# Fung-Lab/MatDeepLearn

Hardware: AMD Instinct MI355X
Metric: edges/sec training CGCNN on bulk_data (higher is better)
Workload: dtype bf16

## Files before the change

### include/mdl_hip.h

```cpp
#ifndef MDL_HIP_H
#define MDL_HIP_H

#include <stddef.h>
#include <stdint.h>

#ifdef __cplusplus
extern "C" {
#endif

#define MDL_VERSION 100

enum { MDL_F32 = 0, MDL_BF16 = 1 };
enum { MDL_SUM = 0, MDL_MEAN = 1, MDL_MAX = 2 };
enum {
    MDL_OK = 0,
    MDL_E_ARG = -1,
    MDL_E_UNSUPP = -2,
    MDL_E_LAUNCH = -3
};

#define MDL_DTYPE_MASK 0xff
#define MDL_DETERMINISTIC 0x100
#define MDL_K3_PER_WAVE 0x200
#define MDL_K3_EDGE_LANE 0x400
#define MDL_BN_SHIFT_ROW 0x800
#define MDL_SPLIT_BF16 0x1000
#define MDL_MLP_F32_IO 0x2000

typedef void* mdlStream_t;

int mdl_version(void);
const char* mdl_last_error_string(void);
int mdl_debug_last_k3(void);

int mdl_rbf_expand(const float* d, const float* offsets, float coeff, void* out, int64_t E, int G,
                   int64_t ld_out, int out_dtype, mdlStream_t stream);

int mdl_csr_rowptr(const int32_t* sorted_index, int64_t E, int64_t N, int32_t* rowptr, mdlStream_t stream);

int mdl_segment_reduce_fwd(const void* src, const int32_t* rowptr, const int32_t* perm, void* out,
                           int32_t* argmax, int64_t N, int64_t C, int reduce, int dtype, mdlStream_t stream);
int mdl_segment_reduce_bwd(const void* grad_out, const int32_t* rowptr, const int32_t* seg,
                           const int32_t* perm, const int32_t* argmax, void* grad_src, int64_t N,
                           int64_t E, int64_t C, int reduce, int dtype, mdlStream_t stream);
int mdl_segment_reduce_bwd_add(const void* grad_out, const int32_t* rowptr, const int32_t* seg, const int32_t* perm,
                               const void* addend, void* grad_src, int64_t N, int64_t E, int64_t C, int reduce, int dtype,
                               mdlStream_t stream);

size_t mdl_cgconv_wpack_bytes(int C, int G, int dtype);
int mdl_cgconv_pack_weights(const float* w_f, const float* b_f, const float* w_s, const float* b_s, int C,
                            int G, void* wpack, float* bpack, int dtype, mdlStream_t stream);
int mdl_cgconv_pack_weights_node(const float* w_f, const float* b_f, const float* w_s, const float* b_s, int C,
                                 int G, void* wpack, float* bpack, void* wn_t, int dtype, mdlStream_t stream);

int mdl_cgconv_pack_weights_multi(int L, const float* const* w_f, const float* const* b_f, const float* const* w_s,
                                  const float* const* b_s, int C, int G, void* const* wpack, float* const* bpack,
                                  void* const* wn_t, int dtype, mdlStream_t stream);

int mdl_cgconv_fwd(const void* x, const void* edge_attr, const int32_t* rowptr, const int32_t* src,
                   const int32_t* tgt, const int32_t* eperm, const void* wpack, const float* bpack,
                   void* out, int64_t N, int64_t E, int C, int G, int aggr, int dtype, mdlStream_t stream);

typedef struct MdlCgConv {
    uint32_t size;
    int32_t dtype;
    uint32_t flags;
    int32_t aggr;
    int64_t N, E;
    int32_t C, G;
    const void* x;
    const void* edge_attr;
    const int32_t* rowptr;
    const int32_t* src;
    const int32_t* tgt;
    const int32_t* eperm;
    const void* wpack;
    const float* bpack;
    void* out;
    const void* grad_out;
    void* r_tgt;
    void* r_src;
    int32_t r_src_dtype;
    float* dwe;
    float* db;
    void* workspace;
    size_t workspace_bytes;
    const int32_t* balance;
} MdlCgConv;
int mdl_cgconv_fwd_ex(const MdlCgConv* args, mdlStream_t stream);
int mdl_cgconv_bwd_ex(const MdlCgConv* args, mdlStream_t stream);

int mdl_cgconv_balance(const int32_t* rowptr, const int32_t* src, int64_t N, int32_t* cost, mdlStream_t stream);

size_t mdl_cgconv_workspace_bytes(int64_t N, int64_t E, int C, int G, int dtype);

typedef struct MdlCgNode {
    uint32_t size;
    int32_t dtype;
    uint32_t flags;
    int32_t zero_src;
    int64_t N;
    int32_t C;
    int32_t r_src_dtype;
    const void* x;
    const void* grad_out;
    const void* r_tgt;
    void* r_src;
    const void* wn_t;
    void* dx;
    float* dwn;
} MdlCgNode;
int mdl_cgconv_bwd_node_ex(const MdlCgNode* args, mdlStream_t stream);

int mdl_cgconv_pack_node_weights(const float* w_f, const float* w_s, int C, int G, void* wn_t, int dtype, mdlStream_t stream);
int mdl_cgconv_assemble_grads(const float* dwn, const float* dwe, const float* db, int C, int G, float* dw_f, float* dw_s,
                              float* db_f, float* db_s, mdlStream_t stream);

int mdl_assemble_batch(const int64_t* ids, const int64_t* noff, const int64_t* eoff, const int64_t* node_ptr,
                       const int64_t* edge_ptr, const float* x_all, const int32_t* src_l, const int32_t* tgt_l,
                       const float* dist, const float* dist_norm, const int32_t* lrowptr, const float* y_all,
                       void* x, int64_t* batch, int32_t* rowptr, int32_t* src, int32_t* tgt, float* ew, float* dn,
                       float* y, int B, int F, int T, int target_index, int dtype, mdlStream_t stream);
int mdl_assemble_batch_padded(const int64_t* ids, const int64_t* noff, const int64_t* eoff, const int64_t* node_ptr,
                              const int64_t* edge_ptr, const float* x_all, const int32_t* src_l, const int32_t* tgt_l,
                              const float* dist, const float* dist_norm, const int32_t* lrowptr, const float* y_all,
                              void* x, int64_t* batch, int32_t* rowptr, int32_t* src, int32_t* tgt, float* ew, float* dn,
                              float* y, int B, int F, int T, int target_index, int dtype, int64_t n_cap, int64_t e_cap,
                              int32_t* pool_seg, int32_t* col_s, int32_t* eid_s, int32_t* src_s, mdlStream_t stream);

int mdl_ssp_bwd(const void* g, const void* y, void* dx, int64_t n, int dtype, mdlStream_t stream);

int mdl_linear_act_stats(const void* x, const void* w, const void* bias, const void* p1, const int32_t* idx1, const void* p2,
                         const int32_t* idx2, const void* p3, const int32_t* idx3, void* out, int64_t N, int K, int M, int act,
                         float* bn_sums, const int64_t* n_rows_dev, int dtype, mdlStream_t stream);
int mdl_linear_gather_act(const void* x, const void* w, const void* bias, const void* p1, const int32_t* idx1,
                          const void* p2, const int32_t* idx2, const void* p3, const int32_t* idx3, void* out,
                          int64_t N, int K, int M, int act, int dtype, mdlStream_t stream);

int mdl_nnconv_msg_fwd(const void* Y, const void* h, const int32_t* rowptr_s, const int32_t* eid_s, void* m, int64_t N,
                       int Co, int D3, int dtype, mdlStream_t stream);
int mdl_nnconv_msg_bwd(const void* Y, const void* h, const void* dm, const int32_t* rowptr_s, const int32_t* eid_s,
                       void* dh, void* dY, int64_t N, int Co, int D3, int dtype, mdlStream_t stream);

int mdl_pad_batch_tail(const int64_t* noff, const int64_t* eoff, int B, int64_t n_cap, int32_t* rowptr, int64_t* batch,
                       mdlStream_t stream);

int mdl_assemble_transposed(const int64_t* ids, const int64_t* noff, const int64_t* eoff, const int64_t* node_ptr,
                            const int64_t* edge_ptr, const int32_t* src_l, const int32_t* tgt_l, const int32_t* eperm_s,
                            const int32_t* lrowptr_s, int32_t* rowptr_s, int32_t* col_s, int32_t* eid_s, int32_t* src_s, int B,
                            int64_t n_cap, mdlStream_t stream);
int mdl_pad_edge_tail(const int64_t* noff, const int64_t* eoff, int B, int64_t n_cap, int64_t e_cap, int32_t* src, int32_t* tgt,
                      int32_t* col_s, int32_t* eid_s, int32_t* src_s, mdlStream_t stream);

int mdl_loss_fwd_bwd(const float* pred, const float* y, int64_t n, int kind, float* loss, float* grad, mdlStream_t stream);
int mdl_loss_fwd_bwd_rows(const float* pred, const float* y, int64_t n, int64_t n_total, int kind, float* loss, float* grad,
                          mdlStream_t stream);

#define MDL_BN_REPLICAS 16
int mdl_bn_sums_rows(void);
int mdl_bn_stats_n(const void* x, float* sums, int64_t N, int C, const int64_t* n_rows_dev, int dtype, mdlStream_t stream);
int mdl_bn_apply_n(const void* x, float* sums, const float* gamma, const float* beta, float* save, float* running_mean,
                   float* running_var, void* y, int64_t N, int C, float eps, float momentum, const int64_t* n_rows_dev,
                   int dtype, mdlStream_t stream);
int mdl_bn_bwd_stats_n(const void* dy, const void* x, const float* save, float* sums, int64_t N, int C,
                       const int64_t* n_rows_dev, int dtype, mdlStream_t stream);
int mdl_bn_bwd_apply_n(const void* dy, const void* x, const float* save, float* sums, const float* gamma, void* dx,
                       int64_t N, int C, const int64_t* n_rows_dev, int dtype, mdlStream_t stream);
int mdl_bn_bwd_apply_relu_n(const void* dy, const void* x, const float* save, float* sums, const float* gamma, void* dx,
                            int64_t N, int C, const int64_t* n_rows_dev, int dtype, mdlStream_t stream);
int mdl_linear_act(const void* x, const void* w, const void* bias, void* out, int64_t N, int K, int M, int act, int dtype,
                   mdlStream_t stream);
int mdl_linear_act_in(const void* x, const void* y, int xact, const void* w, const void* bias, void* out, int64_t N, int K,
                      int M, int act, int dtype, mdlStream_t stream);

int mdl_mlp_head_fwd(const void* x, const void* const* w, const void* const* b, void* const* h, int64_t N, int K0, int NL,
                     const int* M, int dtype, mdlStream_t stream);
int mdl_mlp_head_bwd(const void* x, const void* const* w, const void* const* h, const void* gy, void* dx, float* const* dw,
                     float* const* db, int64_t N, int K0, int NL, const int* M, int dtype, mdlStream_t stream);

int mdl_gru_gates_fwd(const void* gi, const void* gh, const float* h, float* h_out, void* out_lp, int64_t N, int C, int dtype,
                      mdlStream_t stream);
int mdl_gru_gates_bwd(const void* gi, const void* gh, const float* h, const float* g_h, const void* g_lp, void* dgi, void* dgh,
                      float* dh, int64_t N, int C, int dtype, mdlStream_t stream);

int mdl_linear_wide(const void* x, const void* w, void* out, int64_t N, int K, int64_t M, int dtype, mdlStream_t stream);

int mdl_gemm_tn(const void* a, int64_t lda, int M, const void* b, int64_t ldb, int K, float* c, int64_t N, int dtype,
                mdlStream_t stream);
int mdl_gemm_tn_colsum(const void* a, int64_t lda, int M, const void* b, int64_t ldb, int K, float* c, float* colsum,
                       int64_t N, int dtype, mdlStream_t stream);
int mdl_gemm_tn_act(const void* a, int64_t lda, int M, const void* y, int64_t ldy, int act, const void* b, int64_t ldb,
                    int K, float* c, float* colsum, int64_t N, int dtype, mdlStream_t stream);
int mdl_dense_bwd(const void* g, int64_t ldg, int M, const void* y, int64_t ldy, int act, const void* x, int64_t ldx, int K,
                  const void* w, void* dx, int64_t lddx, int xout, void* gm, float* dw, float* db, int64_t N, int dtype,
                  mdlStream_t stream);
size_t mdl_tn_scratch_bytes(void);
int mdl_dense_bwd_ex(const void* g, int64_t ldg, int M, const void* y, int64_t ldy, int act, const void* x, int64_t ldx, int K,
                     const void* w, void* dx, int64_t lddx, int xout, void* gm, float* dw, float* db, void* scratch, int64_t N,
                     int dtype, mdlStream_t stream);
int mdl_gemm_tn_ex(const void* a, int64_t lda, int M, const void* y, int64_t ldy, int act, const void* b, int64_t ldb, int K,
                   float* c, float* colsum, void* scratch, int64_t N, int dtype, mdlStream_t stream);

int mdl_gather_rows(const void* src, const int32_t* idx, void* out, int64_t E, int64_t C, int dtype,
                    mdlStream_t stream);
int mdl_gather_mul_reduce(const void* h, const void* w, const float* scale, const int32_t* rowptr,
                          const int32_t* col, const int32_t* eid, void* out, int64_t N, int64_t F, int reduce,
                          int dtype, mdlStream_t stream);
int mdl_gather_mul_reduce_dw(const void* g, const void* w, const float* scale, const int32_t* rowptr_s,
                             const int32_t* col_s, const int32_t* eid_s, void* dh, const void* h, void* dw,
                             int64_t N, int64_t F, int dtype, mdlStream_t stream);
int mdl_cfconv_supported(int F, int G, int dtype);
size_t mdl_cfconv_wpack_bytes(void);
int mdl_cfconv_pack_weights(const float* w1, const float* b1, const float* w2, const float* b2, int F, int G, void* wpack,
                            mdlStream_t stream);
int mdl_cfconv_fwd(const void* rbf, const float* cut, const void* h, const int32_t* rowptr, const int32_t* src,
                   const int32_t* tgt, const void* wpack, void* out, void* a1, void* w, int64_t N, int64_t E, int F, int G,
                   int dtype, mdlStream_t stream);
size_t mdl_cfconv_bwd_w_scratch_bytes(void);
int mdl_cfconv_bwd_w(const void* rbf, const float* cut, const void* h, const void* g, const int32_t* rowptr, const int32_t* src,
                     const int32_t* tgt, const void* wpack, float* dw1, float* db1, float* dw2, float* db2, void* scratch, int64_t N,
                     int64_t E, int F, int G, int dtype, mdlStream_t stream);
int mdl_edge_mul(const void* a, const int32_t* ia, const void* b, const int32_t* ib, const float* scale, void* out,
                 int64_t E, int64_t F, int dtype, mdlStream_t stream);
int mdl_edge_dot(const void* a, const int32_t* ia, const void* b, const int32_t* ib, const void* w, float* out, int64_t E,
                 int64_t F, int dtype, mdlStream_t stream);
int mdl_cfconv_bwd_edge_supported(int F, int G, int dtype);
int mdl_cfconv_bwd_edge(const void* rbf, const float* cut, const void* h, const void* g, const int32_t* rowptr, const int32_t* src,
                        const int32_t* tgt, const void* wpack, const float* w1, const float* b1, const float* w2, const float* b2,
                        int64_t N, int64_t E, int F, int G, int dtype, float* dcut, void* drbf, const float* d_norm,
                        const float* offsets, float coeff, float scale, float* dd, mdlStream_t stream);

int mdl_split_bf16(const float* src, void* hi, void* lo, int64_t n, mdlStream_t stream);

size_t mdl_graph_workspace_bytes(int64_t N, int64_t G, int max_neighbors);
int mdl_graph_build(const double* pos, const int64_t* node_ptr, const double* cell, const int32_t* pbc, int64_t N, int64_t G,
                    double radius, int max_neighbors, int64_t* edge_ptr, int32_t* src, int32_t* tgt, float* dist,
                    int32_t* out_deg, int64_t edge_capacity, void* workspace, size_t workspace_bytes, mdlStream_t stream);

int mdl_rbf_expand_bwd(const void* g_out, int64_t ld_g, int g_dtype, const float* d, const float* offsets, float coeff,
                       float* dd, int64_t E, int G, mdlStream_t stream);

int mdl_cgconv_bwd_edge(const void* x, const void* edge_attr, const int32_t* rowptr, const int32_t* src, const int32_t* tgt,
                        const void* wpack, const float* bpack, const void* grad_out, int64_t N, int64_t E, int C, int G,
                        int aggr, int dtype, void* de, const float* d_norm, const float* offsets, float coeff, float scale,
                        float* dd, mdlStream_t stream);

int mdl_linear_rbf_dist_grad_supported(int M, int G, int dtype);
int mdl_linear_rbf_dist_grad(const void* g, int64_t ld_g, const void* act_y, int64_t ld_y, const void* w, int dtype,
                             const float* d, const float* offsets, float coeff, float scale, float* dd, int accumulate,
                             int64_t E, int M, int G, mdlStream_t stream);

size_t mdl_edge_geometry_workspace_bytes(int64_t G);
int mdl_edge_geometry_fwd(const double* pos, const int64_t* node_ptr, const double* cell, const int32_t* pbc, int64_t N,
                          int64_t G, const int32_t* src, const int32_t* tgt, int64_t E, float* dist, float* u,
                          void* workspace, size_t workspace_bytes, mdlStream_t stream);
int mdl_edge_geometry_bwd(const float* dd, const float* u, const int32_t* rowptr_t, const int32_t* eid_t,
                          const int32_t* rowptr_s, const int32_t* eid_s, int64_t N, int64_t E, float* dpos,
                          mdlStream_t stream);

size_t mdl_edge_strain_grad_workspace_bytes(int64_t G, int64_t E, int32_t slices);
int mdl_edge_strain_grad(const float* dd, const float* dist, const float* u, const int32_t* rowptr_t, const int32_t* eid_t,
                         const int64_t* node_ptr, int64_t N, int64_t G, int64_t E, int32_t slices, float* out, void* workspace,
                         size_t workspace_bytes, mdlStream_t stream);
// ... 37 lines not shown
```

### matdeeplearn_amd/_build.py

```python
import os
import shutil
import subprocess
import sys
from concurrent.futures import ThreadPoolExecutor

HERE = os.path.dirname(os.path.abspath(__file__))
CSRC = os.path.join(HERE, "csrc")
LIBDIR = os.path.join(HERE, "lib")
OBJDIR = os.path.join(HERE, "lib", "obj")
LIB = os.path.join(LIBDIR, "libmdl_hip.so")
FLAGS = ["--offload-arch=gfx950", "-O3", "-std=c++17", "-fPIC", "-munsafe-fp-atomics", "-Wno-unused-result"]
FILE_FLAGS = {"cgconv_ep.hip": ["-mllvm", "-amdgpu-mfma-vgpr-form=1"], "cfconv.hip": ["-mllvm", "-amdgpu-mfma-vgpr-form=1"],
              "graph_build.hip": ["-ffp-contract=off"],
              "edge_geom.hip": ["-ffp-contract=off"],
              "vacf.hip": ["-ffp-contract=off"]}
FILE_DEPS = {}


def _hipcc():
    for c in (os.environ.get("HIPCC"), "/opt/rocm/bin/hipcc", shutil.which("hipcc")):
        if c and os.path.exists(c):
            return c
    raise RuntimeError("hipcc not found (need ROCm >= 7.0 to build libmdl_hip.so)")


def sources():
    return sorted(os.path.join(CSRC, f) for f in os.listdir(CSRC) if f.endswith(".hip"))


def _deps_mtime():
    hdrs = [os.path.join(CSRC, f) for f in os.listdir(CSRC) if f.endswith((".h", ".inc"))]
    hdrs += [os.path.join(os.path.dirname(HERE), "include", h) for h in ("mdl_hip.h", "mdl_hip_analysis.h", "mdl_hip_dynamics.h")]
    return max(os.path.getmtime(h) for h in hdrs)


def needs_build():
    if not os.path.exists(LIB):
        return True
    t = os.path.getmtime(LIB)
    return any(os.path.getmtime(s) > t for s in sources()) or _deps_mtime() > t


def build(force=False, verbose=True):
    if not force and not needs_build():
        return LIB
    cc = _hipcc()
    os.makedirs(OBJDIR, exist_ok=True)
    hdr_t = _deps_mtime()

    def compile_one(src):
        base = os.path.basename(src)
        obj = os.path.join(OBJDIR, base[:-4] + ".o")
        src_t = max([os.path.getmtime(src)] + [os.path.getmtime(os.path.join(CSRC, d)) for d in FILE_DEPS.get(base, [])])
        if force or not os.path.exists(obj) or os.path.getmtime(obj) < max(src_t, hdr_t):
            cmd = [cc] + FLAGS + FILE_FLAGS.get(base, []) + ["-c", src, "-o", obj]
            if verbose:
                print("[mdl build]", " ".join(cmd), file=sys.stderr)
            subprocess.run(cmd, check=True)
        return obj

    with ThreadPoolExecutor(max_workers=4) as ex:
        objs = list(ex.map(compile_one, sources()))
    cmd = [cc, "--offload-arch=gfx950", "-shared", "-fPIC", "-o", LIB] + objs
    if verbose:
        print("[mdl build]", " ".join(cmd), file=sys.stderr)
    subprocess.run(cmd, check=True)
    return LIB


if __name__ == "__main__":
    print(build(force="--force" in sys.argv))
```

### matdeeplearn_amd/_lib.py

```python
import ctypes
import os

import torch

HERE = os.path.dirname(os.path.abspath(__file__))
LIB_PATH = os.path.join(HERE, "lib", "libmdl_hip.so")


def use_library(path):
    global LIB_PATH, _lib
    if _lib is not None and os.path.abspath(path) != os.path.abspath(LIB_PATH):
        raise MdlError("use_library(%s): %s is already loaded in this process" % (path, LIB_PATH))
    LIB_PATH = path

MDL_F32, MDL_BF16 = 0, 1
MDL_SUM, MDL_MEAN, MDL_MAX = 0, 1, 2
MDL_DTYPE_MASK, MDL_DETERMINISTIC, MDL_K3_PER_WAVE, MDL_K3_EDGE_LANE = 0xFF, 0x100, 0x200, 0x400
MDL_MLP_F32_IO = 0x2000
MDL_SPLIT_BF16 = 0x1000
MDL_BN_SHIFT_ROW = 0x800
MDL_BN_REPLICAS = 16
REDUCE = {"sum": MDL_SUM, "add": MDL_SUM, "mean": MDL_MEAN, "max": MDL_MAX}

_vp, _i64, _i32, _f32, _sz = ctypes.c_void_p, ctypes.c_int64, ctypes.c_int, ctypes.c_float, ctypes.c_size_t
_u32 = ctypes.c_uint32


class MdlCgConv(ctypes.Structure):
    _fields_ = [("size", _u32), ("dtype", _i32), ("flags", _u32), ("aggr", _i32), ("N", _i64), ("E", _i64), ("C", _i32), ("G", _i32),
                ("x", _vp), ("edge_attr", _vp), ("rowptr", _vp), ("src", _vp), ("tgt", _vp), ("eperm", _vp), ("wpack", _vp),
                ("bpack", _vp), ("out", _vp), ("grad_out", _vp), ("r_tgt", _vp), ("r_src", _vp), ("r_src_dtype", _i32),
                ("dwe", _vp), ("db", _vp), ("workspace", _vp), ("workspace_bytes", _sz), ("balance", _vp)]


class MdlCgNode(ctypes.Structure):
    _fields_ = [("size", _u32), ("dtype", _i32), ("flags", _u32), ("zero_src", _i32), ("N", _i64), ("C", _i32), ("r_src_dtype", _i32),
                ("x", _vp), ("grad_out", _vp), ("r_tgt", _vp), ("r_src", _vp), ("wn_t", _vp), ("dx", _vp), ("dwn", _vp)]


def _dp(t):
    return None if t is None else t.data_ptr()


def cg_args(**kw):
    a = MdlCgConv()
    a.size = ctypes.sizeof(MdlCgConv)
    for k, v in kw.items():
        setattr(a, k, _dp(v) if torch.is_tensor(v) else v)
    return a


def cg_node_args(**kw):
    a = MdlCgNode()
    a.size = ctypes.sizeof(MdlCgNode)
    for k, v in kw.items():
        setattr(a, k, _dp(v) if torch.is_tensor(v) else v)
    return a

PROTOTYPES = {
    "mdl_version": (_i32, []),
    "mdl_last_error_string": (ctypes.c_char_p, []),
    "mdl_debug_last_k3": (_i32, []),
    "mdl_rbf_expand": (_i32, [_vp, _vp, _f32, _vp, _i64, _i32, _i64, _i32, _vp]),
    "mdl_csr_rowptr": (_i32, [_vp, _i64, _i64, _vp, _vp]),
    "mdl_segment_reduce_fwd": (_i32, [_vp, _vp, _vp, _vp, _vp, _i64, _i64, _i32, _i32, _vp]),
    "mdl_segment_reduce_bwd": (_i32, [_vp, _vp, _vp, _vp, _vp, _vp, _i64, _i64, _i64, _i32, _i32, _vp]),
    "mdl_segment_reduce_bwd_add": (_i32, [_vp, _vp, _vp, _vp, _vp, _vp, _i64, _i64, _i64, _i32, _i32, _vp]),
    "mdl_cgconv_wpack_bytes": (_sz, [_i32, _i32, _i32]),
    "mdl_cgconv_pack_weights": (_i32, [_vp, _vp, _vp, _vp, _i32, _i32, _vp, _vp, _i32, _vp]),
    "mdl_cgconv_pack_weights_node": (_i32, [_vp, _vp, _vp, _vp, _i32, _i32, _vp, _vp, _vp, _i32, _vp]),
    "mdl_cgconv_pack_weights_multi": (_i32, [_i32, _vp, _vp, _vp, _vp, _i32, _i32, _vp, _vp, _vp, _i32, _vp]),
    "mdl_cgconv_fwd": (_i32, [_vp] * 9 + [_i64, _i64, _i32, _i32, _i32, _i32, _vp]),
    "mdl_cgconv_fwd_ex": (_i32, [ctypes.POINTER(MdlCgConv), _vp]),
    "mdl_cgconv_bwd_ex": (_i32, [ctypes.POINTER(MdlCgConv), _vp]),
    "mdl_cgconv_bwd_node_ex": (_i32, [ctypes.POINTER(MdlCgNode), _vp]),
    "mdl_cgconv_workspace_bytes": (ctypes.c_size_t, [_i64, _i64, _i32, _i32, _i32]),
    "mdl_cgconv_balance": (_i32, [_vp, _vp, _i64, _vp, _vp]),
    "mdl_cgconv_pack_node_weights": (_i32, [_vp, _vp, _i32, _i32, _vp, _i32, _vp]),
    "mdl_cgconv_assemble_grads": (_i32, [_vp, _vp, _vp, _i32, _i32, _vp, _vp, _vp, _vp, _vp]),
    "mdl_assemble_batch": (_i32, [_vp] * 20 + [_i32, _i32, _i32, _i32, _i32, _vp]),
    "mdl_assemble_batch_padded": (_i32, [_vp] * 20 + [_i32, _i32, _i32, _i32, _i32, _i64, _i64, _vp, _vp, _vp, _vp, _vp]),
    "mdl_nnconv_msg_fwd": (_i32, [_vp] * 5 + [_i64, _i32, _i32, _i32, _vp]),
    "mdl_nnconv_msg_bwd": (_i32, [_vp] * 7 + [_i64, _i32, _i32, _i32, _vp]),
    "mdl_pad_batch_tail": (_i32, [_vp, _vp, _i32, _i64, _vp, _vp, _vp]),
    "mdl_assemble_transposed": (_i32, [_vp] * 13 + [_i32, _i64, _vp]),
    "mdl_pad_edge_tail": (_i32, [_vp, _vp, _i32, _i64, _i64, _vp, _vp, _vp, _vp, _vp, _vp]),
    "mdl_loss_fwd_bwd": (_i32, [_vp, _vp, _i64, _i32, _vp, _vp, _vp]),
    "mdl_loss_fwd_bwd_rows": (_i32, [_vp, _vp, _i64, _i64, _i32, _vp, _vp, _vp]),
    "mdl_bn_sums_rows": (_i32, []),
    "mdl_bn_stats_n": (_i32, [_vp, _vp, _i64, _i32, _vp, _i32, _vp]),
    "mdl_bn_apply_n": (_i32, [_vp] * 8 + [_i64, _i32, _f32, _f32, _vp, _i32, _vp]),
    "mdl_bn_bwd_stats_n": (_i32, [_vp, _vp, _vp, _vp, _i64, _i32, _vp, _i32, _vp]),
    "mdl_bn_bwd_apply_n": (_i32, [_vp] * 6 + [_i64, _i32, _vp, _i32, _vp]),
    "mdl_bn_bwd_apply_relu_n": (_i32, [_vp] * 6 + [_i64, _i32, _vp, _i32, _vp]),
    "mdl_linear_act": (_i32, [_vp, _vp, _vp, _vp, _i64, _i32, _i32, _i32, _i32, _vp]),
    "mdl_dense_bwd": (_i32, [_vp, _i64, _i32, _vp, _i64, _i32, _vp, _i64, _i32, _vp, _vp, _i64, _i32, _vp, _vp, _vp, _i64, _i32, _vp]),
    "mdl_dense_bwd_ex": (_i32, [_vp, _i64, _i32, _vp, _i64, _i32, _vp, _i64, _i32, _vp, _vp, _i64, _i32, _vp, _vp, _vp, _vp, _i64, _i32, _vp]),
    "mdl_tn_scratch_bytes": (_sz, []),
    "mdl_linear_act_stats": (_i32, [_vp, _vp, _vp, _vp, _vp, _vp, _vp, _vp, _vp, _vp, _i64, _i32, _i32, _i32, _vp, _vp, _i32, _vp]),
    "mdl_linear_act_in": (_i32, [_vp, _vp, _i32, _vp, _vp, _vp, _i64, _i32, _i32, _i32, _i32, _vp]),
    "mdl_ssp_bwd": (_i32, [_vp, _vp, _vp, _i64, _i32, _vp]),
    "mdl_linear_gather_act": (_i32, [_vp] * 10 + [_i64, _i32, _i32, _i32, _i32, _vp]),
    "mdl_linear_wide": (_i32, [_vp, _vp, _vp, _i64, _i32, _i64, _i32, _vp]),
    "mdl_mlp_head_fwd": (_i32, [_vp, _vp, _vp, _vp, _i64, _i32, _i32, _vp, _i32, _vp]),
    "mdl_mlp_head_bwd": (_i32, [_vp, _vp, _vp, _vp, _vp, _vp, _vp, _i64, _i32, _i32, _vp, _i32, _vp]),
    "mdl_gru_gates_fwd": (_i32, [_vp, _vp, _vp, _vp, _vp, _i64, _i32, _i32, _vp]),
    "mdl_gru_gates_bwd": (_i32, [_vp, _vp, _vp, _vp, _vp, _vp, _vp, _vp, _i64, _i32, _i32, _vp]),
    "mdl_gemm_tn": (_i32, [_vp, _i64, _i32, _vp, _i64, _i32, _vp, _i64, _i32, _vp]),
    "mdl_split_bf16": (_i32, [_vp, _vp, _vp, _i64, _vp]),
    "mdl_gemm_tn_colsum": (_i32, [_vp, _i64, _i32, _vp, _i64, _i32, _vp, _vp, _i64, _i32, _vp]),
    "mdl_gemm_tn_act": (_i32, [_vp, _i64, _i32, _vp, _i64, _i32, _vp, _i64, _i32, _vp, _vp, _i64, _i32, _vp]),
    "mdl_gemm_tn_ex": (_i32, [_vp, _i64, _i32, _vp, _i64, _i32, _vp, _i64, _i32, _vp, _vp, _vp, _i64, _i32, _vp]),
    "mdl_gather_rows": (_i32, [_vp, _vp, _vp, _i64, _i64, _i32, _vp]),
    "mdl_gather_mul_reduce": (_i32, [_vp] * 7 + [_i64, _i64, _i32, _i32, _vp]),
    "mdl_gather_mul_reduce_dw": (_i32, [_vp] * 9 + [_i64, _i64, _i32, _vp]),
    "mdl_edge_mul": (_i32, [_vp] * 6 + [_i64, _i64, _i32, _vp]),
    "mdl_cfconv_supported": (_i32, [_i32, _i32, _i32]),
    "mdl_cfconv_wpack_bytes": (_sz, []),
    "mdl_cfconv_pack_weights": (_i32, [_vp] * 4 + [_i32, _i32, _vp, _vp]),
    "mdl_cfconv_fwd": (_i32, [_vp] * 10 + [_i64, _i64, _i32, _i32, _i32, _vp]),
    "mdl_cfconv_bwd_w_scratch_bytes": (_sz, []),
    "mdl_cfconv_bwd_w": (_i32, [_vp] * 13 + [_i64, _i64, _i32, _i32, _i32, _vp]),
    "mdl_cfconv_bwd_edge_supported": (_i32, [_i32, _i32, _i32]),
    "mdl_cfconv_bwd_edge": (_i32, [_vp] * 12 + [_i64, _i64, _i32, _i32, _i32, _vp, _vp, _vp, _vp, _f32, _f32, _vp, _vp]),
    "mdl_edge_dot": (_i32, [_vp] * 6 + [_i64, _i64, _i32, _vp]),
    "mdl_graph_workspace_bytes": (_sz, [_i64, _i64, _i32]),
    "mdl_graph_build": (_i32, [_vp] * 4 + [_i64, _i64, ctypes.c_double, _i32] + [_vp] * 5 + [_i64, _vp, _sz, _vp]),
    "mdl_rbf_expand_bwd": (_i32, [_vp, _i64, _i32, _vp, _vp, _f32, _vp, _i64, _i32, _vp]),
    "mdl_cgconv_bwd_edge": (_i32, [_vp] * 8 + [_i64, _i64, _i32, _i32, _i32, _i32, _vp, _vp, _vp, _f32, _f32, _vp, _vp]),
    "mdl_linear_rbf_dist_grad_supported": (_i32, [_i32, _i32, _i32]),
    "mdl_linear_rbf_dist_grad": (_i32, [_vp, _i64, _vp, _i64, _vp, _i32, _vp, _vp, _f32, _f32, _vp, _i32, _i64, _i32, _i32, _vp]),
    "mdl_edge_geometry_workspace_bytes": (_sz, [_i64]),
    "mdl_edge_geometry_fwd": (_i32, [_vp] * 4 + [_i64, _i64, _vp, _vp, _i64, _vp, _vp, _vp, _sz, _vp]),
    "mdl_edge_geometry_bwd": (_i32, [_vp] * 6 + [_i64, _i64, _vp, _vp]),
    "mdl_edge_strain_grad_workspace_bytes": (_sz, [_i64, _i64, _i32]),
    "mdl_edge_strain_grad": (_i32, [_vp] * 6 + [_i64, _i64, _i64, _i32, _vp, _vp, _sz, _vp]),
    "mdl_set2set_supported": (_i32, [_i32, _i32, _i32]),
    "mdl_set2set_fwd": (_i32, [_vp] * 12 + [_i64, _i64, _i32, _i32, _i32, _vp]),
    "mdl_set2set_bwd": (_i32, [_vp] * 13 + [_i64, _i64, _i32, _i32, _i32, _vp]),
    "mdl_fire_step": (_i32, [_vp] * 5 + [_i64, _i64] + [_vp] * 7 + [_i32] + [ctypes.c_double] * 6 + [_vp, _vp, _i64] + [_vp] * 9 + [_vp]),
    "mdl_fire_cell_step": (_i32, [_vp] * 13 + [_i64, _i64] + [_vp] * 9 + [_i32] + [ctypes.c_double] * 7 + [_vp]),
    "mdl_md_step": (_i32, [_vp] * 6 + [_i64, _i64] + [_vp] * 8 + [ctypes.c_double] + [_vp] * 6 + [ctypes.c_double, _vp]),
    "mdl_md_velocities": (_i32, [_vp] * 4 + [_i64, _i64, _vp, _vp, _i32, _vp]),
}

_f64 = ctypes.c_double
ANALYSIS_PROTOTYPES = {
    "mdl_rdf_accumulate": (_i32, [_vp] * 6 + [_i64, _i64, _i64, _f64, _i32, _i32] + [_vp] * 4 + [_vp]),
    "mdl_msd_accumulate": (_i32, [_vp] * 8 + [_i64, _i64, _i32, _i32, _i32, _i32, _vp, _vp, _vp]),
}

DYNAMICS_PROTOTYPES = {
    "mdl_md_onstep_velocity": (_i32, [_vp] * 8 + [_i64, _i64, _vp, _vp]),
    "mdl_vacf_accumulate": (_i32, [_vp] * 8 + [_i64, _i64, _i32, _i32, _i32, _i32, _vp, _vp, _vp]),
}

_lib = None


class MdlError(RuntimeError):
    pass


def lib():
    global _lib
    if _lib is None:
        if not os.path.exists(LIB_PATH):
            raise MdlError(
                "libmdl_hip.so not found at %s — build it with `python -m matdeeplearn_amd._build` "
                "(hipcc --offload-arch=gfx950).  matdeeplearn_amd has no CPU/eager fallback." % LIB_PATH)
        handle = ctypes.CDLL(LIB_PATH)
        for name, (res, args) in list(PROTOTYPES.items()) + list(ANALYSIS_PROTOTYPES.items()) + list(DYNAMICS_PROTOTYPES.items()):
            fn = getattr(handle, name)
            fn.restype, fn.argtypes = res, args
        _lib = handle
    return _lib


def check(rc, what):
    if rc != 0:
        raise MdlError("%s failed (%d): %s" % (what, rc, lib().mdl_last_error_string().decode()))


def dtype_code(t):
    if t.dtype == torch.float32:
        return MDL_F32
    if t.dtype == torch.bfloat16:
        return MDL_BF16
    raise MdlError("unsupported dtype %s (float32 or bfloat16)" % t.dtype)


def require_hip(*tensors):
    cur = None
    for t in tensors:
        if t is None:
            continue
        if not t.is_cuda:
            raise MdlError("matdeeplearn_amd ops need tensors on a HIP device (got %s); there is no CPU path — "
                           "the CPU restatement lives in oracle/ and is test infrastructure only" % t.device)
        if cur is None:
            cur = torch.cuda.current_device()
        if t.device.index != cur:
            raise MdlError("tensor on %s but the current HIP device is cuda:%d — call torch.cuda.set_device(%d) in "
                           "this process before using matdeeplearn_amd" % (t.device, cur, t.device.index))


def ptr(t):
    return None if t is None else ctypes.c_void_p(t.data_ptr())


def stream():
    return ctypes.c_void_p(torch._C._cuda_getCurrentRawStream(torch.cuda.current_device()))
```

### matdeeplearn_amd/csrc/cgconv.hip

```cpp
#include "cgconv_tiles.inc"
#include "cgconv_fwd.inc"
#include "cgconv_bwd.inc"

namespace mdl {
#if MDL_EXPERIMENTS
#include "../../experiments/csrc/cgconv_ab.inc"
#include "../../experiments/csrc/cgconv_cb.inc"
#endif
namespace ep {
constexpr int EP_DEFAULT = 2;
constexpr int64_t EP2_MIN_EDGES = 400000;
#if MDL_EXPERIMENTS
int launch(CgParams& p, hipStream_t st, int wgs, const char* name);
#endif
int launch2(CgParams& p, hipStream_t st, int wgs, const char* name);
}

template <typename T>
__device__ __forceinline__ void cgconv_pack_body(const float* __restrict__ wf, const float* __restrict__ bfv,
                                                 const float* __restrict__ ws, const float* __restrict__ bsv,
                                                 int C, int G, const CgDims& d, T* __restrict__ wpack,
                                                 float* __restrict__ bpack, float scale, int bias_col,
                                                 bf16_t* __restrict__ wn_t, int x3 = 0) {
    const int total = 2 * d.Cp * d.WS;
    const int ldw = 2 * C + G;
    if (wn_t) {
        const int tn = C * 4 * d.Cp;
        for (int q = blockIdx.x * blockDim.x + threadIdx.x; q < tn; q += gridDim.x * blockDim.x) {
            const int k = q / (4 * d.Cp), r = q - k * (4 * d.Cp);
            const int blk = r / d.Cp, c = r - blk * d.Cp;
            float v = 0.0f;
            if (c < C) v = ((blk & 1) ? ws : wf)[c * ldw + (blk >> 1) * C + k];
            wn_t[q] = f2bf(v);
        }
    }
    for (int q = blockIdx.x * blockDim.x + threadIdx.x; q < total; q += gridDim.x * blockDim.x) {
        const int row = q / d.WS, k = q - row * d.WS;
        const int part = row / d.Cp, c = row - part * d.Cp;
        const float* W = part ? ws : wf;
        float v = 0.0f;
        if (c < C) {
            if (k < d.KE) {
                if (k < G) v = W[c * ldw + 2 * C + k];
                else if (k == G && bias_col) { const float* b = part ? bsv : bfv; v = b ? b[c] : 0.0f; }
            } else if (k < d.KE + d.Cp) {
                const int kc = k - d.KE;
                if (kc < C) v = W[c * ldw + kc];
            } else if (k < d.KT) {
                const int kc = k - d.KE - d.Cp;
                if (kc < C) v = W[c * ldw + C + kc];
            }
        }
        if constexpr (std::is_same<T, float>::value) {
            if (x3) {
                if (k < d.KT) {
                    unsigned hi, lo;
                    split_pair(v * scale, 0.0f, hi, lo);
                    bf16_t* g = reinterpret_cast<bf16_t*>(wpack + row * d.WS) + (k >> 3) * 16 + (k & 7);
                    g[0] = (bf16_t)(hi & 0xffffu);
                    g[8] = (bf16_t)(lo & 0xffffu);
                } else {
                    wpack[q] = 0.0f;
                }
                continue;
            }
        }
        Elem<T>::st(wpack + q, v * scale);
    }
    for (int q = blockIdx.x * blockDim.x + threadIdx.x; q < 2 * d.Cp; q += gridDim.x * blockDim.x) {
        const int part = q / d.Cp, c = q - part * d.Cp;
        const float* b = part ? bsv : bfv;
        bpack[q] = (c < C && b) ? b[c] * scale : 0.0f;
    }
}

template <typename T>
__global__ __launch_bounds__(256) void cgconv_pack_kernel(const float* __restrict__ wf, const float* __restrict__ bfv,
                                                          const float* __restrict__ ws, const float* __restrict__ bsv,
                                                          int C, int G, CgDims d, T* __restrict__ wpack,
                                                          float* __restrict__ bpack, float scale, int bias_col,
                                                          bf16_t* __restrict__ wn_t = nullptr, int x3 = 0) {
    cgconv_pack_body<T>(wf, bfv, ws, bsv, C, G, d, wpack, bpack, scale, bias_col, wn_t, x3);
}

constexpr int PACK_MAXL = 16;
struct PackMulti {
    const float* wf[PACK_MAXL]; const float* bf[PACK_MAXL]; const float* ws[PACK_MAXL]; const float* bs[PACK_MAXL];
    void* wpack[PACK_MAXL]; float* bpack[PACK_MAXL]; bf16_t* wn_t[PACK_MAXL];
};
template <typename T>
__global__ __launch_bounds__(256) void cgconv_pack_multi_kernel(PackMulti a, int C, int G, CgDims d, float scale, int bias_col, int x3 = 0) {
    const int l = blockIdx.y;
    cgconv_pack_body<T>(a.wf[l], a.bf[l], a.ws[l], a.bs[l], C, G, d, static_cast<T*>(a.wpack[l]), a.bpack[l], scale, bias_col, a.wn_t[l], x3);
}

#if MDL_EXPERIMENTS
__global__ __launch_bounds__(256) void cgconv_pack_split_kernel(const float* __restrict__ wf, const float* __restrict__ bfv,
                                                                const float* __restrict__ ws, const float* __restrict__ bsv,
                                                                int C, int G, int Cp, int KE, int WSe, bf16_t* __restrict__ wpe,
                                                                bf16_t* __restrict__ wproj, float scale) {
    const int ldw = 2 * C + G;
    const int ne = 2 * Cp * WSe, np_ = 2 * 2 * Cp * Cp;
    for (int q = blockIdx.x * blockDim.x + threadIdx.x; q < ne + np_; q += gridDim.x * blockDim.x) {
        float v = 0.0f;
        if (q < ne) {
            const int row = q / WSe, k = q - row * WSe;
            const int part = row / Cp, c = row - part * Cp;
            const float* W = part ? ws : wf;
            if (c < C) {
                if (k < G) v = W[c * ldw + 2 * C + k];
                else if (k == G) { const float* b = part ? bsv : bfv; v = b ? b[c] : 0.0f; }
            }
            wpe[q] = f2bf(v * scale);
        } else {
            const int r = q - ne;
            const int side = r / (2 * Cp * Cp), rr = r - side * (2 * Cp * Cp);
            const int row = rr / Cp, k = rr - row * Cp;
            const int part = row / Cp, c = row - part * Cp;
            const float* W = part ? ws : wf;
            if (c < C && k < C) v = W[c * ldw + side * C + k];
            wproj[r] = f2bf(v * scale);
        }
    }
}
#endif

static constexpr int LDS_CAP = 160 * 1024;
constexpr int FWD_RANGE_EDGES = 64;
constexpr int BWD_RANGE_EDGES = 128;

struct CgEnv {
    int64_t grid_cap;
    int cb_fwd, cb_bwd;
    int cb_wgs;
    int ab_wgs;
    int no_half_groups;
    int no_fast128;
    int no_w_slice;
    int ep;
    int ep_wgs;
};
static const CgEnv& cg_env() {
#if MDL_EXPERIMENTS
    static const CgEnv e = [] {
        CgEnv v;
        const char* s;
        v.grid_cap = (s = getenv("MDL_GRID_CAP")) ? atoll(s) : 0;
        v.cb_fwd = (s = getenv("MDL_CG_CB")) ? (atoi(s) != 0) : -1;
        v.cb_bwd = (s = getenv("MDL_CG_CB_BWD")) ? (atoi(s) != 0) : -1;
        v.cb_wgs = (s = getenv("MDL_CB_WGS")) ? atoi(s) : 0;
        v.ab_wgs = (s = getenv("MDL_AB_WGS")) ? atoi(s) : 0;
        v.no_half_groups = (s = getenv("MDL_CG_NO_HALF")) ? (atoi(s) != 0) : 0;
        v.no_w_slice = (s = getenv("MDL_CG_NO_WSLICE")) ? (atoi(s) != 0) : 0;
        v.no_fast128 = (s = getenv("MDL_CG_NO_FAST128")) ? (atoi(s) != 0) : 0;
        v.ep = (s = getenv("MDL_CG_EP")) ? atoi(s) : -1;
        v.ep_wgs = (s = getenv("MDL_EP_WGS")) ? atoi(s) : 0;
        return v;
    }();
#else
    static const CgEnv e = {0, -1, -1, 0, 0, 0, 0, 0, -1, 0};
#endif
    return e;
}

static volatile int g_last_k3 = 0;

template <typename T>
static int cg_launch(bool bwd, CgParams& p, int dtype, hipStream_t st, const char* name) {
    const bool x3 = (p.flags & MDL_SPLIT_BF16) != 0;
    const CgDims d = cg_dims(p.C, p.G, dtype, x3);
    p.Cp = d.Cp; p.KE = d.KE; p.KT = d.KT; p.WS = d.WS; p.EKS = d.EKS; p.NS = d.NS; p.GP = d.GP;
    p.w_elems = 2 * d.Cp * d.WS;
    const bool wsp = p.pt != nullptr;
    if (wsp) { p.WS = d.EKS; p.w_elems = 2 * d.Cp * d.EKS; }
    p.bias_col = (p.G % 16) != 0;
    p.n_groups = (int)cdiv(p.N, 32);
    if (p.n_groups == 0) return MDL_OK;

    const bool word4 = (p.G * sizeof(T)) % 4 == 0 && (reinterpret_cast<uintptr_t>(p.ea) % 4) == 0;
    const int EW = word4 ? (int)(4 / sizeof(T)) : 1;
    p.GW = p.G / EW;
    p.gw_inv = (unsigned)((0x100000000ull + p.GW - 1) / p.GW);

    int vec = 1;
    if (sizeof(T) == 2) {
        const bool a16 = reinterpret_cast<uintptr_t>(p.x) % 16 == 0, a8 = reinterpret_cast<uintptr_t>(p.x) % 8 == 0;
        if (p.C % 8 == 0 && a16) vec = 8; else if (p.C % 4 == 0 && a8) vec = 4;
    }

    const int et_bytes = (32 * d.EKS * (int)sizeof(T) + 15) & ~15;
    p.wave_lds_bytes = et_bytes + 32 + 128 + 32 + 16 + ((bwd && sizeof(T) == 2) ? 128 * OHS * 2 + 64 + 256 : 0);
    const int w_bytes = (p.w_elems * (int)sizeof(T) + 15) & ~15;
    const bool det = bwd && (p.flags & MDL_DETERMINISTIC) != 0;
    const int waves = det ? 1 : (bwd ? 4 : FWD_THREADS / 64);
    const bool fast = !p.eperm && p.G == 50 && p.C == d.Cp && (d.Cp == 32 || d.Cp == 64) &&
                      (sizeof(T) == 2 ? (vec == 8 && EW == 2) : d.Cp == 64) &&
                      (bwd || (reinterpret_cast<uintptr_t>(p.out) % 16 == 0 && reinterpret_cast<uintptr_t>(p.x) % 16 == 0));
    const bool fast128 = sizeof(T) == 2 && !wsp && !p.ab && !p.eperm && p.G == 50 && p.C == 128 && d.Cp == 128 && vec == 8 && EW == 2 &&
                         p.bias_col && reinterpret_cast<uintptr_t>(p.x) % 16 == 0 &&
                         (bwd ? reinterpret_cast<uintptr_t>(p.gout) % 16 == 0 : reinterpret_cast<uintptr_t>(p.out) % 16 == 0) &&
                         !cg_env().no_fast128;
    bool w_lds = w_bytes + waves * p.wave_lds_bytes <= LDS_CAP;
    int lds = (w_lds ? w_bytes : 0) + waves * p.wave_lds_bytes;
    p.w_slice = 0;
    if (!w_lds && !fast && !wsp && d.NS > 1 && (d.WS * (int)sizeof(T)) % 16 == 0 &&
        64 * d.WS * (int)sizeof(T) + waves * p.wave_lds_bytes <= LDS_CAP && !cg_env().no_w_slice) {
        p.w_slice = 1;
        p.w_elems = 64 * d.WS;
        w_lds = true;
        lds = 64 * d.WS * (int)sizeof(T) + waves * p.wave_lds_bytes;
    }
    const int wg_per_cu = lds * 2 <= LDS_CAP ? 2 : 1;

    const bool all_slices = !bwd && fast && (sizeof(T) == 2 || w_lds);
    const int64_t ranges = std::max<int64_t>(1, std::min<int64_t>(cdiv(p.E, bwd ? BWD_RANGE_EDGES : FWD_RANGE_EDGES), p.N));
    int64_t items = ranges * (all_slices ? 1 : d.NS);
    int64_t grid = cdiv(items, waves);
    const int64_t cap = 256 * ((bwd && BWD_WAVES == 1) ? 1 : wg_per_cu);
    if (grid > cap) grid = cap;
    const CgEnv& env = cg_env();
    if (env.grid_cap > 0 && grid > env.grid_cap) grid = env.grid_cap;
    if (det) { grid = d.NS; p.ctr = nullptr; }
    if constexpr (sizeof(T) == 2) {
        int ep_sel = env.ep >= 0 ? env.ep : ep::EP_DEFAULT;
        if (p.flags & MDL_K3_PER_WAVE) ep_sel = 0;
        const bool force2 = env.ep == 2 || (p.flags & MDL_K3_EDGE_LANE) != 0;
        if (force2) ep_sel = 2;
        if (ep_sel != 0 && !det && bwd && fast && !wsp && d.Cp == 64 && p.bias_col && p.E >= 64) {
            if (ep_sel == 2 && p.rs16 && (force2 || p.E >= ep::EP2_MIN_EDGES)) { g_last_k3 = 2; return ep::launch2(p, st, env.ep_wgs, name); }
#if MDL_EXPERIMENTS
            if (ep_sel == 1 && !p.rs16) return ep::launch(p, st, env.ep_wgs, name);
#endif
        }
    }
    if (bwd) g_last_k3 = det ? 3 : 1;
    p.dwe_combine = (bwd && !det && waves == 4 && d.NS == 2 && w_lds && !p.w_slice && w_bytes >= 2 * 2 * 2 * 16 * 64 * 4) ? 1 : 0;
    while ((grid * waves) % d.NS) ++grid;
    if (p.w_slice) while (grid % d.NS) ++grid;
    p.g_full = p.n_groups;
    if (bwd && p.ctr) {
        if ((int64_t)p.n_groups * d.NS >= 4 * grid * waves && d.NS <= 16) {
            if (hipMemsetAsync(p.ctr, 0, 64, st) != hipSuccess) { set_error("%s: workspace memset failed", name); return MDL_E_LAUNCH; }
            const int64_t tail = 2 * (grid * waves / d.NS);
            p.g_full = (int)std::max<int64_t>(0, (int64_t)p.n_groups - tail);
            if (env.no_half_groups) p.g_full = p.n_groups;
        } else {
            p.ctr = nullptr;
        }
    }

#if MDL_EXPERIMENTS
    if constexpr (sizeof(T) == 2) {
        if (!bwd && p.ab) {
            if (!(fast && all_slices && p.bias_col)) {
                set_error("%s: the saved-gate forward supports bf16, C in {32, 64}, G = 50, target-sorted edge features", name);
                return MDL_E_UNSUPP;
            }
            if (d.Cp == 64) {
                auto kf = cgconv_fwd_kernel<T, 64, 50, 9, 2, 1, true>;
                (void)set_max_dynamic_lds(reinterpret_cast<const void*>(kf), lds);
                hipLaunchKernelGGL(kf, dim3((unsigned)grid), dim3(waves * 64), lds, st, p);
            } else {
                auto kf = cgconv_fwd_kernel<T, 32, 50, 9, 2, 1, true>;
                (void)set_max_dynamic_lds(reinterpret_cast<const void*>(kf), lds);
                hipLaunchKernelGGL(kf, dim3((unsigned)grid), dim3(waves * 64), lds, st, p);
            }
            return check_launch(name);
        }
    }

    if constexpr (sizeof(T) == 2) {
        constexpr int CB_FWD_WG_PER_CU = 2;
        if (env.cb_fwd > 0 && fast && !wsp && !bwd && p.E >= 64 && p.bias_col) {
            const int cb_wgs = env.cb_wgs > 0 ? env.cb_wgs : CB_FWD_WG_PER_CU;
            int64_t cb_grid = std::min<int64_t>(256 * cb_wgs, ranges);
            if (env.grid_cap > 0 && cb_grid > env.grid_cap) cb_grid = env.grid_cap;
            if (d.Cp == 64) {
                const int cb_lds = 2 * cb::Cfg<64>::BUF_FWD;
                hipLaunchKernelGGL(cb::fwd_kernel<64>, dim3((unsigned)cb_grid), dim3(cb::Cfg<64>::NT), cb_lds, st, p);
            } else {
                const int cb_lds = 2 * cb::Cfg<32>::BUF_FWD;
                hipLaunchKernelGGL(cb::fwd_kernel<32>, dim3((unsigned)cb_grid), dim3(cb::Cfg<32>::NT), cb_lds, st, p);
            }
            return check_launch(name);
        }
        if (env.cb_bwd > 0 && fast && !wsp && !p.rs16 && bwd && p.E >= 64 && p.bias_col) {
            const int cb_wgs = env.cb_wgs > 0 ? env.cb_wgs : MDL_CB_BWD_OCC;
            const int64_t cb_grid = std::min<int64_t>(256 * cb_wgs, ranges);
            if (d.Cp == 64) {
                const int cb_lds = 2 * cb::BwdLds<64>::BUF + cb::Cfg<64>::NCB * 32 * (cb::Cfg<64>::KE + 8) * 2;
                auto kf = cb::bwd_kernel<64>;
                set_max_dynamic_lds(reinterpret_cast<const void*>(kf), cb_lds);
                hipLaunchKernelGGL(kf, dim3((unsigned)cb_grid), dim3(cb::Cfg<64>::NT), cb_lds, st, p);
            } else {
                const int cb_lds = 2 * cb::BwdLds<32>::BUF + cb::Cfg<32>::NCB * 32 * (cb::Cfg<32>::KE + 8) * 2;
                auto kf = cb::bwd_kernel<32>;
                set_max_dynamic_lds(reinterpret_cast<const void*>(kf), cb_lds);
                hipLaunchKernelGGL(kf, dim3((unsigned)cb_grid), dim3(cb::Cfg<32>::NT), cb_lds, st, p);
            }
            return check_launch(name);
        }
    }

#endif

#define MDL_CG_LAUNCH(CP_, G_, VEC_, EW_, WM_)                                                               \
    do {                                                                                                     \
        auto kf = bwd ? cgconv_bwd_kernel<T, CP_, G_, VEC_, EW_, WM_> : cgconv_fwd_kernel<T, CP_, G_, VEC_, EW_, WM_>; \
        hipError_t e = set_max_dynamic_lds(reinterpret_cast<const void*>(kf), lds);                 \
        if (e != hipSuccess) { set_error("%s: LDS attribute (%d B): %s", name, lds, hipGetErrorString(e)); return MDL_E_LAUNCH; } \
        hipLaunchKernelGGL(kf, dim3((unsigned)grid), dim3(waves * 64), lds, st, p);                           \
    } while (0)
#define MDL_CG_BY_WL(VEC_, EW_) do { if (w_lds) MDL_CG_LAUNCH(0, 0, VEC_, EW_, 1); else MDL_CG_LAUNCH(0, 0, VEC_, EW_, 0); } while (0)
#define MDL_CG_BY_EW(VEC_) do { if (EW == 2) MDL_CG_BY_WL(VEC_, 2); else MDL_CG_BY_WL(VEC_, 1); } while (0)

#if MDL_EXPERIMENTS
    if (wsp) {
        if constexpr (sizeof(T) == 2) {
            if (!(fast && w_lds && p.bias_col && (bwd || all_slices))) {
                set_error("%s: the W-split kernels support bf16, C in {32, 64}, G = 50, target-sorted edge features", name);
                return MDL_E_UNSUPP;
            }
#define MDL_CG_LAUNCH_WSP(CP_)                                                                                         \
            do {                                                                                                       \
                hipError_t e;                                                                                          \
                if (bwd) {                                                                                             \
                    auto kf = cgconv_bwd_kernel<T, CP_, 50, 9, 2, 1, 1>;                                               \
                    e = set_max_dynamic_lds(reinterpret_cast<const void*>(kf), lds);                                   \
                    if (e == hipSuccess) hipLaunchKernelGGL(kf, dim3((unsigned)grid), dim3(waves * 64), lds, st, p);   \
                } else {                                                                                               \
                    auto kf = cgconv_fwd_kernel<T, CP_, 50, 9, 2, 1, false, 1>;                                        \
                    e = set_max_dynamic_lds(reinterpret_cast<const void*>(kf), lds);                                   \
                    if (e == hipSuccess) hipLaunchKernelGGL(kf, dim3((unsigned)grid), dim3(waves * 64), lds, st, p);   \
                }                                                                                                      \
                if (e != hipSuccess) { set_error("%s: LDS attribute (%d B): %s", name, lds, hipGetErrorString(e)); return MDL_E_LAUNCH; } \
            } while (0)
            if (d.Cp == 64) MDL_CG_LAUNCH_WSP(64); else MDL_CG_LAUNCH_WSP(32);
#undef MDL_CG_LAUNCH_WSP
            return check_launch(name);
        } else {
            set_error("%s: the W-split kernels are bf16 only", name);
            return MDL_E_UNSUPP;
        }
    }
#endif
#ifdef MDL_CG_FAST_ONLY
    if constexpr (sizeof(T) == 2) {
        if (fast && d.Cp == 64) MDL_CG_LAUNCH(64, 50, 9, 2, 1);
        else if (fast128 && p.w_slice) MDL_CG_LAUNCH(128, 50, 9, 2, 1);
    }
#else
    if constexpr (sizeof(T) == 2) {
        if (fast && d.Cp == 64) MDL_CG_LAUNCH(64, 50, 9, 2, 1);
        else if (fast && d.Cp == 32) MDL_CG_LAUNCH(32, 50, 9, 2, 1);
        else if (fast128 && p.w_slice) MDL_CG_LAUNCH(128, 50, 9, 2, 1);
        else if (vec == 8) MDL_CG_BY_EW(8);
        else if (vec == 4) MDL_CG_BY_EW(4);
        else MDL_CG_BY_EW(1);
    } else {
        if (x3) {
            const bool x3_64 = fast && w_lds && d.Cp == 64;
            const bool x3_128 = !p.eperm && p.G == 50 && p.C == 128 && d.Cp == 128 && w_lds && p.w_slice;
            if (!((x3_64 || x3_128) && p.bias_col && !wsp && !det && reinterpret_cast<uintptr_t>(p.x) % 16 == 0)) {
                set_error("%s: MDL_SPLIT_BF16 needs fp32, C = 64 or 128, G = 50, edge features in CSR order, 16-byte aligned x", name);
                return MDL_E_UNSUPP;
            }
            hipError_t e;
#define MDL_CG_LAUNCH_X3(CP_)                                                                                                 \
            do {                                                                                                              \
                if (bwd) {                                                                                                    \
                    auto kf = cgconv_bwd_kernel<T, CP_, 50, 9, 1, 1, 0, true>;                                                \
                    e = set_max_dynamic_lds(reinterpret_cast<const void*>(kf), lds);                                          \
                    if (e == hipSuccess) hipLaunchKernelGGL(kf, dim3((unsigned)grid), dim3(waves * 64), lds, st, p);          \
                } else {                                                                                                      \
                    auto kf = cgconv_fwd_kernel<T, CP_, 50, 9, 1, 1, false, 0, true>;                                         \
                    e = set_max_dynamic_lds(reinterpret_cast<const void*>(kf), lds);                                          \
                    if (e == hipSuccess) hipLaunchKernelGGL(kf, dim3((unsigned)grid), dim3(waves * 64), lds, st, p);          \
                }                                                                                                             \
            } while (0)
            if (x3_64) MDL_CG_LAUNCH_X3(64); else MDL_CG_LAUNCH_X3(128);
#undef MDL_CG_LAUNCH_X3
            if (e != hipSuccess) { set_error("%s: LDS attribute (%d B): %s", name, lds, hipGetErrorString(e)); return MDL_E_LAUNCH; }
        }
        else if (fast && w_lds) MDL_CG_LAUNCH(64, 50, 9, 1, 1);
        else MDL_CG_BY_WL(1, 1);
    }
#endif
#undef MDL_CG_BY_EW
// ... 163 lines not shown
    p.flags = (int)(a->flags & MDL_SPLIT_BF16);
    if (a->dtype == MDL_BF16) return cg_launch<bf16_t>(false, p, a->dtype, (hipStream_t)stream, "mdl_cgconv_fwd_ex");
    return cg_launch<float>(false, p, a->dtype, (hipStream_t)stream, "mdl_cgconv_fwd_ex");
}

extern "C" size_t mdl_cgconv_workspace_bytes(int64_t, int64_t, int, int, int) { return 64; }

#if MDL_EXPERIMENTS
extern "C" size_t mdl_cgconv_gate_row_bytes(int C, int G, int dtype) {
    return (dtype == MDL_BF16 && G == 50 && (C == 32 || C == 64)) ? (size_t)4 * C : 0;
}

extern "C" int mdl_cgconv_fwd_save(const void* x, const void* edge_attr, const int32_t* rowptr, const int32_t* src,
                                   const int32_t* tgt, const void* wpack, const float* bpack, void* out, void* gate,
                                   int64_t N, int64_t E, int C, int G, int aggr, int dtype, mdlStream_t stream) {
    using namespace mdl;
    int rc = cg_check("mdl_cgconv_fwd_save", x, edge_attr, rowptr, src, tgt, wpack, bpack, N, E, C, G, aggr, dtype);
    if (rc) return rc;
    MDL_REQUIRE(mdl_cgconv_gate_row_bytes(C, G, dtype) != 0, MDL_E_UNSUPP,
                "mdl_cgconv_fwd_save: unsupported C=%d G=%d dtype=%d (bf16, C in {32, 64}, G = 50)", C, G, dtype);
    MDL_REQUIRE(N == 0 || out, MDL_E_ARG, "mdl_cgconv_fwd_save: null out");
    MDL_REQUIRE(E == 0 || (gate && reinterpret_cast<uintptr_t>(gate) % 4 == 0), MDL_E_ARG, "mdl_cgconv_fwd_save: bad gate buffer");
    MDL_REQUIRE(reinterpret_cast<uintptr_t>(x) % 16 == 0 && reinterpret_cast<uintptr_t>(edge_attr) % 4 == 0, MDL_E_ARG,
                "mdl_cgconv_fwd_save: x must be 16-byte and edge_attr 4-byte aligned");
    CgParams p = {};
    p.x = x; p.ea = edge_attr; p.rowptr = rowptr; p.src = src; p.tgt = tgt; p.eperm = nullptr;
    p.wpack = wpack; p.bpack = bpack; p.out = out; p.ab = E ? gate : nullptr; p.N = N; p.E = E; p.C = C; p.G = G; p.aggr = aggr;
    return cg_launch<bf16_t>(false, p, dtype, (hipStream_t)stream, "mdl_cgconv_fwd_save");
}

extern "C" int mdl_cgconv_bwd_saved(const void* edge_attr, const int32_t* rowptr, const int32_t* src, const int32_t* tgt,
                                    const void* gate, const void* grad_out, void* r_tgt, float* r_src, float* dwe, float* db,
                                    int64_t N, int64_t E, int C, int G, int aggr, int dtype, void* workspace, size_t ws_bytes,
                                    mdlStream_t stream) {
    using namespace mdl;
    MDL_REQUIRE(mdl_cgconv_gate_row_bytes(C, G, dtype) != 0, MDL_E_UNSUPP,
                "mdl_cgconv_bwd_saved: unsupported C=%d G=%d dtype=%d (bf16, C in {32, 64}, G = 50)", C, G, dtype);
    MDL_REQUIRE(N >= 0 && E >= 0 && N < (1ll << 31) - 64 && E < (1ll << 31) - 64, MDL_E_ARG, "mdl_cgconv_bwd_saved: bad N=%lld E=%lld",
                (long long)N, (long long)E);
    MDL_REQUIRE(aggr == MDL_MEAN || aggr == MDL_SUM, MDL_E_UNSUPP, "mdl_cgconv_bwd_saved: unsupported aggr %d", aggr);
    MDL_REQUIRE(N == 0 || (rowptr && grad_out && r_tgt && r_src && dwe), MDL_E_ARG, "mdl_cgconv_bwd_saved: null pointer");
    MDL_REQUIRE(E == 0 || (edge_attr && src && tgt && gate), MDL_E_ARG, "mdl_cgconv_bwd_saved: null edge pointer");
    MDL_REQUIRE(reinterpret_cast<uintptr_t>(gate) % 4 == 0 && reinterpret_cast<uintptr_t>(edge_attr) % 4 == 0, MDL_E_ARG,
                "mdl_cgconv_bwd_saved: gate / edge_attr must be 4-byte aligned");
    CgParams p = {};
    p.ea = edge_attr; p.rowptr = rowptr; p.src = src; p.tgt = tgt; p.ab = const_cast<void*>(gate); p.gout = grad_out;
    p.r_tgt = r_tgt; p.r_src = r_src; p.dwe = dwe; p.db = db; p.N = N; p.E = E; p.C = C; p.G = G; p.aggr = aggr;
    p.ctr = (workspace && ws_bytes >= 64) ? static_cast<unsigned*>(workspace) : nullptr;
    return cg_launch_bwd_ab(p, (hipStream_t)stream, "mdl_cgconv_bwd_saved");
}

extern "C" size_t mdl_cgconv_wsplit_bytes(int C, int G, int dtype, int which) {
    using namespace mdl;
    if (dtype != MDL_BF16 || G != 50 || (C != 32 && C != 64)) return 0;
    const CgDims d = cg_dims(C, G, dtype);
    const size_t b = which == 0 ? (size_t)2 * d.Cp * d.EKS * 2 : (size_t)2 * 2 * d.Cp * d.Cp * 2;
    return (b + 15) & ~(size_t)15;
}

extern "C" int mdl_cgconv_pack_weights_split(const float* w_f, const float* b_f, const float* w_s, const float* b_s, int C,
                                             int G, void* wpack_e, void* wproj, float* bpack, int dtype, mdlStream_t stream) {
    using namespace mdl;
    MDL_REQUIRE(w_f && w_s && wpack_e && wproj && bpack, MDL_E_ARG, "mdl_cgconv_pack_weights_split: null pointer");
    MDL_REQUIRE(mdl_cgconv_wsplit_bytes(C, G, dtype, 0) != 0, MDL_E_UNSUPP,
                "mdl_cgconv_pack_weights_split: unsupported C=%d G=%d dtype=%d (bf16, C in {32, 64}, G = 50)", C, G, dtype);
    const CgDims d = cg_dims(C, G, dtype);
    const int total = 2 * d.Cp * d.EKS + 4 * d.Cp * d.Cp;
    hipStream_t st = (hipStream_t)stream;
    hipLaunchKernelGGL(cgconv_pack_split_kernel, dim3((unsigned)cdiv(total, 256)), dim3(256), 0, st, w_f, b_f, w_s, b_s, C, G, d.Cp,
                       d.KE, d.EKS, (bf16_t*)wpack_e, (bf16_t*)wproj, Gate<true>::W_SCALE);
    if (hipMemsetAsync(bpack, 0, 2 * d.Cp * sizeof(float), st) != hipSuccess) { set_error("mdl_cgconv_pack_weights_split: memset failed"); return MDL_E_LAUNCH; }
    return check_launch("mdl_cgconv_pack_weights_split");
}

extern "C" int mdl_cgconv_fwd_p(const void* x, const void* p_tgt, const void* p_src, const void* edge_attr, const int32_t* rowptr,
                                const int32_t* src, const int32_t* tgt, const void* wpack_e, const float* bpack, void* out,
                                int64_t N, int64_t E, int C, int G, int aggr, int dtype, mdlStream_t stream) {
    using namespace mdl;
    int rc = cg_check("mdl_cgconv_fwd_p", x, edge_attr, rowptr, src, tgt, wpack_e, bpack, N, E, C, G, aggr, dtype);
    if (rc) return rc;
    MDL_REQUIRE(N == 0 || (out && p_tgt && p_src), MDL_E_ARG, "mdl_cgconv_fwd_p: null pointer");
    MDL_REQUIRE(reinterpret_cast<uintptr_t>(p_tgt) % 16 == 0 && reinterpret_cast<uintptr_t>(p_src) % 16 == 0, MDL_E_ARG,
                "mdl_cgconv_fwd_p: the projections must be 16-byte aligned");
    CgParams p = {};
    p.x = x; p.pt = p_tgt; p.ps = p_src; p.ea = edge_attr; p.rowptr = rowptr; p.src = src; p.tgt = tgt; p.eperm = nullptr;
    p.wpack = wpack_e; p.bpack = bpack; p.out = out; p.N = N; p.E = E; p.C = C; p.G = G; p.aggr = aggr;
    if (dtype != MDL_BF16) { set_error("mdl_cgconv_fwd_p: bf16 only"); return MDL_E_UNSUPP; }
    return cg_launch<bf16_t>(false, p, dtype, (hipStream_t)stream, "mdl_cgconv_fwd_p");
}

extern "C" int mdl_cgconv_bwd_p(const void* p_tgt, const void* p_src, const void* edge_attr, const int32_t* rowptr,
                                const int32_t* src, const int32_t* tgt, const void* wpack_e, const float* bpack,
                                const void* grad_out, void* r_tgt, float* r_src, float* dwe, float* db, int64_t N, int64_t E,
                                int C, int G, int aggr, int dtype, void* workspace, size_t ws_bytes, mdlStream_t stream) {
    using namespace mdl;
    int rc = cg_check("mdl_cgconv_bwd_p", p_tgt, edge_attr, rowptr, src, tgt, wpack_e, bpack, N, E, C, G, aggr, dtype);
    if (rc) return rc;
    MDL_REQUIRE(N == 0 || (grad_out && r_tgt && r_src && dwe && p_src), MDL_E_ARG, "mdl_cgconv_bwd_p: null pointer");
    MDL_REQUIRE(reinterpret_cast<uintptr_t>(p_tgt) % 16 == 0 && reinterpret_cast<uintptr_t>(p_src) % 16 == 0, MDL_E_ARG,
                "mdl_cgconv_bwd_p: the projections must be 16-byte aligned");
    CgParams p = {};
    p.x = p_tgt; p.pt = p_tgt; p.ps = p_src; p.ea = edge_attr; p.rowptr = rowptr; p.src = src; p.tgt = tgt; p.eperm = nullptr;
    p.wpack = wpack_e; p.bpack = bpack; p.gout = grad_out; p.r_tgt = r_tgt; p.r_src = r_src; p.dwe = dwe; p.db = db;
    p.N = N; p.E = E; p.C = C; p.G = G; p.aggr = aggr;
    p.ctr = (workspace && ws_bytes >= mdl_cgconv_workspace_bytes(N, E, C, G, dtype)) ? static_cast<unsigned*>(workspace) : nullptr;
    if (dtype != MDL_BF16) { set_error("mdl_cgconv_bwd_p: bf16 only"); return MDL_E_UNSUPP; }
    return cg_launch<bf16_t>(true, p, dtype, (hipStream_t)stream, "mdl_cgconv_bwd_p");
}
#endif

namespace mdl {
__global__ __launch_bounds__(256) void cgconv_balance_kernel(const int32_t* __restrict__ rowptr, const int32_t* __restrict__ src,
                                                             int64_t N, int32_t* __restrict__ cost, int far_w, int far_t, int zero_w) {
    const int64_t n = (int64_t)blockIdx.x * blockDim.x + threadIdx.x;
    if (n == 0) cost[0] = 0;
    if (n >= N) return;
    const int b = rowptr[n], e = rowptr[n + 1];
    int far = 0;
    for (int k = b; k < e; ++k) {
        const int d = src[k] - (int)n;
        far += (d >= far_t || d <= -far_t) ? 1 : 0;
    }
    cost[n + 1] = 4 * (e - b + 1) + far_w * far + (e == b ? zero_w : 0);
}
}

extern "C" int mdl_cgconv_balance(const int32_t* rowptr, const int32_t* src, int64_t N, int32_t* cost, mdlStream_t stream) {
    using namespace mdl;
    MDL_REQUIRE(N >= 0 && (N == 0 || (rowptr && src && cost)), MDL_E_ARG, "mdl_cgconv_balance: bad arguments");
#if MDL_EXPERIMENTS
    static const int far_w = [] { const char* s = getenv("MDL_BAL_W"); return s ? atoi(s) : 5; }();
    static const int far_t = [] { const char* s = getenv("MDL_BAL_T"); return s ? atoi(s) : 48; }();
    static const int zero_w = [] { const char* s = getenv("MDL_BAL_Z"); return s ? atoi(s) : 4; }();
#else
    constexpr int far_w = 5, far_t = 48, zero_w = 4;
#endif
    hipLaunchKernelGGL(cgconv_balance_kernel, dim3((unsigned)cdiv(N + 1, 256)), dim3(256), 0, (hipStream_t)stream, rowptr, src, N, cost,
                       far_w, far_t, zero_w);
    return check_launch("mdl_cgconv_balance");
}

extern "C" int mdl_cgconv_bwd_ex(const MdlCgConv* a, mdlStream_t stream) {
    using namespace mdl;
    MDL_REQUIRE(a && a->size == sizeof(MdlCgConv), MDL_E_ARG, "mdl_cgconv_bwd_ex: argument struct of another layout (size %u, expected %u)",
                a ? a->size : 0u, (unsigned)sizeof(MdlCgConv));
    MDL_REQUIRE((a->flags & ~(uint32_t)(MDL_DETERMINISTIC | MDL_K3_PER_WAVE | MDL_K3_EDGE_LANE | MDL_SPLIT_BF16)) == 0, MDL_E_ARG,
                "mdl_cgconv_bwd_ex: unknown flag bits %#x", a->flags);
    MDL_REQUIRE(!(a->flags & MDL_SPLIT_BF16) || (a->dtype == MDL_F32 && !(a->flags & MDL_DETERMINISTIC)), MDL_E_UNSUPP,
                "mdl_cgconv_bwd_ex: MDL_SPLIT_BF16 goes with MDL_F32 storage (and not with MDL_DETERMINISTIC)");
    const int dtype = a->dtype;
    int rc = cg_check("mdl_cgconv_bwd_ex", a->x, a->edge_attr, a->rowptr, a->src, a->tgt, a->wpack, a->bpack, a->N, a->E, a->C, a->G,
                      a->aggr, dtype);
    if (rc) return rc;
    MDL_REQUIRE(a->N == 0 || (a->grad_out && a->r_tgt && a->r_src && a->dwe), MDL_E_ARG, "mdl_cgconv_bwd_ex: null pointer");
    MDL_REQUIRE(a->r_src_dtype == MDL_F32 || a->r_src_dtype == MDL_BF16, MDL_E_ARG, "mdl_cgconv_bwd_ex: r_src_dtype must be MDL_F32 or MDL_BF16");
    CgParams p = {};
    p.flags = (int)a->flags;
    p.x = a->x; p.ea = a->edge_attr; p.rowptr = a->rowptr; p.src = a->src; p.tgt = a->tgt; p.eperm = a->eperm;
    p.wpack = a->wpack; p.bpack = a->bpack; p.gout = a->grad_out; p.r_tgt = a->r_tgt; p.r_src = static_cast<float*>(a->r_src);
    p.dwe = a->dwe; p.db = a->db;
    p.N = a->N; p.E = a->E; p.C = a->C; p.G = a->G; p.aggr = a->aggr;
    p.ctr = (a->workspace && a->workspace_bytes >= mdl_cgconv_workspace_bytes(a->N, a->E, a->C, a->G, dtype))
                ? static_cast<unsigned*>(a->workspace) : nullptr;
    if (a->r_src_dtype == MDL_BF16) {
        MDL_REQUIRE(dtype == MDL_BF16 && a->G == 50 && (a->C == 32 || a->C == 64 || a->C == 128) && !a->eperm, MDL_E_UNSUPP,
                    "mdl_cgconv_bwd_ex: bf16 by-source sums need bf16, C in {32, 64, 128}, G = 50, no eperm (C=%d G=%d dtype=%d)",
                    a->C, a->G, dtype);
        MDL_REQUIRE(reinterpret_cast<uintptr_t>(a->x) % 16 == 0 && reinterpret_cast<uintptr_t>(a->edge_attr) % 4 == 0 &&
                        reinterpret_cast<uintptr_t>(a->r_src) % 4 == 0, MDL_E_ARG,
                    "mdl_cgconv_bwd_ex: x must be 16-byte, edge_attr / r_src 4-byte aligned");
        p.rs16 = 1;
        p.balance = a->balance;
    } else {
        MDL_REQUIRE(!a->balance && (a->flags & (MDL_K3_PER_WAVE | MDL_K3_EDGE_LANE)) == 0, MDL_E_ARG,
                    "mdl_cgconv_bwd_ex: the balance prefix and the MDL_K3_* flags go with bf16 by-source sums");
    }
    if (dtype == MDL_BF16) return cg_launch<bf16_t>(true, p, dtype, (hipStream_t)stream, "mdl_cgconv_bwd_ex");
    return cg_launch<float>(true, p, dtype, (hipStream_t)stream, "mdl_cgconv_bwd_ex");
}

extern "C" int mdl_debug_last_k3(void) { return mdl::g_last_k3; }
```

### matdeeplearn_amd/csrc/cgconv_ep.hip

```cpp
#define MDL_CG_EP_TU 1
#include "cgconv_tiles.inc"

namespace mdl {
#include "cgconv_ep_common.inc"
#if MDL_EXPERIMENTS
#include "../../experiments/csrc/cgconv_ep.inc"
#endif
#include "cgconv_ep2.inc"
namespace ep {
int launch2(CgParams& p, hipStream_t st, int wgs, const char* name) {
    typedef Cfg2<64> F;
    const int64_t eg = std::min<int64_t>(wgs > 0 ? wgs : 256, std::max<int64_t>(1, cdiv(p.E, 32 * F::NA * 2)));
    auto kf = bwd2_kernel<64>;
    hipError_t e = set_max_dynamic_lds(reinterpret_cast<const void*>(kf), F::LDS);
    if (e != hipSuccess) { set_error("%s: LDS attribute (%d B): %s", name, F::LDS, hipGetErrorString(e)); return MDL_E_LAUNCH; }
    p.ctr = nullptr;
    hipLaunchKernelGGL(kf, dim3((unsigned)eg), dim3(F::NT), F::LDS, st, p);
    return check_launch(name);
}
#if MDL_EXPERIMENTS
int launch(CgParams& p, hipStream_t st, int wgs, const char* name) {
    typedef Cfg<64> F;
    const int64_t eg = std::min<int64_t>(wgs > 0 ? wgs : 256, std::max<int64_t>(1, cdiv(p.E, 32 * F::NW * 2)));
    auto kf = bwd_kernel<64>;
    hipError_t e = set_max_dynamic_lds(reinterpret_cast<const void*>(kf), F::LDS);
    if (e != hipSuccess) { set_error("%s: LDS attribute (%d B): %s", name, F::LDS, hipGetErrorString(e)); return MDL_E_LAUNCH; }
    hipLaunchKernelGGL(kf, dim3((unsigned)eg), dim3(F::NT), F::LDS, st, p);
    return check_launch(name);
}
#endif
}
}
```

### matdeeplearn_amd/csrc/cgconv_ep2.inc

```

namespace ep {

template <int C_>
struct Cfg2 {
    static constexpr int NB = 2 * C_ / 32;
    static constexpr int NA = 4;
    static constexpr int NT = (NA + NB) * WAVE;
    static constexpr int G = 50, KE = 64, EKS = KE + 8;
    static constexpr int KT = KE + 2 * C_;
    static constexpr int WS = KT + 8;
    static constexpr int NKX = C_ / 16;
    static constexpr int NWT = 4;
    static constexpr int WOFF = 48;
    static constexpr int NCH = 2 * C_ / 4;
    static constexpr int DCS = 32 * 8 + 32;
    static constexpr int W_BYTES = 2 * C_ * WS * 2;
    static constexpr int OFF_ET = 0;
    static constexpr int OFF_DP = OFF_ET + 32 * EKS * 2;
    static constexpr int OFF_TSL = OFF_DP + NCH * DCS;
    static constexpr int OFF_SSL = OFF_TSL + 64;
    static constexpr int OFF_META = OFF_SSL + 64;
    static constexpr int BUF = OFF_META + 32;
    static constexpr int LDS = W_BYTES + 2 * NA * BUF;
    static_assert(NB == 4 && NA == 4, "written for C = 64");
// ... 292 lines not shown
        for (int r = 0; r < 16; ++r) A[r] = 0.0f;
    };
    const unsigned rsplat = (unsigned)(i << OHK_SH) * 0x00010001u;

    bf16x8 dpf[2];
    u32x2 tq[2][2], sq[2][2];
    auto request = [&](const char* bj) {
        const char* a = bj + F::OFF_DP + (8 * cb + 4 * (i >> 4) + (t16 & 3)) * F::DCS + (4 * h + (t16 >> 2)) * 8;
#pragma unroll
        for (int ks = 0; ks < 2; ++ks) {
            const s16x4 lo = __builtin_amdgcn_ds_read_tr16_b64_v4i16((lds4_t)(a + 128 * ks));
            const s16x4 hi = __builtin_amdgcn_ds_read_tr16_b64_v4i16((lds4_t)(a + 128 * ks + 64));
            dpf[ks] = bf16x8{lo[0], lo[1], lo[2], lo[3], hi[0], hi[1], hi[2], hi[3]};
        }
        const u32x2* tw = reinterpret_cast<const u32x2*>(bj + F::OFF_TSL) + h;
        const u32x2* sw = reinterpret_cast<const u32x2*>(bj + F::OFF_SSL) + h;
#pragma unroll
        for (int ks = 0; ks < 2; ++ks) {
            tq[ks][0] = tw[4 * ks]; tq[ks][1] = tw[4 * ks + 2];
            sq[ks][0] = sw[4 * ks]; sq[ks][1] = sw[4 * ks + 2];
        }
    };

    auto tile_step = [&](const char* bj, int jn0, int jn1, int jfl, unsigned touched, const char* bnext) {
        const bool valid = (jfl & 1) != 0;
        const bool act = valid && ((jfl >> 8) & 0xff) != 0;
        const bool newg = valid && jn0 != cn0;
        TMARK(0);
        if (newg) {
            const int nwb = max(jn0 - F::WOFF, 0);
            if (cn0 >= 0) {
                TMARK(7);
                flush_r();
                TMARK(8);
                if (act && nwb == cwb + 32) {
                    flush_w(Wacc[0], cwb);
                    TMARK(9);
#pragma unroll
                    for (int mt = 0; mt + 1 < NWT; ++mt) Wacc[mt] = Wacc[mt + 1];
                    zero16(Wacc[NWT - 1]);
                    TMARK(10);
                } else if (!act || nwb != cwb) {
#pragma unroll
                    for (int mt = 0; mt < NWT; ++mt) {
                        flush_w(Wacc[mt], cwb + 32 * mt);
                        zero16(Wacc[mt]);
                    }
                }
            }
            zero16(Racc);
            cwb = nwb;
        }
        if (valid && !act) {
            bf16_t* rt = static_cast<bf16_t*>(p.r_tgt);
#pragma unroll
            for (int r = 0; r < 16; ++r) {
                const int n = jn0 + d_row(r, h);
                if (n < jn1) rt[(int64_t)n * C2 + col] = 0;
            }
        }
        cn0 = valid ? (act ? jn0 : -1) : cn0;
        cn1 = valid ? jn1 : cn1;
        TMARK(1);
        if (!act) {
            request(bnext);
            return;
        }
        unsigned xs[2][4];
        const bf16x8 d0 = dpf[0], d1 = dpf[1];
        {
            const u32x2 t0 = tq[0][0], t1 = tq[0][1];
            const bf16x8 tf0 = __builtin_bit_cast(bf16x8, u32x4{oh2x(t0[0] ^ rsplat), oh2x(t0[1] ^ rsplat), oh2x(t1[0] ^ rsplat), oh2x(t1[1] ^ rsplat)});
            asm volatile("s_nop 1\n\tv_mfma_f32_32x32x16_bf16 %[R], %[t0], %[d0], %[R]" : [R] "+v"(Racc) : [t0] "v"(tf0), [d0] "v"(d0));
            const u32x2 u0 = tq[1][0], u1 = tq[1][1];
            const bf16x8 tf1 = __builtin_bit_cast(bf16x8, u32x4{oh2x(u0[0] ^ rsplat), oh2x(u0[1] ^ rsplat), oh2x(u1[0] ^ rsplat), oh2x(u1[1] ^ rsplat)});
#pragma unroll
            for (int ks = 0; ks < 2; ++ks) {
                const u32x2 s0 = sq[ks][0], s1 = sq[ks][1];
                xs[ks][0] = s0[0] ^ rsplat; xs[ks][1] = s0[1] ^ rsplat; xs[ks][2] = s1[0] ^ rsplat; xs[ks][3] = s1[1] ^ rsplat;
            }
            asm volatile("s_nop 1\n\tv_mfma_f32_32x32x16_bf16 %[R], %[t1], %[d1], %[R]\n\ts_nop 3" : [R] "+v"(Racc) : [t1] "v"(tf1), [d1] "v"(d1));
        }
        TMARK(2);
        bf16x8 ebf[2][2];
        {
            const bf16_t* const etj = reinterpret_cast<const bf16_t*>(bj + F::OFF_ET);
#pragma unroll
            for (int nt = 0; nt < 2; ++nt)
#pragma unroll
                for (int ks = 0; ks < 2; ++ks) {
                    const bf16_t* base = etj + (16 * ks + 4 * h + (t16 >> 2)) * F::EKS + nt * 32 + (i & 16) + 4 * (t16 & 3);
                    const s16x4 lo = __builtin_amdgcn_ds_read_tr16_b64_v4i16((lds4_t)(base));
                    const s16x4 hi = __builtin_amdgcn_ds_read_tr16_b64_v4i16((lds4_t)(base + 8 * F::EKS));
                    ebf[nt][ks] = bf16x8{lo[0], lo[1], lo[2], lo[3], hi[0], hi[1], hi[2], hi[3]};
                }
        }
        request(bnext);
#pragma unroll
        for (int mt = 0; mt < NWT; ++mt) {
            if (touched & (1u << mt)) {
                const unsigned m = (unsigned)((32 * mt) << OHK_SH) * 0x00010001u;
                const bf16x8 w0 = __builtin_bit_cast(bf16x8, u32x4{oh2x(xs[0][0] ^ m), oh2x(xs[0][1] ^ m), oh2x(xs[0][2] ^ m), oh2x(xs[0][3] ^ m)});
                asm volatile("s_nop 1\n\tv_mfma_f32_32x32x16_bf16 %[W], %[w0], %[d0], %[W]" : [W] "+v"(Wacc[mt]) : [w0] "v"(w0), [d0] "v"(d0));
                const bf16x8 w1 = __builtin_bit_cast(bf16x8, u32x4{oh2x(xs[1][0] ^ m), oh2x(xs[1][1] ^ m), oh2x(xs[1][2] ^ m), oh2x(xs[1][3] ^ m)});
                asm volatile("s_nop 1\n\tv_mfma_f32_32x32x16_bf16 %[W], %[w1], %[d1], %[W]\n\ts_nop 3" : [W] "+v"(Wacc[mt]) : [w1] "v"(w1), [d1] "v"(d1));
            }
        }
        TMARK(3);
        asm volatile(
            "v_mfma_f32_32x32x16_bf16 %[E0], %[d0], %[e00], %[E0]\n\t"
            "v_mfma_f32_32x32x16_bf16 %[E1], %[d0], %[e10], %[E1]\n\t"
            "v_mfma_f32_32x32x16_bf16 %[E0], %[d1], %[e01], %[E0]\n\t"
            "v_mfma_f32_32x32x16_bf16 %[E1], %[d1], %[e11], %[E1]\n\t"
            "s_nop 7"
            : [E0] "+v"(dwe[0]), [E1] "+v"(dwe[1])
            : [d0] "v"(d0), [d1] "v"(d1), [e00] "v"(ebf[0][0]), [e01] "v"(ebf[0][1]), [e10] "v"(ebf[1][0]), [e11] "v"(ebf[1][1]));
        TMARK(4);
    };

    {
        bool rh0, rh1, rh2;
        (void)take<NA>(p, wk, 0, rh0);
        (void)take<NA>(p, wk, 0, rh1);
        (void)take<NA>(p, wk, 0, rh2);
        bool have = rh0;
        for (int t = 0;; ++t) {
            if (t > 0) {
                const char* set = smem + F::W_BYTES + (((t - 1) & 1) * NA) * F::BUF;
                have = __builtin_amdgcn_readfirstlane(reinterpret_cast<const int*>(set + F::OFF_META)[6]) != 0;
                TMARK(11);
                const i32x4 hd = *reinterpret_cast<const i32x4*>(set + (lane & (NA - 1)) * F::BUF + F::OFF_META);
                request(set);
                TMARK(12);
#pragma unroll 1
                for (int j = 0; j < NA; ++j)
                    tile_step(set + j * F::BUF, __builtin_amdgcn_readlane(hd[0], j), __builtin_amdgcn_readlane(hd[1], j),
                              __builtin_amdgcn_readlane(hd[2], j), (unsigned)__builtin_amdgcn_readlane(hd[3], j),
                              set + ((j + 1) & (NA - 1)) * F::BUF);
            }
            TMARK(5);
            lds_barrier();
            TMARK(6);
            TTILE();
            if (!have) break;
        }
    }
    if (cn0 >= 0) {
        flush_r();
#pragma unroll
        for (int mt = 0; mt < NWT; ++mt) flush_w(Wacc[mt], cwb + 32 * mt);
    }
    TFLUSH(32);
    asm volatile("s_nop 15\n\ts_nop 15\n\ts_nop 15\n\ts_nop 15\n\ts_nop 15\n\ts_nop 15" : "+v"(dwe[0]), "+v"(dwe[1]));
#pragma unroll
    for (int nt = 0; nt < 2; ++nt) {
        const int gcol = nt * 32 + i;
        if (gcol < F::G) {
#pragma unroll
            for (int r = 0; r < 16; ++r) unsafeAtomicAdd(p.dwe + (int64_t)(32 * cb + d_row(r, h)) * p.GP + gcol, dwe[nt][r] * escale);
        } else if (gcol == F::G && p.db) {
#pragma unroll
            for (int r = 0; r < 16; ++r) unsafeAtomicAdd(p.db + 32 * cb + d_row(r, h), dwe[nt][r] * escale);
        }
    }
}

}
```

### matdeeplearn_amd/csrc/cgconv_node.hip

```cpp
#include "mdl_common.h"

namespace mdl {

constexpr int K3C_NW = 8;

typedef __attribute__((ext_vector_type(4))) unsigned u32x4_t;

__device__ __forceinline__ bf16x8 pack8(const float* v) {
    u32x4_t r = {pk_bf16(v[0], v[1]), pk_bf16(v[2], v[3]), pk_bf16(v[4], v[5]), pk_bf16(v[6], v[7])};
    return __builtin_bit_cast(bf16x8, r);
}

template <int CP, bool RS16 = false, int NW = 4>
__global__ __launch_bounds__(64 * NW, 2) void cgconv_node_stream_kernel(const bf16_t* __restrict__ x, const bf16_t* __restrict__ gout,
                                                                    const bf16_t* __restrict__ r_tgt,
                                                                    const float* __restrict__ r_src,
                                                                    const bf16_t* __restrict__ wn_t, bf16_t* __restrict__ dx,
                                                                    float* __restrict__ dwn, int64_t N, int zero_src) {
    typedef __attribute__((ext_vector_type(4))) short s16x4;
    typedef __attribute__((address_space(3))) s16x4* lds4_t;
    constexpr int TN = 64;
    constexpr int K4 = 4 * CP;
    constexpr int LD = K4 + 8;
    constexpr int LX = CP + 8;
    constexpr int NT = CP / 32;
    constexpr int TCH = 2 * CP / 8;
    constexpr int SCH = 2 * CP / 4;
    constexpr int NTH = 64 * NW;
    constexpr int NTL = TN * TCH / NTH;
    constexpr int NSL = RS16 ? NTL : TN * SCH / NTH;
    constexpr int XCH = CP / 8;
    constexpr int NXL = TN * XCH / NTH;
    constexpr int MJ = (K4 / 32) * NT / NW;
    static_assert(NTL >= 1 && NSL >= 1 && NXL >= 1 && MJ >= 1, "too many waves for this width");
    extern __shared__ __attribute__((aligned(16))) char smem[];
    bf16_t* wl = reinterpret_cast<bf16_t*>(smem);
    bf16_t* rl = wl + CP * LD;
    bf16_t* xl = rl + TN * LD;
    const int tid = threadIdx.x, lane = tid & 63, i = lane & 31, h = lane >> 5, wv = __builtin_amdgcn_readfirstlane(tid >> 6);
    for (int q = tid; q < CP * (K4 / 8); q += NTH) {
        const int row = q / (K4 / 8), c8 = q - row * (K4 / 8);
        *reinterpret_cast<bf16x8*>(wl + row * LD + c8 * 8) = *reinterpret_cast<const bf16x8*>(wn_t + row * K4 + c8 * 8);
    }
    f32x16 dw[MJ];
#pragma unroll
    for (int j = 0; j < MJ; ++j)
#pragma unroll
        for (int r = 0; r < 16; ++r) dw[j][r] = 0.0f;

    const int64_t n_tiles = (N + TN - 1) / TN;
    u32x4_t treg[NTL];
    f32x4 sreg[NSL];
    u32x4_t xreg[NXL];
    static_assert(NTH % TCH == 0 && NTH % SCH == 0 && NTH % XCH == 0, "chunk mapping");
    constexpr int TROWS = NTH / TCH, SROWS = NTH / SCH, XROWS = NTH / XCH;
    const int trow0 = tid / TCH, tcc = tid % TCH, srow0 = tid / SCH, scc = tid % SCH, xrow0 = tid / XCH, xcc = tid % XCH;
    const int to = (trow0 * (2 * CP) + 8 * tcc) * 2, so = (srow0 * (2 * CP) + 4 * scc) * 4, xo = (xrow0 * CP + 8 * xcc) * 2;
    auto rsrc = [](const void* base, int64_t bytes) {
        return __builtin_amdgcn_make_buffer_rsrc(const_cast<void*>(base), 0, (int)(bytes < 0x7fffffffLL ? bytes : 0x7fffffffLL), 0x00020000);
    };
    auto opaque = [](int v) { asm volatile("" : "+s"(v)); return v; };
    auto load_tile = [&](int64_t tile) {
        const int64_t nb = tile * TN, rem = N - nb;
        const __amdgpu_buffer_rsrc_t tr = rsrc(r_tgt + nb * (2 * CP), rem * (2 * CP * 2));
        const __amdgpu_buffer_rsrc_t sr = RS16 ? rsrc(reinterpret_cast<const bf16_t*>(r_src) + nb * (2 * CP), rem * (2 * CP * 2))
                                               : rsrc(r_src + nb * (2 * CP), rem * (2 * CP * 4));
        const __amdgpu_buffer_rsrc_t xr = rsrc(x + nb * CP, rem * (CP * 2));
#pragma unroll
        for (int l = 0; l < NTL; ++l) treg[l] = __builtin_amdgcn_raw_buffer_load_b128(tr, to + opaque(l * (TROWS * 2 * CP * 2)), 0, 0);
#pragma unroll
        for (int l = 0; l < NSL; ++l)
            sreg[l] = __builtin_bit_cast(f32x4, __builtin_amdgcn_raw_buffer_load_b128(
                sr, RS16 ? to + opaque(l * (TROWS * 2 * CP * 2)) : so + opaque(l * (SROWS * 2 * CP * 4)), 0, 0));
#pragma unroll
        for (int l = 0; l < NXL; ++l) xreg[l] = __builtin_amdgcn_raw_buffer_load_b128(xr, xo + opaque(l * (XROWS * CP * 2)), 0, 0);
    };
    int64_t tile = blockIdx.x;
    if (tile < n_tiles) load_tile(tile);
    for (; tile < n_tiles; tile += gridDim.x) {
        const int64_t nb = tile * TN;
        __syncthreads();
#pragma unroll
        for (int l = 0; l < NTL; ++l) *reinterpret_cast<u32x4_t*>(rl + (trow0 + l * TROWS) * LD + 8 * tcc) = treg[l];
#pragma unroll
        for (int l = 0; l < NSL; ++l) {
            if constexpr (RS16) {
                *reinterpret_cast<u32x4_t*>(rl + (trow0 + l * TROWS) * LD + 2 * CP + 8 * tcc) = __builtin_bit_cast(u32x4_t, sreg[l]);
            } else {
                typedef __attribute__((ext_vector_type(2))) unsigned u32x2_t;
                const u32x2_t v = {pk_bf16(sreg[l][0], sreg[l][1]), pk_bf16(sreg[l][2], sreg[l][3])};
                *reinterpret_cast<u32x2_t*>(rl + (srow0 + l * SROWS) * LD + 2 * CP + 4 * scc) = v;
            }
        }
        if (zero_src) {
            const int64_t rem = N - nb;
            const __amdgpu_buffer_rsrc_t sz = RS16 ? rsrc(reinterpret_cast<const bf16_t*>(r_src) + nb * (2 * CP), rem * (2 * CP * 2))
                                                   : rsrc(r_src + nb * (2 * CP), rem * (2 * CP * 4));
#pragma unroll
            for (int l = 0; l < NSL; ++l)
                __builtin_amdgcn_raw_buffer_store_b128(u32x4_t{0u, 0u, 0u, 0u}, sz,
                                                       RS16 ? to + opaque(l * (TROWS * 2 * CP * 2)) : so + opaque(l * (SROWS * 2 * CP * 4)), 0, 0);
        }
#pragma unroll
        for (int l = 0; l < NXL; ++l) {
            *reinterpret_cast<u32x4_t*>(xl + (xrow0 + l * XROWS) * LX + 8 * xcc) = xreg[l];
        }
        __syncthreads();
        const bool dxw = wv < 2 * NT;
        const int mt0 = wv / NT, nt0 = wv - mt0 * NT;
        const int64_t remg = N - nb - mt0 * 32;
        const int go = (4 * h * CP + nt0 * 32 + i) * 2;
        const bool more = tile + gridDim.x < n_tiles;
        if (!dxw) {
            if (more) load_tile(tile + gridDim.x);
        } else {
            short gv[16];
            const __amdgpu_buffer_rsrc_t gr = rsrc(gout + (nb + mt0 * 32) * CP, (remg > 0 ? remg : 0) * (CP * 2));
#pragma unroll
            for (int r = 0; r < 16; ++r) gv[r] = __builtin_amdgcn_raw_buffer_load_b16(gr, go + ((r & 3) + 8 * (r >> 2)) * CP * 2, 0, 0);
            if (more) load_tile(tile + gridDim.x);
            f32x16 acc;
#pragma unroll
            for (int r = 0; r < 16; ++r) acc[r] = 0.0f;
#pragma unroll
            for (int kk = 0; kk < K4 / 16; ++kk) {
                const bf16x8 a = *reinterpret_cast<const bf16x8*>(rl + (mt0 * 32 + i) * LD + 16 * kk + 8 * h);
                const bf16x8 b = *reinterpret_cast<const bf16x8*>(wl + (nt0 * 32 + i) * LD + 16 * kk + 8 * h);
                acc = __builtin_amdgcn_mfma_f32_32x32x16_bf16(a, b, acc, 0, 0, 0);
            }
            const __amdgpu_buffer_rsrc_t dr = rsrc(dx + (nb + mt0 * 32) * CP, (remg > 0 ? remg : 0) * (CP * 2));
#pragma unroll
            for (int r = 0; r < 16; ++r)
                __builtin_amdgcn_raw_buffer_store_b16((short)f2bf(bf2f((bf16_t)gv[r]) + acc[r]), dr, go + ((r & 3) + 8 * (r >> 2)) * CP * 2, 0, 0);
        }
#pragma unroll
        for (int j = 0; j < MJ; ++j) {
            const int blk = wv * MJ + j, mt = blk / NT, nt = blk - mt * NT;
            const int t = i & 15;
#pragma unroll
            for (int ks = 0; ks < TN / 16; ++ks) {
                const bf16_t* pa = rl + (16 * ks + 8 * h + (t >> 2)) * LD + mt * 32 + (i & 16) + 4 * (t & 3);
                const bf16_t* pb = xl + (16 * ks + 8 * h + (t >> 2)) * LX + nt * 32 + (i & 16) + 4 * (t & 3);
                const s16x4 a0 = __builtin_amdgcn_ds_read_tr16_b64_v4i16((lds4_t)pa), a1 = __builtin_amdgcn_ds_read_tr16_b64_v4i16((lds4_t)(pa + 4 * LD));
                const s16x4 b0 = __builtin_amdgcn_ds_read_tr16_b64_v4i16((lds4_t)pb), b1 = __builtin_amdgcn_ds_read_tr16_b64_v4i16((lds4_t)(pb + 4 * LX));
                const bf16x8 af = {a0[0], a0[1], a0[2], a0[3], a1[0], a1[1], a1[2], a1[3]};
                const bf16x8 bfr = {b0[0], b0[1], b0[2], b0[3], b1[0], b1[1], b1[2], b1[3]};
                dw[j] = __builtin_amdgcn_mfma_f32_32x32x16_bf16(af, bfr, dw[j], 0, 0, 0);
            }
        }
    }
#pragma unroll
    for (int j = 0; j < MJ; ++j) {
        const int blk = wv * MJ + j, mt = blk / NT, nt = blk - mt * NT;
#pragma unroll
        for (int r = 0; r < 16; ++r) {
            const int R = mt * 32 + d_row(r, h), K = nt * 32 + i;
            unsafeAtomicAdd(dwn + (int64_t)R * CP + K, dw[j][r]);
        }
    }
}

template <int CP, int NW>
__global__ __launch_bounds__(64 * NW, 1) void cgconv_node_x3_kernel(const float* __restrict__ x, const float* __restrict__ gout,
                                                                    const float* __restrict__ r_tgt, float* __restrict__ r_src,
                                                                    const float* __restrict__ wn_t, float* __restrict__ dx,
                                                                    float* __restrict__ dwn, int64_t N, int zero_src) {
    typedef __attribute__((ext_vector_type(4))) short s16x4;
    typedef __attribute__((address_space(3))) s16x4* lds4_t;
    typedef __attribute__((ext_vector_type(2))) unsigned u32x2_t;
    constexpr int TN = 64, K4 = 4 * CP, LD = K4 + 8, LX = CP + 8, NT = CP / 32, NTH = 64 * NW;
    constexpr int RCH = 2 * CP / 4;
    constexpr int XCH = CP / 4;
    constexpr int NRL = TN * RCH / NTH;
    constexpr int NXL = TN * XCH / NTH;
    constexpr int MJ = (K4 / 32) * NT / NW;
    static_assert(NRL >= 1 && NXL >= 1 && MJ >= 1 && NTH % RCH == 0 && NTH % XCH == 0 && 2 * NT <= NW, "shape / wave count");
    extern __shared__ __attribute__((aligned(16))) char smem[];
    bf16_t* wl_h = reinterpret_cast<bf16_t*>(smem);
    bf16_t* wl_l = wl_h + CP * LD;
    bf16_t* rl_h = wl_l + CP * LD;
    bf16_t* rl_l = rl_h + TN * LD;
    bf16_t* xl_h = rl_l + TN * LD;
    bf16_t* xl_l = xl_h + TN * LX;
    const int tid = threadIdx.x, lane = tid & 63, i = lane & 31, h = lane >> 5, wv = __builtin_amdgcn_readfirstlane(tid >> 6);
    auto split4 = [](const f32x4& v, u32x2_t& hi, u32x2_t& lo) {
        const unsigned ha = pk_bf16(v[0], v[1]), hb = pk_bf16(v[2], v[3]);
        hi = u32x2_t{ha, hb};
        lo = u32x2_t{pk_bf16(v[0] - __builtin_bit_cast(float, ha << 16), v[1] - __builtin_bit_cast(float, ha & 0xffff0000u)),
                     pk_bf16(v[2] - __builtin_bit_cast(float, hb << 16), v[3] - __builtin_bit_cast(float, hb & 0xffff0000u))};
    };
    for (int q = tid; q < CP * (K4 / 4); q += NTH) {
        const int row = q / (K4 / 4), c4 = q - row * (K4 / 4);
        u32x2_t hi, lo;
        split4(*reinterpret_cast<const f32x4*>(wn_t + row * K4 + c4 * 4), hi, lo);
        *reinterpret_cast<u32x2_t*>(wl_h + row * LD + c4 * 4) = hi;
        *reinterpret_cast<u32x2_t*>(wl_l + row * LD + c4 * 4) = lo;
    }
    f32x16 dw[MJ];
#pragma unroll
    for (int j = 0; j < MJ; ++j)
#pragma unroll
        for (int r = 0; r < 16; ++r) dw[j][r] = 0.0f;

    const int64_t n_tiles = (N + TN - 1) / TN;
    f32x4 treg[NRL], sreg[NRL], xreg[NXL];
    constexpr int RROWS = NTH / RCH, XROWS = NTH / XCH;
    const int rrow0 = tid / RCH, rcc = tid % RCH, xrow0 = tid / XCH, xcc = tid % XCH;
    const int ro = (rrow0 * (2 * CP) + 4 * rcc) * 4, xo = (xrow0 * CP + 4 * xcc) * 4;
    auto rsrc = [](const void* base, int64_t bytes) {
        return __builtin_amdgcn_make_buffer_rsrc(const_cast<void*>(base), 0, (int)(bytes < 0 ? 0 : (bytes < 0x7fffffffLL ? bytes : 0x7fffffffLL)), 0x00020000);
    };
    auto opaque = [](int v) { asm volatile("" : "+s"(v)); return v; };
    auto load_tile = [&](int64_t tile) {
        const int64_t nb = tile * TN, rem = N - nb;
        const __amdgpu_buffer_rsrc_t tr = rsrc(r_tgt + nb * (2 * CP), rem * (2 * CP * 4));
        const __amdgpu_buffer_rsrc_t sr = rsrc(r_src + nb * (2 * CP), rem * (2 * CP * 4));
        const __amdgpu_buffer_rsrc_t xr = rsrc(x + nb * CP, rem * (CP * 4));
#pragma unroll
        for (int l = 0; l < NRL; ++l) treg[l] = __builtin_bit_cast(f32x4, __builtin_amdgcn_raw_buffer_load_b128(tr, ro + opaque(l * (RROWS * 2 * CP * 4)), 0, 0));
#pragma unroll
        for (int l = 0; l < NRL; ++l) sreg[l] = __builtin_bit_cast(f32x4, __builtin_amdgcn_raw_buffer_load_b128(sr, ro + opaque(l * (RROWS * 2 * CP * 4)), 0, 0));
#pragma unroll
        for (int l = 0; l < NXL; ++l) xreg[l] = __builtin_bit_cast(f32x4, __builtin_amdgcn_raw_buffer_load_b128(xr, xo + opaque(l * (XROWS * CP * 4)), 0, 0));
    };
    int64_t tile = blockIdx.x;
    if (tile < n_tiles) load_tile(tile);
    for (; tile < n_tiles; tile += gridDim.x) {
        const int64_t nb = tile * TN;
        __syncthreads();
#pragma unroll
        for (int l = 0; l < NRL; ++l) {
            u32x2_t hi, lo;
            split4(treg[l], hi, lo);
            *reinterpret_cast<u32x2_t*>(rl_h + (rrow0 + l * RROWS) * LD + 4 * rcc) = hi;
            *reinterpret_cast<u32x2_t*>(rl_l + (rrow0 + l * RROWS) * LD + 4 * rcc) = lo;
            split4(sreg[l], hi, lo);
            *reinterpret_cast<u32x2_t*>(rl_h + (rrow0 + l * RROWS) * LD + 2 * CP + 4 * rcc) = hi;
            *reinterpret_cast<u32x2_t*>(rl_l + (rrow0 + l * RROWS) * LD + 2 * CP + 4 * rcc) = lo;
        }
        if (zero_src) {
            const __amdgpu_buffer_rsrc_t sz = rsrc(r_src + nb * (2 * CP), (N - nb) * (2 * CP * 4));
#pragma unroll
            for (int l = 0; l < NRL; ++l)
                __builtin_amdgcn_raw_buffer_store_b128(u32x4_t{0u, 0u, 0u, 0u}, sz, ro + opaque(l * (RROWS * 2 * CP * 4)), 0, 0);
        }
#pragma unroll
        for (int l = 0; l < NXL; ++l) {
            u32x2_t hi, lo;
            split4(xreg[l], hi, lo);
            *reinterpret_cast<u32x2_t*>(xl_h + (xrow0 + l * XROWS) * LX + 4 * xcc) = hi;
            *reinterpret_cast<u32x2_t*>(xl_l + (xrow0 + l * XROWS) * LX + 4 * xcc) = lo;
        }
        __syncthreads();
        const bool dxw = wv < 2 * NT;
        const int mt0 = wv / NT, nt0 = wv - mt0 * NT;
        const int64_t remg = N - nb - mt0 * 32;
        const int go = (4 * h * CP + nt0 * 32 + i) * 4;
        const bool more = tile + gridDim.x < n_tiles;
        if (!dxw) {
            if (more) load_tile(tile + gridDim.x);
        } else {
            float gv[16];
            const __amdgpu_buffer_rsrc_t gr = rsrc(gout + (nb + mt0 * 32) * CP, (remg > 0 ? remg : 0) * (CP * 4));
#pragma unroll
            for (int r = 0; r < 16; ++r)
                gv[r] = __builtin_bit_cast(float, __builtin_amdgcn_raw_buffer_load_b32(gr, go + ((r & 3) + 8 * (r >> 2)) * CP * 4, 0, 0));
            if (more) load_tile(tile + gridDim.x);
            f32x16 acc;
#pragma unroll
            for (int r = 0; r < 16; ++r) acc[r] = 0.0f;
#pragma unroll
            for (int kk = 0; kk < K4 / 16; ++kk) {
                const int ao = (mt0 * 32 + i) * LD + 16 * kk + 8 * h, bo = (nt0 * 32 + i) * LD + 16 * kk + 8 * h;
                const bf16x8 ah = *reinterpret_cast<const bf16x8*>(rl_h + ao), al = *reinterpret_cast<const bf16x8*>(rl_l + ao);
                const bf16x8 bh = *reinterpret_cast<const bf16x8*>(wl_h + bo), bl = *reinterpret_cast<const bf16x8*>(wl_l + bo);
                acc = __builtin_amdgcn_mfma_f32_32x32x16_bf16(al, bh, acc, 0, 0, 0);
                acc = __builtin_amdgcn_mfma_f32_32x32x16_bf16(ah, bl, acc, 0, 0, 0);
                acc = __builtin_amdgcn_mfma_f32_32x32x16_bf16(ah, bh, acc, 0, 0, 0);
            }
            const __amdgpu_buffer_rsrc_t dr = rsrc(dx + (nb + mt0 * 32) * CP, (remg > 0 ? remg : 0) * (CP * 4));
#pragma unroll
            for (int r = 0; r < 16; ++r)
                __builtin_amdgcn_raw_buffer_store_b32(__builtin_bit_cast(unsigned, gv[r] + acc[r]), dr, go + ((r & 3) + 8 * (r >> 2)) * CP * 4, 0, 0);
        }
#pragma unroll
        for (int j = 0; j < MJ; ++j) {
            const int blk = wv * MJ + j, mt = blk / NT, nt = blk - mt * NT;
            const int t = i & 15;
#pragma unroll
            for (int ks = 0; ks < TN / 16; ++ks) {
                const int pa = (16 * ks + 8 * h + (t >> 2)) * LD + mt * 32 + (i & 16) + 4 * (t & 3);
                const int pb = (16 * ks + 8 * h + (t >> 2)) * LX + nt * 32 + (i & 16) + 4 * (t & 3);
                auto frag = [&](const bf16_t* base, int off, int ld) {
                    const s16x4 v0 = __builtin_amdgcn_ds_read_tr16_b64_v4i16((lds4_t)(base + off));
                    const s16x4 v1 = __builtin_amdgcn_ds_read_tr16_b64_v4i16((lds4_t)(base + off + 4 * ld));
                    return bf16x8{v0[0], v0[1], v0[2], v0[3], v1[0], v1[1], v1[2], v1[3]};
                };
                const bf16x8 ah = frag(rl_h, pa, LD), al = frag(rl_l, pa, LD), bh = frag(xl_h, pb, LX), bl = frag(xl_l, pb, LX);
                dw[j] = __builtin_amdgcn_mfma_f32_32x32x16_bf16(al, bh, dw[j], 0, 0, 0);
                dw[j] = __builtin_amdgcn_mfma_f32_32x32x16_bf16(ah, bl, dw[j], 0, 0, 0);
                dw[j] = __builtin_amdgcn_mfma_f32_32x32x16_bf16(ah, bh, dw[j], 0, 0, 0);
            }
        }
    }
#pragma unroll
    for (int j = 0; j < MJ; ++j) {
        const int blk = wv * MJ + j, mt = blk / NT, nt = blk - mt * NT;
#pragma unroll
        for (int r = 0; r < 16; ++r) {
            const int R = mt * 32 + d_row(r, h), K = nt * 32 + i;
            unsafeAtomicAdd(dwn + (int64_t)R * CP + K, dw[j][r]);
        }
    }
}

}

namespace mdl {
template <typename TO>
__global__ __launch_bounds__(256) void cgconv_pack_node_kernel(const float* __restrict__ wf, const float* __restrict__ ws, int C,
                                                               int Cp, int ldw, TO* __restrict__ wn_t) {
    const int total = C * 4 * Cp;
    for (int q = blockIdx.x * blockDim.x + threadIdx.x; q < total; q += gridDim.x * blockDim.x) {
        const int k = q / (4 * Cp), r = q - k * (4 * Cp);
        const int blk = r / Cp, c = r - blk * Cp;
        float v = 0.0f;
        if (c < C) v = ((blk & 1) ? ws : wf)[c * ldw + (blk >> 1) * C + k];
        if constexpr (std::is_same<TO, float>::value) wn_t[q] = v; else wn_t[q] = f2bf(v);
    }
}
__global__ __launch_bounds__(256) void cgconv_grads_kernel(const float* __restrict__ dwn, const float* __restrict__ dwe,
                                                           const float* __restrict__ db, int C, int Cp, int G, int GP,
                                                           float* __restrict__ dwf, float* __restrict__ dws,
                                                           float* __restrict__ dbf, float* __restrict__ dbs) {
    const int ldw = 2 * C + G, total = 2 * C * ldw;
    for (int q = blockIdx.x * blockDim.x + threadIdx.x; q < total; q += gridDim.x * blockDim.x) {
        const int part = q / (C * ldw), rem = q - part * (C * ldw);
        const int c = rem / ldw, k = rem - c * ldw;
        float v;
        if (k < C) v = dwn[(part * Cp + c) * C + k];
        else if (k < 2 * C) v = dwn[((2 + part) * Cp + c) * C + (k - C)];
        else v = dwe[(part * Cp + c) * GP + (k - 2 * C)];
        (part ? dws : dwf)[rem] = v;
    }
    for (int q = blockIdx.x * blockDim.x + threadIdx.x; q < 2 * C; q += gridDim.x * blockDim.x) {
        const int part = q / C, c = q - part * C;
        float* dst = part ? dbs : dbf;
        if (dst) dst[c] = db[part * Cp + c];
    }
}
}

extern "C" int mdl_cgconv_pack_node_weights(const float* w_f, const float* w_s, int C, int G, void* wn_t, int dtype,
                                            mdlStream_t stream) {
    using namespace mdl;
    MDL_REQUIRE(dtype == MDL_BF16 || dtype == MDL_F32, MDL_E_UNSUPP, "mdl_cgconv_pack_node_weights: dtype must be MDL_BF16 or MDL_F32");
    MDL_REQUIRE(w_f && w_s && wn_t && C >= 1 && G >= 0, MDL_E_ARG, "mdl_cgconv_pack_node_weights: bad arguments");
    const int Cp = (C + 31) / 32 * 32;
    if (dtype == MDL_F32)
        hipLaunchKernelGGL(cgconv_pack_node_kernel<float>, dim3((unsigned)cdiv((int64_t)C * 4 * Cp, 256)), dim3(256), 0, (hipStream_t)stream,
                           w_f, w_s, C, Cp, 2 * C + G, (float*)wn_t);
    else
    hipLaunchKernelGGL(cgconv_pack_node_kernel<bf16_t>, dim3((unsigned)cdiv((int64_t)C * 4 * Cp, 256)), dim3(256), 0, (hipStream_t)stream, w_f,
                       w_s, C, Cp, 2 * C + G, (bf16_t*)wn_t);
    return check_launch("mdl_cgconv_pack_node_weights");
}

extern "C" int mdl_cgconv_assemble_grads(const float* dwn, const float* dwe, const float* db, int C, int G, float* dw_f,
                                         float* dw_s, float* db_f, float* db_s, mdlStream_t stream) {
    using namespace mdl;
    MDL_REQUIRE(dwn && dwe && db && dw_f && dw_s && C >= 1 && G >= 0, MDL_E_ARG, "mdl_cgconv_assemble_grads: bad arguments");
    const int Cp = (C + 31) / 32 * 32, GP = (G + 63) / 64 * 64;
    hipLaunchKernelGGL(cgconv_grads_kernel, dim3((unsigned)cdiv((int64_t)2 * C * (2 * C + G), 256)), dim3(256), 0, (hipStream_t)stream,
                       dwn, dwe, db, C, Cp, G, GP, dw_f, dw_s, db_f, db_s);
    return check_launch("mdl_cgconv_assemble_grads");
}

static int bwd_node_launch(const void* x, const void* grad_out, const void* r_tgt, float* r_src, const void* wn_t, void* dx,
                           float* dwn, int64_t N, int C, int dtype, int zero_src, bool rs16, mdlStream_t stream);

extern "C" int mdl_cgconv_bwd_node_ex(const MdlCgNode* a, mdlStream_t stream) {
    MDL_REQUIRE(a && a->size == sizeof(MdlCgNode), MDL_E_ARG, "mdl_cgconv_bwd_node_ex: argument struct of another layout (size %u, expected %u)",
                a ? a->size : 0u, (unsigned)sizeof(MdlCgNode));
    MDL_REQUIRE((a->flags & ~(uint32_t)(MDL_DETERMINISTIC | MDL_SPLIT_BF16)) == 0, MDL_E_ARG, "mdl_cgconv_bwd_node_ex: unknown flag bits %#x", a->flags);
    MDL_REQUIRE(a->r_src_dtype == MDL_F32 || a->r_src_dtype == MDL_BF16, MDL_E_ARG, "mdl_cgconv_bwd_node_ex: r_src_dtype must be MDL_F32 or MDL_BF16");
    if (a->flags & MDL_SPLIT_BF16) {
        using namespace mdl;
        MDL_REQUIRE(a->dtype == MDL_F32 && a->r_src_dtype == MDL_F32 && a->C == 64 && !(a->flags & MDL_DETERMINISTIC), MDL_E_UNSUPP,
                    "mdl_cgconv_bwd_node_ex: MDL_SPLIT_BF16 needs MDL_F32 storage, fp32 by-source sums, C = 64 (C=%d dtype=%d)", a->C, a->dtype);
        MDL_REQUIRE(a->N >= 0 && (a->N == 0 || (a->x && a->grad_out && a->r_tgt && a->r_src && a->wn_t && a->dx && a->dwn)), MDL_E_ARG,
                    "mdl_cgconv_bwd_node_ex: bad arguments");
        MDL_REQUIRE(reinterpret_cast<uintptr_t>(a->wn_t) % 16 == 0 && reinterpret_cast<uintptr_t>(a->r_tgt) % 16 == 0 &&
                        reinterpret_cast<uintptr_t>(a->r_src) % 16 == 0 && reinterpret_cast<uintptr_t>(a->x) % 16 == 0 &&
                        reinterpret_cast<uintptr_t>(a->grad_out) % 4 == 0 && reinterpret_cast<uintptr_t>(a->dx) % 4 == 0, MDL_E_ARG,
                    "mdl_cgconv_bwd_node_ex: 16-byte alignment required");
        if (a->N == 0) return MDL_OK;
        constexpr int NWX = 8;
        const int lds = (2 * 64 * (256 + 8) + 2 * 64 * (256 + 8) + 2 * 64 * (64 + 8)) * 2;
        int64_t sgrid = cdiv(a->N, 64);
        if (sgrid > 256) sgrid = 256;
        auto kf = cgconv_node_x3_kernel<64, NWX>;
        hipError_t e = set_max_dynamic_lds(reinterpret_cast<const void*>(kf), lds);
        if (e != hipSuccess) { set_error("mdl_cgconv_bwd_node_ex: LDS attribute (%d B): %s", lds, hipGetErrorString(e)); return MDL_E_LAUNCH; }
        hipLaunchKernelGGL(kf, dim3((unsigned)sgrid), dim3(64 * NWX), lds, (hipStream_t)stream, (const float*)a->x, (const float*)a->grad_out,
                           (const float*)a->r_tgt, static_cast<float*>(a->r_src), (const float*)a->wn_t, (float*)a->dx, a->dwn, a->N, a->zero_src);
        return check_launch("mdl_cgconv_bwd_node_ex");
    }
    return bwd_node_launch(a->x, a->grad_out, a->r_tgt, static_cast<float*>(a->r_src), a->wn_t, a->dx, a->dwn, a->N, a->C,
                           a->dtype | (int)a->flags, a->zero_src, a->r_src_dtype == MDL_BF16, stream);
}

static int bwd_node_launch(const void* x, const void* grad_out, const void* r_tgt, float* r_src, const void* wn_t, void* dx,
                           float* dwn, int64_t N, int C, int dtype, int zero_src, bool rs16, mdlStream_t stream) {
    using namespace mdl;
    const bool det = (dtype & MDL_DETERMINISTIC) != 0;
    dtype &= MDL_DTYPE_MASK;
    MDL_REQUIRE(dtype == MDL_BF16, MDL_E_UNSUPP, "mdl_cgconv_bwd_node: bf16 only (fp32 parity mode uses library GEMMs)");
    MDL_REQUIRE(C == 32 || C == 64, MDL_E_UNSUPP, "mdl_cgconv_bwd_node: C must be 32 or 64 (got %d)", C);
    MDL_REQUIRE(N >= 0 && (N == 0 || (x && grad_out && r_tgt && r_src && wn_t && dx && dwn)), MDL_E_ARG,
                "mdl_cgconv_bwd_node: bad arguments");
    MDL_REQUIRE(reinterpret_cast<uintptr_t>(wn_t) % 16 == 0 && reinterpret_cast<uintptr_t>(r_tgt) % 16 == 0 &&
                    reinterpret_cast<uintptr_t>(r_src) % 16 == 0, MDL_E_ARG, "mdl_cgconv_bwd_node: 16-byte alignment required");
    if (N == 0) return MDL_OK;
    hipStream_t st = (hipStream_t)stream;
    int64_t sgrid = cdiv(N, 64);
    if (det) sgrid = 1;
    if (sgrid > 256) sgrid = 256;
    if (C == 64) {
        const int lds = (64 * (256 + 8) + 64 * (256 + 8) + 64 * (64 + 8)) * 2;
        auto kf = rs16 ? cgconv_node_stream_kernel<64, true, K3C_NW> : cgconv_node_stream_kernel<64, false, K3C_NW>;
        set_max_dynamic_lds(reinterpret_cast<const void*>(kf), lds);
        hipLaunchKernelGGL(kf, dim3((unsigned)sgrid), dim3(64 * K3C_NW), lds, st, (const bf16_t*)x, (const bf16_t*)grad_out,
                           (const bf16_t*)r_tgt, r_src, (const bf16_t*)wn_t, (bf16_t*)dx, dwn, N, zero_src);
    } else {
        const int lds = (32 * (128 + 8) + 64 * (128 + 8) + 64 * (32 + 8)) * 2;
        auto kf = rs16 ? cgconv_node_stream_kernel<32, true> : cgconv_node_stream_kernel<32, false>;
        hipLaunchKernelGGL(kf, dim3((unsigned)sgrid), dim3(256), lds, st, (const bf16_t*)x, (const bf16_t*)grad_out,
                           (const bf16_t*)r_tgt, r_src, (const bf16_t*)wn_t, (bf16_t*)dx, dwn, N, zero_src);
    }
    return check_launch("mdl_cgconv_bwd_node");
}
```

### matdeeplearn_amd/csrc/cgconv_tiles.inc

```
#pragma once
#include <stdlib.h>
#include <type_traits>

#include "mdl_common.h"

#ifndef MDL_EXPERIMENTS
#define MDL_EXPERIMENTS 0
#endif

#ifdef MDL_CG_EP_TU
#define mdl_debug_life mdl_debug_life_ep
#define mdl_debug_read mdl_debug_read_ep
#define mdl_debug_reset mdl_debug_reset_ep
#endif
#ifdef MDL_CG_TIMING
__device__ long long g_cg_dbg[48];
__device__ long long g_cg_life[2][4096][3];
extern "C" int mdl_debug_life(long long* host, int which) {
    return (int)hipMemcpyFromSymbol(host, HIP_SYMBOL(g_cg_life), sizeof(long long) * 4096 * 3, sizeof(long long) * 4096 * 3 * which);
}
extern "C" int mdl_debug_read(long long* host48) {
    return (int)hipMemcpyFromSymbol(host48, HIP_SYMBOL(g_cg_dbg), 48 * sizeof(long long));
}
extern "C" int mdl_debug_reset() {
    long long z[48] = {0};
    return (int)hipMemcpyToSymbol(HIP_SYMBOL(g_cg_dbg), z, sizeof(z));
}
#define TDECL const long long tstart = clock64(), wstart = wall_clock64(); long long tprev = tstart; long long tacc[13] = {0, 0, 0, 0, 0, 0, 0, 0, 0, 0, 0, 0, 0}; long long tcount = 0
#define TMARK(k) do { __builtin_amdgcn_sched_barrier(0); const long long _t = clock64(); tacc[k] += _t - tprev; tprev = _t; __builtin_amdgcn_sched_barrier(0); } while (0)
#define TPIN16(v) do { _Pragma("unroll") for (int _r = 0; _r < 16; ++_r) asm volatile("" : "+v"(v[_r])); } while (0)
#define TTILE() (tcount += 1)
#define TRESET() TMARK(10)
#define TFLUSH(base) do { if (gw == 0 && lane == 0) { for (int _k = 0; _k < 13; ++_k) g_cg_dbg[(base) + _k] += tacc[_k]; g_cg_dbg[(base) + 15] += tcount; g_cg_dbg[(base) + 14] += clock64() - tstart; g_cg_dbg[(base) + 13] += wall_clock64() - wstart; } if (lane == 0 && gw < 4096) { g_cg_life[(base) / 16][gw][0] = wstart; g_cg_life[(base) / 16][gw][1] = wall_clock64(); g_cg_life[(base) / 16][gw][2] = tcount; } } while (0)
#else
#define TDECL do { } while (0)
#define TMARK(k) do { } while (0)
#define TPIN16(v) do { } while (0)
#define TTILE() do { } while (0)
#define TRESET() do { } while (0)
#define TFLUSH(base) do { } while (0)
#endif


namespace mdl {

struct CgParams {
    const void* x;
    const void* ea;
    const int32_t* rowptr;
    const int32_t* src;
    const int32_t* tgt;
    const int32_t* eperm;
    const void* wpack;
    const float* bpack;
    void* out;
    const void* gout;
    void* r_tgt;
    float* r_src;
    float* dwe;
    float* db;
    unsigned* ctr;
    void* ab;
    const int32_t* balance;
    int dwe_combine;
    int rs16;
    int flags;
    const void* pt;
    const void* ps;
    int64_t N, E;
    int C, G, Cp, KE, KT, WS, EKS, NS, GP, aggr;
    int GW;
    unsigned gw_inv;
    int n_groups;
    int g_full;
    int w_elems;
    int w_slice;
    int wave_lds_bytes;
    int bias_col;
};

struct CgDims {
    int Cp, KE, KT, WS, EKS, NS, GP;
};

static inline int rup(int a, int b) { return (a + b - 1) / b * b; }

static CgDims cg_dims(int C, int G, int dtype, bool x3 = false) {
    CgDims d;
    d.Cp = rup(C, 32);
    d.KE = rup(G, 16);
    d.KT = d.KE + 2 * d.Cp;
    const int pad = dtype == MDL_BF16 ? 8 : (x3 ? 4 : 1);
    d.WS = d.KT + pad;
    d.EKS = d.KE + pad;
    d.NS = d.Cp / 32;
    d.GP = rup(G, 64);
    return d;
}

template <typename T> struct Mma;
template <> struct Mma<bf16_t> {
    static constexpr int KSTEP = 16;
    static constexpr bool FAST = true;
    typedef bf16x8 frag_t;
    __device__ static __forceinline__ f32x16 mma(frag_t a, frag_t b, f32x16 c) {
        return __builtin_amdgcn_mfma_f32_32x32x16_bf16(a, b, c, 0, 0, 0);
    }
    __device__ static __forceinline__ frag_t zero() { return frag_t{0, 0, 0, 0, 0, 0, 0, 0}; }
};
template <> struct Mma<float> {
    static constexpr int KSTEP = 2;
    static constexpr bool FAST = false;
    typedef float frag_t;
    __device__ static __forceinline__ f32x16 mma(frag_t a, frag_t b, f32x16 c) {
        return __builtin_amdgcn_mfma_f32_32x32x2f32(a, b, c, 0, 0, 0);
    }
    __device__ static __forceinline__ frag_t zero() { return 0.0f; }
};

__device__ __forceinline__ bf16x8 ld_frag(const bf16_t* base, int row, int ld, int k0, int h) {
    return *reinterpret_cast<const bf16x8*>(base + row * ld + k0 + 8 * h);
}
__device__ __forceinline__ float ld_frag(const float* base, int row, int ld, int k0, int h) {
    return base[row * ld + k0 + h];
}

template <int VEC>
__device__ __forceinline__ bf16x8 ld_xfrag(const bf16_t* rowp, int c0, int h, int C) {
    const int c = c0 + 8 * h;
    bf16x8 v = {0, 0, 0, 0, 0, 0, 0, 0};
    if (VEC == 9) {
        v = *reinterpret_cast<const bf16x8*>(rowp + c);
    } else if (VEC == 8) {
        if (c < C) v = *reinterpret_cast<const bf16x8*>(rowp + c);
    } else if (VEC == 4) {
        bf16x4 lo = {0, 0, 0, 0}, hi = {0, 0, 0, 0};
        if (c < C) lo = *reinterpret_cast<const bf16x4*>(rowp + c);
        if (c + 4 < C) hi = *reinterpret_cast<const bf16x4*>(rowp + c + 4);
        v = bf16x8{lo[0], lo[1], lo[2], lo[3], hi[0], hi[1], hi[2], hi[3]};
    } else {
#pragma unroll
        for (int j = 0; j < 8; ++j)
            if (c + j < C) v[j] = (short)rowp[c + j];
    }
    return v;
}
template <int VEC>
__device__ __forceinline__ float ld_xfrag(const float* rowp, int c0, int h, int C) {
    const int c = c0 + h;
    if (VEC == 9) return rowp[c];
    return c < C ? rowp[c] : 0.0f;
}

typedef __attribute__((ext_vector_type(4))) unsigned u32x4;
__device__ __forceinline__ bf16x8 pack_bf16x8(const float* v) {
    u32x4 r = {pk_bf16(v[0], v[1]), pk_bf16(v[2], v[3]), pk_bf16(v[4], v[5]), pk_bf16(v[6], v[7])};
    return __builtin_bit_cast(bf16x8, r);
}

struct SplitFrag { bf16x8 hi, lo; };
__device__ __forceinline__ void split_pair(float v0, float v1, unsigned& hi, unsigned& lo) {
    hi = pk_bf16(v0, v1);
    const float r0 = v0 - __builtin_bit_cast(float, hi << 16);
    const float r1 = v1 - __builtin_bit_cast(float, hi & 0xffff0000u);
    lo = pk_bf16(r0, r1);
}
__device__ __forceinline__ SplitFrag split8(const f32x4& a, const f32x4& b) {
    unsigned h0, h1, h2, h3, l0, l1, l2, l3;
    split_pair(a[0], a[1], h0, l0);
    split_pair(a[2], a[3], h1, l1);
    split_pair(b[0], b[1], h2, l2);
    split_pair(b[2], b[3], h3, l3);
    return SplitFrag{__builtin_bit_cast(bf16x8, u32x4{h0, h1, h2, h3}), __builtin_bit_cast(bf16x8, u32x4{l0, l1, l2, l3})};
}
__device__ __forceinline__ SplitFrag split8_at(const float* p) {
    return split8(*reinterpret_cast<const f32x4*>(p), *reinterpret_cast<const f32x4*>(p + 4));
}
__device__ __forceinline__ f32x16 mma_x3(const SplitFrag& a, const SplitFrag& b, f32x16 c) {
    c = __builtin_amdgcn_mfma_f32_32x32x16_bf16(a.lo, b.hi, c, 0, 0, 0);
    c = __builtin_amdgcn_mfma_f32_32x32x16_bf16(a.hi, b.lo, c, 0, 0, 0);
    return __builtin_amdgcn_mfma_f32_32x32x16_bf16(a.hi, b.hi, c, 0, 0, 0);
}
__device__ __forceinline__ SplitFrag ld_wfrag_x3(const float* wbase, int row, int ld, int k0, int h) {
    const char* g = reinterpret_cast<const char*>(wbase + row * ld) + (k0 / 8 + h) * 32;
    return SplitFrag{*reinterpret_cast<const bf16x8*>(g), *reinterpret_cast<const bf16x8*>(g + 16)};
}

template <typename T, int CP_, int G_, int EW, int WSP = 0, bool X3 = false>
struct Dims {
    static constexpr bool STATIC = (CP_ != 0) && (G_ != 0);
    static constexpr int PADW = std::is_same<T, bf16_t>::value ? 8 : (X3 ? 4 : 1);
    static_assert(!X3 || (std::is_same<T, float>::value && STATIC && WSP == 0), "x3: fp32 storage, static shapes");
    int C, Cp, G, KE, WS, EKS, GW;
    __device__ __forceinline__ Dims(const CgParams& p) {
        C = p.C;
        Cp = CP_ ? CP_ : p.Cp;
        G = G_ ? G_ : p.G;
        KE = G_ ? ((G_ + 15) / 16 * 16) : p.KE;
        WS = KE + (WSP ? 0 : 2 * Cp) + PADW;
        EKS = KE + PADW;
        GW = G / EW;
    }
};

template <typename T>
struct WaveCtx {
    T* et;
    unsigned* tsl;
    int* srcl;
    unsigned* ssl;
    bf16_t* oh_t;
    bf16_t* oh_e;
    bf16_t* oh_w;
// ... 504 lines not shown
```

### matdeeplearn_amd/ops.py

```python
import collections
import os
import weakref

import torch

from . import _lib
from ._lib import MdlError, check, dtype_code, lib, ptr, require_hip, stream

_ACT_CODE = {"relu": 1, "ssp": 2}
_LN2 = 0.6931471805599453


def _f32c(t):
    return None if t is None else t.detach().float().contiguous()


def _stream_key(device):
    return (device.index, torch.cuda.current_stream(device).cuda_stream)


class EdgeCSR:

    __slots__ = ("rowptr", "src", "tgt", "eperm", "N", "E", "_row", "_col", "_t", "_attr", "_tb", "_bal", "partial", "__weakref__")

    def __init__(self, rowptr, src, tgt, eperm, N, E, row=None, col=None):
        self.rowptr, self.src, self.tgt, self.eperm, self.N, self.E = rowptr, src, tgt, eperm, int(N), int(E)
        self._attr = None
        self._bal = None
        self._row, self._col, self._t, self._tb = row, col, None, None
        self.partial = False

    def set_transposed(self, t):
        self._t = tuple(t)

    def set_transposed_builder(self, fn):
        self._tb = fn

    def balance(self):
        if self._bal is None:
            cost = torch.empty(self.N + 1, dtype=torch.int32, device=self.rowptr.device)
            check(lib().mdl_cgconv_balance(ptr(self.rowptr), ptr(self.src), self.N, ptr(cost), stream()), "mdl_cgconv_balance")
            self._bal = torch.cumsum(cost, 0, dtype=torch.int32)
        return self._bal

    def refresh_balance(self):
        if not (_BALANCE and self.E >= 400000 and self.eperm is None):
            return
        if self._bal is None:
            self._bal = torch.zeros(self.N + 1, dtype=torch.int32, device=self.rowptr.device)
        cost = torch.empty(self.N + 1, dtype=torch.int32, device=self.rowptr.device)
        check(lib().mdl_cgconv_balance(ptr(self.rowptr), ptr(self.src), self.N, ptr(cost), stream()), "mdl_cgconv_balance")
        torch.cumsum(cost, 0, dtype=torch.int32, out=self._bal)

    def seg_tgt(self):
        if self.eperm is not None:
            return None
        return make_seg_index(self.rowptr, self.tgt, partial=self.partial)

    def seg_src(self):
        if self.eperm is not None:
            return None
        rowptr_s, _, eid_s, src_sorted = self.transposed()
        si = make_seg_index(rowptr_s, src_sorted, partial=self.partial)
        si.perm = eid_s
        return si

    def sorted_attr(self, edge_attr):
        if self.eperm is None:
            return edge_attr
        k = (edge_attr.data_ptr(), edge_attr._version, edge_attr.dtype, tuple(edge_attr.shape))
        if self._attr is None or self._attr[0] != k:
            self._attr = (k, edge_attr.index_select(0, self.eperm.long()).contiguous(), edge_attr)
        return self._attr[1]

    @property
    def row(self):
        if self._row is None:
            self._row = _unsort_edges(self.src, self)
        return self._row

    @property
    def col(self):
        if self._col is None:
            self._col = _unsort_edges(self.tgt, self)
        return self._col

    def transposed(self):
        if self._t is None and self._tb is not None:
            self._t = tuple(self._tb())
        if self._t is None:
            perm = torch.argsort(self.src, stable=True)
            src_sorted = self.src.index_select(0, perm)
            col_s = self.tgt.index_select(0, perm)
            eid_s = (perm if self.eperm is None else self.eperm.long().index_select(0, perm)).to(torch.int32)
            self._t = (csr_rowptr(src_sorted.contiguous(), self.N), col_s.contiguous(), eid_s.contiguous(),
                       src_sorted.contiguous())
        return self._t


def csr_rowptr(sorted_index_i32, num_segments):
    require_hip(sorted_index_i32)
    rowptr = torch.empty(num_segments + 1, dtype=torch.int32, device=sorted_index_i32.device)
    check(lib().mdl_csr_rowptr(ptr(sorted_index_i32), sorted_index_i32.numel(), num_segments, ptr(rowptr), stream()),
          "mdl_csr_rowptr")
    return rowptr


def build_csr(edge_index, num_nodes, assume_sorted=False):
    require_hip(edge_index)
    row, col = edge_index[0], edge_index[1]
    if assume_sorted:
        tgt = col.to(torch.int32).contiguous()
        src = row.to(torch.int32).contiguous()
        eperm = None
    else:
        perm = torch.argsort(col, stable=True)
        tgt = col.index_select(0, perm).to(torch.int32)
        src = row.index_select(0, perm).to(torch.int32)
        eperm = perm.to(torch.int32)
    return EdgeCSR(csr_rowptr(tgt, num_nodes), src, tgt, eperm, num_nodes, col.numel(),
                   row=None if assume_sorted else row.to(torch.int32).contiguous(),
                   col=None if assume_sorted else col.to(torch.int32).contiguous())


_CSR_CACHE = collections.OrderedDict()
_CSR_CACHE_MAX = 64
_CSR_CACHE_MAX_BYTES = 256 << 20
_csr_cache_bytes = 0


def _key(edge_index, n):
    return (edge_index.data_ptr(), edge_index._version, tuple(edge_index.shape), int(n), edge_index.device.index)


def _csr_entry_bytes(edge_index, csr):
    return edge_index.numel() * edge_index.element_size() + 4 * (3 * csr.E + csr.N + 1) + (4 * csr.E if csr.eperm is not None else 0)


def register_csr(edge_index, csr):
    global _csr_cache_bytes
    k = _key(edge_index, csr.N)
    old = _CSR_CACHE.pop(k, None)
    if old is not None:
        _csr_cache_bytes -= old[2]
    nb = _csr_entry_bytes(edge_index, csr)
    _CSR_CACHE[k] = (csr, edge_index, nb)
    _csr_cache_bytes += nb
    while len(_CSR_CACHE) > 1 and (len(_CSR_CACHE) > _CSR_CACHE_MAX or _csr_cache_bytes > _CSR_CACHE_MAX_BYTES):
        _csr_cache_bytes -= _CSR_CACHE.popitem(last=False)[1][2]


def csr_for(edge_index, num_nodes):
    if NO_INDEX_CACHE:
# ... 192 lines not shown


def make_seg_index(rowptr_i32, seg_i32, partial=False):
    si = _SegIndex()
    si.N, si.E, si.partial = rowptr_i32.numel() - 1, seg_i32.numel(), bool(partial)
    si.rowptr, si.seg, si.perm = rowptr_i32, seg_i32, None
    return si


def scatter_mean(src, index, dim=0, dim_size=None, assume_sorted=False):
    return scatter(src, index, dim, dim_size, "mean", assume_sorted)


def scatter_add(src, index, dim=0, dim_size=None, assume_sorted=False):
    return scatter(src, index, dim, dim_size, "sum", assume_sorted)


def global_mean_pool(x, batch, size=None, seg_index=None):
    return scatter(x, batch, 0, size, "mean", assume_sorted=True, seg_index=seg_index)


def global_add_pool(x, batch, size=None, seg_index=None):
    return scatter(x, batch, 0, size, "sum", assume_sorted=True, seg_index=seg_index)


def global_max_pool(x, batch, size=None, seg_index=None):
    return scatter(x, batch, 0, size, "max", assume_sorted=True, seg_index=seg_index)


POOLS = {"global_mean_pool": global_mean_pool, "global_add_pool": global_add_pool,
         "global_max_pool": global_max_pool}


def _rup(a, b):
    return (a + b - 1) // b * b


KERNEL_EVENTS = None


def _launch_timed(key, fn):
    ev = KERNEL_EVENTS
    if ev is None or key not in ev:
        return fn()
    a, b = torch.cuda.Event(enable_timing=True), torch.cuda.Event(enable_timing=True)
    a.record()
    rc = fn()
    b.record()
    ev[key].append((a, b))
    return rc


class ZeroArena:

    def __init__(self, device, nbytes=4 << 20):
        self.buf = torch.empty(nbytes // 4, dtype=torch.float32, device=device)
        self.off = 0

    def reset(self):
        self.buf.zero_()
        self.off = 0

    def take(self, shape):
        n = 1
        for d in shape:
            n *= int(d)
        n_al = (n + 63) & ~63
        if self.off + n_al > self.buf.numel():
            return None
        t = self.buf[self.off:self.off + n].view(*shape)
        self.off += n_al
        return t


_ARENA = None

_GRAD_ARENA = None


def new_grad_arena(device, nfloats):
    global _GRAD_ARENA
    _GRAD_ARENA = [torch.zeros(int(nfloats), dtype=torch.float32, device=device), 0]


def _zeros_grad(n, device):
    a = _GRAD_ARENA
    n_al = (int(n) + 63) & ~63
    if a is not None and a[0].device == device and a[1] + n_al <= a[0].numel():
        t = a[0][a[1]:a[1] + int(n)]
        a[1] += n_al
        return t
    return torch.zeros(int(n), dtype=torch.float32, device=device)


class zero_arena:
    def __init__(self, device, nbytes=4 << 20):
        self.key = (torch.device(device), nbytes)

    _cache = {}

    def __enter__(self):
        global _ARENA
        a = zero_arena._cache.get(self.key)
        if a is None:
            a = zero_arena._cache[self.key] = ZeroArena(*self.key)
        a.reset()
        self.prev, _ARENA = _ARENA, a
        return a

    def __exit__(self, *exc):
        global _ARENA
        _ARENA = self.prev
        return False


def _zeros_step(shape, device):
    a = _ARENA
    if a is not None and a.buf.device == device:
        t = a.take(shape)
        if t is not None:
            return t
    return torch.zeros(shape, dtype=torch.float32, device=device)


_WS = {}


def _workspace(device, nbytes):
    key = _stream_key(device)
    t = _WS.get(key)
    if t is None or t.numel() < nbytes:
        t = _WS[key] = torch.empty(max(int(nbytes), 256), dtype=torch.uint8, device=device)
    return t


_TN_SCRATCH = True
_TNS = {}


_TN_SCRATCH_MIN_ROWS = 4096
_DENSE_MIN_ROWS = 64


def _tn_scratch(device, rows=None):
    if not _TN_SCRATCH or (rows is not None and rows < _TN_SCRATCH_MIN_ROWS):
        return None
    key = _stream_key(device)
    t = _TNS.get(key)
    if t is None:
        t = _TNS[key] = torch.empty(lib().mdl_tn_scratch_bytes(), dtype=torch.uint8, device=device)
    return t


def _gemm_tn(a, lda, M, y, ldy, act, b, ldb, K, c, colsum, N, flags, device):
    return lib().mdl_gemm_tn_ex(ptr(a), lda, M, ptr(y), ldy, act, ptr(b), ldb, K, ptr(c), ptr(colsum), ptr(_tn_scratch(device, N)), N, flags,
                                stream())


_DET = False


def set_deterministic(on=True):
    global _DET
    prev, _DET = _DET, bool(on)
    return prev


class deterministic:
    def __init__(self, on=True):
        self.on = on

    def __enter__(self):
        self.prev = set_deterministic(self.on)
        return self

    def __exit__(self, *exc):
        set_deterministic(self.prev)
        return False


OPTIONS = {
    "deterministic": ("_DET", "bit-reproducible launch shapes of every atomically accumulating kernel (slow; HIP-vs-HIP tests)"),
    "gmr_dw": ("_GMR_DW", "CFConv backward: dh and dw from one walk over the by-source CSR"),
    "balance": ("_BALANCE", "cost-balanced node ranges for the edge-per-lane CGConv backward (E >= 4e5)"),
    "pad128": ("_PAD128", "C in (96, 128): static 128-channel CGConv kernels on zero-padded rows"),
    "rsrc16": ("_RSRC16", "by-source sums of the CGConv backward in bf16 (packed atomics)"),
    "cfconv_fused": ("_CFCONV_FUSED", "K4: the fused CFConv forward"),
    "cfconv_recompute": ("_CFCONV_RECOMPUTE", "K4b: CFConv backward with the filter recomputed (no per-edge activations)"),
    "tn_colsum": ("_TN_COLSUM", "bias gradients out of the TN GEMM"),
    "dense_bwd": ("_DENSE_BWD", "dX + dW + db of a tall dense layer in one pass"),
    "dense_bwd_wide": ("_DENSE_BWD_WIDE", "... also when both widths exceed 128"),
    "mlp_head": ("_MLP_HEAD", "post-FC head as one launch per direction"),
    "linear_wide": ("_LINEAR_WIDE", "NNConv's Y = x W2r on the streaming kernel"),
    "set2set_fused": ("_SET2SET_FUSED", "Set2Set readout: all processing steps in one launch per direction (off: torch's LSTM + the composed attention)"),
    "tn_scratch": ("_TN_SCRATCH", "weight-gradient blocks of the TN products as plain stores + a reduce launch (off: atomics from every workgroup)"),
}


def configure(**kw):
    prev = {}
    g = globals()
    for k, v in kw.items():
        if k not in OPTIONS:
            raise MdlError("ops.configure: unknown option %r (known: %s)" % (k, ", ".join(sorted(OPTIONS))))
        attr = OPTIONS[k][0]
        prev[k] = g[attr]
        g[attr] = bool(v)
    return prev


def options():
    return {k: globals()[a] for k, (a, _) in OPTIONS.items()}


def _dflag():
    return _lib.MDL_DETERMINISTIC if _DET else 0


K3_VARIANT = None


def _k3flag():
    return {None: 0, "per_wave": _lib.MDL_K3_PER_WAVE, "edge_lane": _lib.MDL_K3_EDGE_LANE}[K3_VARIANT]


def last_k3():
    return int(lib().mdl_debug_last_k3())


_GMR_DW = True
_BALANCE = True
_PAD128 = True
_RSRC16 = True


_RSRC = {}


_RSRC_CAP = {}


def _take_rsrc(nfloats, device):
    if torch.cuda.is_current_stream_capturing():
        owned = _RSRC_CAP.setdefault(device.index, [])
        for ent in owned:
            if ent[0].numel() >= nfloats and not ent[1]:
                return ent
        cand = [k for k, v in _RSRC.items() if k[0] == device.index and not v[1] and v[0].numel() >= nfloats]
        if not cand:
            return None
        ent = _RSRC.pop(max(cand, key=lambda k: _RSRC[k][0].numel()))
        owned.append(ent)
        return ent
    key = _stream_key(device)
    ent = _RSRC.get(key)
    if ent is None or ent[0].numel() < nfloats or ent[1]:
        ent = _RSRC[key] = [torch.zeros(int(nfloats), dtype=torch.float32, device=device), False]
    return ent


class _CGConvFn(torch.autograd.Function):
    @staticmethod
    def forward(ctx, x, edge_attr, w_f, b_f, w_s, b_s, csr, aggr, packed=None, split=False, d_norm=None, rbf=None):
        require_hip(x, edge_attr, w_f, w_s)
        if edge_attr.dtype != x.dtype:
            raise MdlError("cgconv: x (%s) and edge_attr (%s) must share a dtype" % (x.dtype, edge_attr.dtype))
        x, edge_attr = x.contiguous(), edge_attr.contiguous()
        N, C = x.shape
        E, G = edge_attr.shape
        if csr.N != N or csr.E != E:
            raise MdlError("cgconv: CSR (%d nodes, %d edges) does not match x/edge_attr (%d, %d)" % (csr.N, csr.E, N, E))
        dt = dtype_code(x)
        L = lib()
        sp = _lib.MDL_SPLIT_BF16 if (split and dt == _lib.MDL_F32 and G == 50 and E > 0 and not _DET
                                     and ((C == 64 and x.data_ptr() % 16 == 0) or (_PAD128 and 96 < C <= 128))) else 0
        ctx.split = sp
        wf32, ws32, bf32, bs32 = _f32c(w_f), _f32c(w_s), _f32c(b_f), _f32c(b_s)
        nbytes = L.mdl_cgconv_wpack_bytes(C, G, dt | sp)
        if nbytes == 0:
            raise MdlError("cgconv: unsupported C=%d G=%d" % (C, G))
        Ck = C
        if _PAD128 and (dt == _lib.MDL_BF16 or sp) and G == 50 and 96 < C < 128 and (csr.eperm is None or sp) and E > 0:
            Ck = 128
            x = torch.nn.functional.pad(x, (0, Ck - C))
        use_packed = packed is not None and packed[3] == (C, G, dt)
        wn_t = None
        if use_packed:
            wpack, bpack, wn_t = packed[:3]
        elif dt == _lib.MDL_BF16 and (C in (32, 64) or Ck == 128) and any(ctx.needs_input_grad):
            wpack = torch.empty(nbytes, dtype=torch.uint8, device=x.device)
            bpack = torch.empty(2 * _rup(C, 32), dtype=torch.float32, device=x.device)
            wn_t = torch.empty((C, 4 * _rup(C, 32)), dtype=torch.bfloat16, device=x.device)
            check(L.mdl_cgconv_pack_weights_node(ptr(wf32), ptr(bf32), ptr(ws32), ptr(bs32), C, G, ptr(wpack), ptr(bpack),
                                                 ptr(wn_t), dt, stream()), "mdl_cgconv_pack_weights_node")
        else:
            wpack, bpack = _plain_pack(wf32, bf32, ws32, bs32, C, G, dt | sp, x.device, nbytes)
        ctx.wn_t = wn_t
        out = torch.empty_like(x)
        edge_attr = csr.sorted_attr(edge_attr)
        args = _lib.cg_args(dtype=dt, flags=sp, aggr=aggr, N=N, E=E, C=Ck, G=G, x=x, edge_attr=edge_attr, rowptr=csr.rowptr, src=csr.src,
                            tgt=csr.tgt, wpack=wpack, bpack=bpack, out=out)
        check(_launch_timed("fwd", lambda: L.mdl_cgconv_fwd_ex(args, stream())), "mdl_cgconv_fwd_ex")
        dist_saved = () if d_norm is None else (d_norm.detach().contiguous(), rbf[0].contiguous())
        ctx.save_for_backward(x, edge_attr, wf32, ws32, wpack, bpack, *dist_saved)
        ctx.rbf_coeff = None if d_norm is None else float(rbf[1])
        ctx.bias32 = (bf32, bs32)
        ctx.csr, ctx.aggr, ctx.has_bias = csr, aggr, (b_f is not None, b_s is not None)
        ctx.wdtypes = (w_f.dtype, w_s.dtype)
        ctx.C = C
        return out if Ck == C else out[:, :C].contiguous()

    @staticmethod
    @torch.autograd.function.once_differentiable
    def backward(ctx, g):
        need_de = ctx.needs_input_grad[1]
        need_dd = len(ctx.needs_input_grad) > 10 and ctx.needs_input_grad[10] and ctx.rbf_coeff is not None
        de, dd = _cgconv_edge_grads(ctx, g, need_de, need_dd) if (need_de or need_dd) else (None, None)
        grads = _CGConvFn._backward_main(ctx, g)
        return grads[:1] + (de,) + grads[2:] + (dd, None)

    @staticmethod
    def _backward_main(ctx, g):
        x, edge_attr, wf32, ws32, wpack, bpack = ctx.saved_tensors[:6]
        csr = ctx.csr
        N, Ck = x.shape
        C = ctx.C
        E, G = edge_attr.shape
        Cp, GP = _rup(C, 32), _rup(G, 64)
        g = g.contiguous()
        dt = dtype_code(x)
        xk, gk = x, g
        if Ck != C:
            gk = torch.nn.functional.pad(g, (0, Ck - C))
            x = x[:, :C]
        r_tgt = torch.empty((N, 2 * Cp), dtype=x.dtype, device=x.device)
        sp = ctx.split
        node_x3 = bool(sp) and dt == _lib.MDL_F32 and C == 64
        node_hip = (dt == _lib.MDL_BF16 and C == Cp and C in (32, 64)) or node_x3
        rs16 = (_RSRC16 and dt == _lib.MDL_BF16 and (node_hip or Ck == 128) and G == 50 and E > 0
                and x.data_ptr() % 16 == 0 and edge_attr.data_ptr() % 4 == 0)
        nrs = N * 2 * Cp // 2 if rs16 else N * 2 * Cp
        keep = _take_rsrc(nrs, x.device) if node_hip else None
        if keep is not None:
            r_src, keep[1] = keep[0][:nrs], True
            r_src = r_src.view(torch.bfloat16).view(N, 2 * Cp) if rs16 else r_src.view(N, 2 * Cp)
        else:
            r_src = torch.zeros((N, 2 * Cp), dtype=torch.bfloat16 if rs16 else torch.float32, device=x.device)
        small = _zeros_step((2 * Cp * GP + 2 * Cp + 4 * Cp * C,), x.device)
        dwe = small[:2 * Cp * GP].view(2 * Cp, GP)
        db = small[2 * Cp * GP:2 * Cp * GP + 2 * Cp]
        dwn = small[2 * Cp * GP + 2 * Cp:].view(4 * Cp, C)
        ws = _workspace(x.device, lib().mdl_cgconv_workspace_bytes(N, E, C, G, dt))
        fl = _dflag()
        bal = csr.balance() if (rs16 and _BALANCE and E >= 400000 and not fl) else None
        eargs = _lib.cg_args(dtype=dt, flags=fl | (_k3flag() if rs16 else 0) | sp, aggr=ctx.aggr, N=N, E=E, C=Ck, G=G, x=xk, edge_attr=edge_attr,
                             rowptr=csr.rowptr, src=csr.src, tgt=csr.tgt, wpack=wpack, bpack=bpack, grad_out=gk, r_tgt=r_tgt, r_src=r_src,
                             r_src_dtype=_lib.MDL_BF16 if rs16 else _lib.MDL_F32, dwe=dwe, db=db, workspace=ws,
                             workspace_bytes=ws.numel(), balance=bal)
        check(_launch_timed("bwd", lambda: lib().mdl_cgconv_bwd_ex(eargs, stream())), "mdl_cgconv_bwd_ex")
        if node_hip:
            wn_t = _node_weights(ctx, C, Cp, torch.float32 if node_x3 else torch.bfloat16, x.device, wf32, ws32)
            dx = torch.empty_like(x)
            nargs = _lib.cg_node_args(dtype=dt, flags=fl | (sp if node_x3 else 0), zero_src=1 if keep is not None else 0, N=N, C=C,
                                      r_src_dtype=_lib.MDL_BF16 if rs16 else _lib.MDL_F32, x=x, grad_out=g, r_tgt=r_tgt, r_src=r_src,
                                      wn_t=wn_t, dx=dx, dwn=dwn)
            check(_launch_timed("bwd_node", lambda: lib().mdl_cgconv_bwd_node_ex(nargs, stream())), "mdl_cgconv_bwd_node_ex")
            if keep is not None:
                keep[1] = False
            dW_f, db_f, dW_s, db_s = _assemble_grads(ctx, dwn, dwe, db, C, G, x.device, timed=True)
        elif dt == _lib.MDL_BF16 and Cp == 128 and C % 2 == 0 and N > 0:
            rs_b = r_src.to(torch.bfloat16)
            wn_t = _node_weights(ctx, C, Cp, torch.bfloat16, x.device, wf32, ws32)
            dx = torch.addmm(g, r_tgt, wn_t[:, :2 * Cp].t())
            dx.addmm_(rs_b, wn_t[:, 2 * Cp:].t())
            xc = x.contiguous()
            for blk, r in enumerate((r_tgt[:, :Cp], r_tgt[:, Cp:], rs_b[:, :Cp], rs_b[:, Cp:])):
                check(_gemm_tn(r, r.stride(0), Cp, None, 0, 0, xc, xc.stride(0), C, dwn[blk * Cp:(blk + 1) * Cp], None, N, dt | fl,
                               x.device), "mdl_gemm_tn")
            dW_f, db_f, dW_s, db_s = _assemble_grads(ctx, dwn, dwe, db, C, G, x.device, timed=False)
        else:
            Wn = torch.cat([wf32[:, :C], ws32[:, :C], wf32[:, C:2 * C], ws32[:, C:2 * C]], dim=0)
            rt = r_tgt.view(N, 2, Cp)[:, :, :C]
            rs = r_src.view(N, 2, Cp)[:, :, :C]
            cd = torch.float32 if dt == _lib.MDL_F32 else torch.bfloat16
            R = torch.cat([rt[:, 0], rt[:, 1], rs[:, 0], rs[:, 1]], dim=1).to(cd)
            dx = torch.addmm(g, R, Wn.to(cd))
            dWn = torch.mm(R.t(), x).float()
            dW_f = torch.cat([dWn[0:C], dWn[2 * C:3 * C], dwe[:C, :G]], dim=1)
            dW_s = torch.cat([dWn[C:2 * C], dWn[3 * C:4 * C], dwe[Cp:Cp + C, :G]], dim=1)
            db_f = db[:C].clone() if ctx.has_bias[0] else None
            db_s = db[Cp:Cp + C].clone() if ctx.has_bias[1] else None
        return dx, None, dW_f.to(ctx.wdtypes[0]), db_f, dW_s.to(ctx.wdtypes[1]), db_s, None, None, None, None


def _node_weights(ctx, C, Cp, dtype, device, wf32, ws32):
    wn_t, ctx.wn_t = ctx.wn_t, None
    if wn_t is None:
        wn_t = torch.empty((C, 4 * Cp), dtype=dtype, device=device)
        check(lib().mdl_cgconv_pack_node_weights(ptr(wf32), ptr(ws32), C, wf32.shape[1] - 2 * C, ptr(wn_t), dtype_code(wn_t), stream()),
              "mdl_cgconv_pack_node_weights")
    return wn_t


def _assemble_grads(ctx, dwn, dwe, db, C, G, device, timed):
    dW_f = torch.empty((C, 2 * C + G), dtype=torch.float32, device=device)
    dW_s = torch.empty_like(dW_f)
    db_f = torch.empty(C, dtype=torch.float32, device=device) if ctx.has_bias[0] else None
    db_s = torch.empty(C, dtype=torch.float32, device=device) if ctx.has_bias[1] else None
    launch = lambda: lib().mdl_cgconv_assemble_grads(ptr(dwn), ptr(dwe), ptr(db), C, G, ptr(dW_f), ptr(dW_s), ptr(db_f), ptr(db_s), stream())
    check(_launch_timed("bwd_grads", launch) if timed else launch(), "mdl_cgconv_assemble_grads")
    return dW_f, db_f, dW_s, db_s


def cgconv_prepack(convs, x_dtype, device, want_node=True):
    import ctypes
    if len(convs) < 2 or len(convs) > 16 or device.type != "cuda":
        return None
    C, G = convs[0].channels, convs[0].dim
    dt = _lib.MDL_BF16 if x_dtype == torch.bfloat16 else _lib.MDL_F32
    if any(c.channels != C or c.dim != G or c.lin_f.weight.dtype != torch.float32 or not c.lin_f.weight.is_contiguous()
           or not c.lin_s.weight.is_contiguous() or (c.lin_f.bias is None) != (convs[0].lin_f.bias is None) for c in convs):
        return None
    if not (dt == _lib.MDL_BF16 and (C in (32, 64) or (_PAD128 and G == 50 and 96 < C < 128))):
        return None
    L = lib()
    nbytes = L.mdl_cgconv_wpack_bytes(C, G, dt)
    if nbytes == 0:
        return None
    n = len(convs)
    wbuf = torch.empty((n, nbytes), dtype=torch.uint8, device=device)
    bbuf = torch.empty((n, 2 * _rup(C, 32)), dtype=torch.float32, device=device)
    nbuf = torch.empty((n, C, 4 * _rup(C, 32)), dtype=torch.bfloat16, device=device) if want_node else None
    tab = lambda ts: (ctypes.c_void_p * n)(*[None if t is None else t.data_ptr() for t in ts])
    has_b = convs[0].lin_f.bias is not None
    check(L.mdl_cgconv_pack_weights_multi(
        n, tab([c.lin_f.weight.detach() for c in convs]), tab([c.lin_f.bias.detach() for c in convs]) if has_b else None,
        tab([c.lin_s.weight.detach() for c in convs]), tab([c.lin_s.bias.detach() for c in convs]) if has_b else None, C, G,
        tab(list(wbuf)), tab(list(bbuf)), tab(list(nbuf)) if want_node else None, dt, stream()), "mdl_cgconv_pack_weights_multi")
    return [(wbuf[k], bbuf[k], nbuf[k] if want_node else None, (C, G, dt)) for k in range(n)]


def cgconv(x, edge_index, edge_attr, w_f, b_f, w_s, b_s, aggr="mean", csr=None, packed=None, split=False, dist=None):
    if aggr not in ("mean", "add", "sum"):
        raise MdlError("cgconv: aggr must be mean or add")
    if csr is None:
        csr = csr_for(edge_index, x.shape[0])
    if dist is None:
        return _CGConvFn.apply(x, edge_attr, w_f, b_f, w_s, b_s, csr, _lib.REDUCE[aggr], packed, split)
    d_norm, offsets, coeff = _check_dist("cgconv", dist, edge_attr, "edge_attr")
    return _CGConvFn.apply(x, edge_attr, w_f, b_f, w_s, b_s, csr, _lib.REDUCE[aggr], packed, split, d_norm, (offsets.float(), float(coeff)))


def _check_dist(name, dist, edge_attr, what):
    d_norm, offsets, coeff = dist
    require_hip(d_norm, offsets)
    if d_norm.dtype != torch.float32 or d_norm.numel() != edge_attr.shape[0] or offsets.numel() != edge_attr.shape[1]:
        raise MdlError("%s: dist = (d_norm [E] float32, offsets [G], coeff) must match %s %s" % (name, what, tuple(edge_attr.shape)))
    return d_norm, offsets, coeff


def _dist_grad_inputs(name, x, edge_index, d_norm, csr, start, stop, resolution, width, edge_attr, out):
    if csr is None:
        csr = csr_for(edge_index, x.shape[0])
    if d_norm.dtype != torch.float32 or d_norm.numel() != csr.E or csr.N != x.shape[0]:
        raise MdlError("%s: d_norm must be [E] float32 over the CSR's %d edges" % (name, csr.E))
    if out is not None and csr.eperm is not None:
        raise MdlError("%s: out= needs an edge list in CSR (target-sorted) order" % name)
    offsets = rbf_offsets(start, stop, resolution, x.device)
    d_sorted = _sort_edges(d_norm, csr).contiguous()
    if edge_attr is None:
        ea = rbf_expand(d_sorted.detach(), start, stop, resolution, width, out_dtype=x.dtype, offsets=offsets)
    else:
        ea = csr.sorted_attr(edge_attr.detach().contiguous())
    return csr, offsets, d_sorted, ea


def _bwd_edge_launch(x, ea_sorted, csr, wpack, bpack, g, aggr, C, G, de=None, d_sorted=None, offsets=None, coeff=0.0, scale=1.0, dd=None):
    check(_launch_timed("bwd_edge", lambda: lib().mdl_cgconv_bwd_edge(
        ptr(x), ptr(ea_sorted), ptr(csr.rowptr), ptr(csr.src), ptr(csr.tgt), ptr(wpack), ptr(bpack), ptr(g), x.shape[0], ea_sorted.shape[0],
        C, G, aggr, dtype_code(x), ptr(de), ptr(d_sorted), ptr(offsets), float(coeff), float(scale), ptr(dd), stream())),
        "mdl_cgconv_bwd_edge")


def _plain_pack(wf32, bf32, ws32, bs32, C, G, dt, device, nbytes=None):
    wpack = torch.empty(lib().mdl_cgconv_wpack_bytes(C, G, dt) if nbytes is None else nbytes, dtype=torch.uint8, device=device)
    bpack = torch.empty(2 * _rup(C, 32), dtype=torch.float32, device=device)
    check(lib().mdl_cgconv_pack_weights(ptr(wf32), ptr(bf32), ptr(ws32), ptr(bs32), C, G, ptr(wpack), ptr(bpack), dt, stream()),
          "mdl_cgconv_pack_weights")
    return wpack, bpack


def _unsort_edges(t, csr):
    if csr.eperm is None:
        return t
    out = torch.empty_like(t)
    out[csr.eperm.long()] = t
    return out


def _cgconv_edge_grads(ctx, g, need_de, need_dd):
    saved = ctx.saved_tensors
    x, edge_attr, wf32, ws32, wpack, bpack = saved[:6]
    csr = ctx.csr
    C = ctx.C
    E, G = edge_attr.shape
    dt = dtype_code(x)
    if x.shape[1] != C:
        x = x[:, :C].contiguous()
    g = g.contiguous()
    if ctx.split:
        wpack, bpack = _plain_pack(wf32, ctx.bias32[0], ws32, ctx.bias32[1], C, G, dt, x.device)
    de = dd = None
    if need_de:
        de = (torch.zeros if csr.partial else torch.empty)((E, G), dtype=edge_attr.dtype, device=x.device)
        _bwd_edge_launch(x, edge_attr, csr, wpack, bpack, g, ctx.aggr, C, G, de=de)
        de = _unsort_edges(de, csr)
    if need_dd:
        d_norm, offsets = saved[6], saved[7]
        d_sorted = _sort_edges(d_norm, csr)
        dd = torch.zeros(E, dtype=torch.float32, device=x.device)
        _bwd_edge_launch(x, edge_attr, csr, wpack, bpack, g, ctx.aggr, C, G, d_sorted=d_sorted, offsets=offsets, coeff=ctx.rbf_coeff, dd=dd)
        dd = _unsort_edges(dd, csr)
    return de, dd


def cgconv_dist_grad(x, edge_index, d_norm, w_f, b_f, w_s, b_s, grad_out, aggr="mean", csr=None, start=0.0, stop=1.0, resolution=50,
                     width=0.2, scale=1.0, edge_attr=None, out=None):
    if aggr not in ("mean", "add", "sum"):
        raise MdlError("cgconv_dist_grad: aggr must be mean or add")
    require_hip(x, d_norm, w_f, w_s, grad_out)
    with torch.no_grad():
        C, G, dt = x.shape[1], int(resolution), dtype_code(x)
        if lib().mdl_cgconv_wpack_bytes(C, G, dt) == 0:
            raise MdlError("cgconv_dist_grad: unsupported C=%d G=%d" % (C, G))
        csr, offsets, d_sorted, ea = _dist_grad_inputs("cgconv_dist_grad", x, edge_index, d_norm, csr, start, stop, G, width, edge_attr, out)
        wpack, bpack = _plain_pack(_f32c(w_f), _f32c(b_f), _f32c(w_s), _f32c(b_s), C, G, dt, x.device)
        dd = out if out is not None else torch.zeros(csr.E, dtype=torch.float32, device=x.device)
        _bwd_edge_launch(x.detach().contiguous(), ea, csr, wpack, bpack, grad_out.detach().to(x.dtype).contiguous(), _lib.REDUCE[aggr], C, G,
                         d_sorted=d_sorted, offsets=offsets, coeff=rbf_coeff(start, stop, width), scale=scale, dd=dd)
        return dd if out is not None else _unsort_edges(dd, csr)


class _Gather(torch.autograd.Function):
    @staticmethod
    def forward(ctx, src, index):
        require_hip(src, index)
        src = src.contiguous()
        idx = index.to(torch.int32).contiguous()
        C = src.numel() // max(src.shape[0], 1)
        out = torch.empty((idx.numel(),) + tuple(src.shape[1:]), dtype=src.dtype, device=src.device)
        check(lib().mdl_gather_rows(ptr(src), ptr(idx), ptr(out), idx.numel(), C, dtype_code(src), stream()),
              "mdl_gather_rows")
        ctx.index, ctx.n = index, src.shape[0]
        return out

    @staticmethod
    def backward(ctx, g):
        return scatter(g, ctx.index, 0, ctx.n, "sum"), None


def gather(src, index):
    return _Gather.apply(src, index)
# ... 1979 lines not shown
```

Before: 826.0 million.

## Write CGConv backward weight-gradient partials per workgroup and reduce in assembly

```diff
diff --git a/include/mdl_hip.h b/include/mdl_hip.h
--- a/include/mdl_hip.h
+++ b/include/mdl_hip.h
@@ -86,6 +86,9 @@
     void* workspace;
     size_t workspace_bytes;
     const int32_t* balance;
+    float* part;
+    int32_t part_cap;
+    int32_t* part_used;
 } MdlCgConv;
 int mdl_cgconv_fwd_ex(const MdlCgConv* args, mdlStream_t stream);
 int mdl_cgconv_bwd_ex(const MdlCgConv* args, mdlStream_t stream);
@@ -109,6 +112,10 @@
     const void* wn_t;
     void* dx;
     float* dwn;
+    float* part;
+    int64_t part_stride;
+    int32_t part_cap;
+    int32_t* part_used;
 } MdlCgNode;
 int mdl_cgconv_bwd_node_ex(const MdlCgNode* args, mdlStream_t stream);
 
diff --git a/include/mdl_hip_cgconv_part.h b/include/mdl_hip_cgconv_part.h
--- /dev/null
+++ b/include/mdl_hip_cgconv_part.h
@@ -0,0 +1,18 @@
+#ifndef MDL_HIP_CGCONV_PART_H
+#define MDL_HIP_CGCONV_PART_H
+
+#include "mdl_hip.h"
+
+#ifdef __cplusplus
+extern "C" {
+#endif
+
+size_t mdl_cgconv_part_slice_floats(int C, int G);
+
+int mdl_cgconv_assemble_grads_ex(const float* part, int n_node, int n_edge, const float* dwe, const float* db, int C, int G,
+                                 float* dw_f, float* dw_s, float* db_f, float* db_s, mdlStream_t stream);
+
+#ifdef __cplusplus
+}
+#endif
+#endif
diff --git a/matdeeplearn_amd/_build.py b/matdeeplearn_amd/_build.py
--- a/matdeeplearn_amd/_build.py
+++ b/matdeeplearn_amd/_build.py
@@ -30,7 +30,7 @@
 
 def _deps_mtime():
     hdrs = [os.path.join(CSRC, f) for f in os.listdir(CSRC) if f.endswith((".h", ".inc"))]
-    hdrs += [os.path.join(os.path.dirname(HERE), "include", h) for h in ("mdl_hip.h", "mdl_hip_analysis.h", "mdl_hip_dynamics.h")]
+    hdrs += [os.path.join(os.path.dirname(HERE), "include", h) for h in ("mdl_hip.h", "mdl_hip_analysis.h", "mdl_hip_dynamics.h", "mdl_hip_cgconv_part.h")]
     return max(os.path.getmtime(h) for h in hdrs)
 
 
diff --git a/matdeeplearn_amd/_lib.py b/matdeeplearn_amd/_lib.py
--- a/matdeeplearn_amd/_lib.py
+++ b/matdeeplearn_amd/_lib.py
@@ -30,12 +30,14 @@
     _fields_ = [("size", _u32), ("dtype", _i32), ("flags", _u32), ("aggr", _i32), ("N", _i64), ("E", _i64), ("C", _i32), ("G", _i32),
                 ("x", _vp), ("edge_attr", _vp), ("rowptr", _vp), ("src", _vp), ("tgt", _vp), ("eperm", _vp), ("wpack", _vp),
                 ("bpack", _vp), ("out", _vp), ("grad_out", _vp), ("r_tgt", _vp), ("r_src", _vp), ("r_src_dtype", _i32),
-                ("dwe", _vp), ("db", _vp), ("workspace", _vp), ("workspace_bytes", _sz), ("balance", _vp)]
+                ("dwe", _vp), ("db", _vp), ("workspace", _vp), ("workspace_bytes", _sz), ("balance", _vp),
+                ("part", _vp), ("part_cap", _i32), ("part_used", ctypes.POINTER(_i32))]
 
 
 class MdlCgNode(ctypes.Structure):
     _fields_ = [("size", _u32), ("dtype", _i32), ("flags", _u32), ("zero_src", _i32), ("N", _i64), ("C", _i32), ("r_src_dtype", _i32),
-                ("x", _vp), ("grad_out", _vp), ("r_tgt", _vp), ("r_src", _vp), ("wn_t", _vp), ("dx", _vp), ("dwn", _vp)]
+                ("x", _vp), ("grad_out", _vp), ("r_tgt", _vp), ("r_src", _vp), ("wn_t", _vp), ("dx", _vp), ("dwn", _vp),
+                ("part", _vp), ("part_stride", _i64), ("part_cap", _i32), ("part_used", ctypes.POINTER(_i32))]
 
 
 def _dp(t):
@@ -155,6 +157,11 @@
     "mdl_vacf_accumulate": (_i32, [_vp] * 8 + [_i64, _i64, _i32, _i32, _i32, _i32, _vp, _vp, _vp]),
 }
 
+CGCONV_PART_PROTOTYPES = {
+    "mdl_cgconv_part_slice_floats": (_sz, [_i32, _i32]),
+    "mdl_cgconv_assemble_grads_ex": (_i32, [_vp, _i32, _i32, _vp, _vp, _i32, _i32, _vp, _vp, _vp, _vp, _vp]),
+}
+
 _lib = None
 
 
@@ -170,7 +177,8 @@
                 "libmdl_hip.so not found at %s — build it with `python -m matdeeplearn_amd._build` "
                 "(hipcc --offload-arch=gfx950).  matdeeplearn_amd has no CPU/eager fallback." % LIB_PATH)
         handle = ctypes.CDLL(LIB_PATH)
-        for name, (res, args) in list(PROTOTYPES.items()) + list(ANALYSIS_PROTOTYPES.items()) + list(DYNAMICS_PROTOTYPES.items()):
+        for name, (res, args) in list(PROTOTYPES.items()) + list(ANALYSIS_PROTOTYPES.items()) + list(DYNAMICS_PROTOTYPES.items()) + \
+                list(CGCONV_PART_PROTOTYPES.items()):
             fn = getattr(handle, name)
             fn.restype, fn.argtypes = res, args
         _lib = handle
diff --git a/matdeeplearn_amd/csrc/cgconv.hip b/matdeeplearn_amd/csrc/cgconv.hip
--- a/matdeeplearn_amd/csrc/cgconv.hip
+++ b/matdeeplearn_amd/csrc/cgconv.hip
@@ -1,4 +1,5 @@
 #include "cgconv_tiles.inc"
+#include "../../include/mdl_hip_cgconv_part.h"
 #include "cgconv_fwd.inc"
 #include "cgconv_bwd.inc"
 
@@ -234,6 +235,14 @@
         }
     }
     if (bwd) g_last_k3 = det ? 3 : 1;
+    if (bwd && p.part) {
+        const size_t nb = ((size_t)2 * d.Cp * d.GP + 2 * d.Cp) * sizeof(float);
+        if (hipMemsetAsync(p.part, 0, nb, st) != hipSuccess) { set_error("%s: partial-slice memset failed", name); return MDL_E_LAUNCH; }
+        p.dwe = p.part;
+        p.db = p.part + (size_t)2 * d.Cp * d.GP;
+        p.part = nullptr;
+        p.part_used = 1;
+    }
     p.dwe_combine = (bwd && !det && waves == 4 && d.NS == 2 && w_lds && !p.w_slice && w_bytes >= 2 * 2 * 2 * 16 * 64 * 4) ? 1 : 0;
     while ((grid * waves) % d.NS) ++grid;
     if (p.w_slice) while (grid % d.NS) ++grid;
@@ -703,7 +712,9 @@
     int rc = cg_check("mdl_cgconv_bwd_ex", a->x, a->edge_attr, a->rowptr, a->src, a->tgt, a->wpack, a->bpack, a->N, a->E, a->C, a->G,
                       a->aggr, dtype);
     if (rc) return rc;
-    MDL_REQUIRE(a->N == 0 || (a->grad_out && a->r_tgt && a->r_src && a->dwe), MDL_E_ARG, "mdl_cgconv_bwd_ex: null pointer");
+    MDL_REQUIRE(a->N == 0 || (a->grad_out && a->r_tgt && a->r_src && (a->dwe || a->part)), MDL_E_ARG, "mdl_cgconv_bwd_ex: null pointer");
+    MDL_REQUIRE(!a->part || (a->part_cap >= 1 && a->part_used && reinterpret_cast<uintptr_t>(a->part) % 16 == 0), MDL_E_ARG,
+                "mdl_cgconv_bwd_ex: part needs part_cap >= 1, a host part_used and 16-byte alignment");
     MDL_REQUIRE(a->r_src_dtype == MDL_F32 || a->r_src_dtype == MDL_BF16, MDL_E_ARG, "mdl_cgconv_bwd_ex: r_src_dtype must be MDL_F32 or MDL_BF16");
     CgParams p = {};
     p.flags = (int)a->flags;
@@ -726,8 +737,17 @@
         MDL_REQUIRE(!a->balance && (a->flags & (MDL_K3_PER_WAVE | MDL_K3_EDGE_LANE)) == 0, MDL_E_ARG,
                     "mdl_cgconv_bwd_ex: the balance prefix and the MDL_K3_* flags go with bf16 by-source sums");
     }
-    if (dtype == MDL_BF16) return cg_launch<bf16_t>(true, p, dtype, (hipStream_t)stream, "mdl_cgconv_bwd_ex");
-    return cg_launch<float>(true, p, dtype, (hipStream_t)stream, "mdl_cgconv_bwd_ex");
+    if (a->part) {
+        const CgDims d = cg_dims(a->C, a->G, dtype, (a->flags & MDL_SPLIT_BF16) != 0);
+        p.part = a->part + (size_t)4 * d.Cp * a->C;
+        p.part_stride = (int64_t)mdl_cgconv_part_slice_floats(a->C, a->G);
+        p.part_cap = a->part_cap;
+        *a->part_used = 0;
+    }
+    rc = dtype == MDL_BF16 ? cg_launch<bf16_t>(true, p, dtype, (hipStream_t)stream, "mdl_cgconv_bwd_ex")
+                           : cg_launch<float>(true, p, dtype, (hipStream_t)stream, "mdl_cgconv_bwd_ex");
+    if (a->part) *a->part_used = p.part_used;
+    return rc;
 }
 
 extern "C" int mdl_debug_last_k3(void) { return mdl::g_last_k3; }
diff --git a/matdeeplearn_amd/csrc/cgconv_ep.hip b/matdeeplearn_amd/csrc/cgconv_ep.hip
--- a/matdeeplearn_amd/csrc/cgconv_ep.hip
+++ b/matdeeplearn_amd/csrc/cgconv_ep.hip
@@ -10,7 +10,11 @@
 namespace ep {
 int launch2(CgParams& p, hipStream_t st, int wgs, const char* name) {
     typedef Cfg2<64> F;
-    const int64_t eg = std::min<int64_t>(wgs > 0 ? wgs : 256, std::max<int64_t>(1, cdiv(p.E, 32 * F::NA * 2)));
+    int64_t eg = std::min<int64_t>(wgs > 0 ? wgs : 256, std::max<int64_t>(1, cdiv(p.E, 32 * F::NA * 2)));
+    if (p.part) {
+        eg = std::min<int64_t>(eg, p.part_cap);
+        p.part_used = (int)eg;
+    }
     auto kf = bwd2_kernel<64>;
     hipError_t e = set_max_dynamic_lds(reinterpret_cast<const void*>(kf), F::LDS);
     if (e != hipSuccess) { set_error("%s: LDS attribute (%d B): %s", name, F::LDS, hipGetErrorString(e)); return MDL_E_LAUNCH; }
diff --git a/matdeeplearn_amd/csrc/cgconv_ep2.inc b/matdeeplearn_amd/csrc/cgconv_ep2.inc
--- a/matdeeplearn_amd/csrc/cgconv_ep2.inc
+++ b/matdeeplearn_amd/csrc/cgconv_ep2.inc
@@ -468,6 +468,21 @@
     }
     TFLUSH(32);
     asm volatile("s_nop 15\n\ts_nop 15\n\ts_nop 15\n\ts_nop 15\n\ts_nop 15\n\ts_nop 15" : "+v"(dwe[0]), "+v"(dwe[1]));
+    if (p.part) {
+        float* const pw = p.part + (int64_t)blockIdx.x * p.part_stride;
+        float* const pb = pw + 2 * C_ * p.GP;
+#pragma unroll
+        for (int nt = 0; nt < 2; ++nt) {
+            const int gcol = nt * 32 + i;
+#pragma unroll
+            for (int r = 0; r < 16; ++r) {
+                const float v = dwe[nt][r] * escale;
+                if (gcol < F::G) pw[(32 * cb + d_row(r, h)) * p.GP + gcol] = v;
+                else if (gcol == F::G) pb[32 * cb + d_row(r, h)] = v;
+            }
+        }
+        return;
+    }
 #pragma unroll
     for (int nt = 0; nt < 2; ++nt) {
         const int gcol = nt * 32 + i;
diff --git a/matdeeplearn_amd/csrc/cgconv_node.hip b/matdeeplearn_amd/csrc/cgconv_node.hip
--- a/matdeeplearn_amd/csrc/cgconv_node.hip
+++ b/matdeeplearn_amd/csrc/cgconv_node.hip
@@ -1,4 +1,5 @@
 #include "mdl_common.h"
+#include "../../include/mdl_hip_cgconv_part.h"
 
 namespace mdl {
 
@@ -16,7 +17,8 @@
                                                                     const bf16_t* __restrict__ r_tgt,
                                                                     const float* __restrict__ r_src,
                                                                     const bf16_t* __restrict__ wn_t, bf16_t* __restrict__ dx,
-                                                                    float* __restrict__ dwn, int64_t N, int zero_src) {
+                                                                    float* __restrict__ dwn, int64_t N, int zero_src,
+                                                                    float* __restrict__ part, int64_t part_stride) {
     typedef __attribute__((ext_vector_type(4))) short s16x4;
     typedef __attribute__((address_space(3))) s16x4* lds4_t;
     constexpr int TN = 64;
@@ -149,13 +151,15 @@
             }
         }
     }
+    float* const dst = part ? part + (int64_t)blockIdx.x * part_stride : dwn;
 #pragma unroll
     for (int j = 0; j < MJ; ++j) {
         const int blk = wv * MJ + j, mt = blk / NT, nt = blk - mt * NT;
 #pragma unroll
         for (int r = 0; r < 16; ++r) {
             const int R = mt * 32 + d_row(r, h), K = nt * 32 + i;
-            unsafeAtomicAdd(dwn + (int64_t)R * CP + K, dw[j][r]);
+            if (part) dst[R * CP + K] = dw[j][r];
+            else unsafeAtomicAdd(dst + (int64_t)R * CP + K, dw[j][r]);
         }
     }
 }
@@ -349,6 +353,64 @@
         if (dst) dst[c] = db[part * Cp + c];
     }
 }
+constexpr int GR_W = 16;
+__global__ __launch_bounds__(64 * GR_W) void cgconv_grads_part_kernel(const float* __restrict__ part, int64_t stride, int n_node,
+                                                                       int n_edge, const float* __restrict__ dwe,
+                                                                       const float* __restrict__ db, int C, int Cp, int G, int GP,
+                                                                       float* __restrict__ dwf, float* __restrict__ dws,
+                                                                       float* __restrict__ dbf, float* __restrict__ dbs) {
+    __shared__ float red[GR_W][64];
+    const int lane = threadIdx.x & 63, w = threadIdx.x >> 6;
+    const int e = blockIdx.x * 64 + lane;
+    const int n_dwn = 4 * Cp * C, n_dwe = 2 * Cp * GP, total = n_dwn + n_dwe + 2 * Cp;
+    float acc = 0.0f;
+    if (e < total) {
+        int n = e < n_dwn ? n_node : n_edge;
+        const float* src = part + e;
+        if (n == 0) {
+            src = e < n_dwn + n_dwe ? dwe + (e - n_dwn) : db + (e - n_dwn - n_dwe);
+            n = 1;
+        }
+#pragma unroll 8
+        for (int s = w; s < n; s += GR_W) acc += src[(int64_t)s * stride];
+    }
+    red[w][lane] = acc;
+    __syncthreads();
+    if (w != 0 || e >= total) return;
+    float v = red[0][lane];
+#pragma unroll
+    for (int k = 1; k < GR_W; ++k) v += red[k][lane];
+    const int ldw = 2 * C + G;
+    if (e < n_dwn) {
+        const int R = e / C, k = e - R * C, blk = R / Cp, c = R - blk * Cp;
+        if (c < C) ((blk & 1) ? dws : dwf)[c * ldw + (blk >> 1) * C + k] = v;
+    } else if (e < n_dwn + n_dwe) {
+        const int q = e - n_dwn, R = q / GP, g = q - R * GP, part_i = R / Cp, c = R - part_i * Cp;
+        if (c < C && g < G) (part_i ? dws : dwf)[c * ldw + 2 * C + g] = v;
+    } else {
+        const int R = e - n_dwn - n_dwe, part_i = R / Cp, c = R - part_i * Cp;
+        float* dstb = part_i ? dbs : dbf;
+        if (c < C && dstb) dstb[c] = v;
+    }
+}
+}
+
+extern "C" size_t mdl_cgconv_part_slice_floats(int C, int G) {
+    if (C < 1 || G < 0) return 0;
+    const size_t Cp = (size_t)(C + 31) / 32 * 32, GP = (size_t)(G + 63) / 64 * 64;
+    return 4 * Cp * C + 2 * Cp * GP + 2 * Cp;
+}
+
+extern "C" int mdl_cgconv_assemble_grads_ex(const float* part, int n_node, int n_edge, const float* dwe, const float* db, int C, int G,
+                                            float* dw_f, float* dw_s, float* db_f, float* db_s, mdlStream_t stream) {
+    using namespace mdl;
+    MDL_REQUIRE(part && dw_f && dw_s && C >= 1 && G >= 0 && n_node >= 1 && n_edge >= 0 && (n_edge >= 1 || (dwe && db)), MDL_E_ARG,
+                "mdl_cgconv_assemble_grads_ex: bad arguments");
+    const int Cp = (C + 31) / 32 * 32, GP = (G + 63) / 64 * 64;
+    const int64_t slice = (int64_t)mdl_cgconv_part_slice_floats(C, G);
+    hipLaunchKernelGGL(cgconv_grads_part_kernel, dim3((unsigned)cdiv(slice, 64)), dim3(64 * GR_W), 0, (hipStream_t)stream, part, slice,
+                       n_node, n_edge, dwe, db, C, Cp, G, GP, dw_f, dw_s, db_f, db_s);
+    return check_launch("mdl_cgconv_assemble_grads_ex");
 }
 
 extern "C" int mdl_cgconv_pack_node_weights(const float* w_f, const float* w_s, int C, int G, void* wn_t, int dtype,
@@ -377,13 +439,18 @@
 }
 
 static int bwd_node_launch(const void* x, const void* grad_out, const void* r_tgt, float* r_src, const void* wn_t, void* dx,
-                           float* dwn, int64_t N, int C, int dtype, int zero_src, bool rs16, mdlStream_t stream);
+                           float* dwn, int64_t N, int C, int dtype, int zero_src, bool rs16, float* part, int64_t part_stride, int part_cap,
+                           int32_t* part_used, mdlStream_t stream);
 
 extern "C" int mdl_cgconv_bwd_node_ex(const MdlCgNode* a, mdlStream_t stream) {
     MDL_REQUIRE(a && a->size == sizeof(MdlCgNode), MDL_E_ARG, "mdl_cgconv_bwd_node_ex: argument struct of another layout (size %u, expected %u)",
                 a ? a->size : 0u, (unsigned)sizeof(MdlCgNode));
     MDL_REQUIRE((a->flags & ~(uint32_t)(MDL_DETERMINISTIC | MDL_SPLIT_BF16)) == 0, MDL_E_ARG, "mdl_cgconv_bwd_node_ex: unknown flag bits %#x", a->flags);
     MDL_REQUIRE(a->r_src_dtype == MDL_F32 || a->r_src_dtype == MDL_BF16, MDL_E_ARG, "mdl_cgconv_bwd_node_ex: r_src_dtype must be MDL_F32 or MDL_BF16");
+    MDL_REQUIRE(!a->part || (!(a->flags & (MDL_SPLIT_BF16 | MDL_DETERMINISTIC)) && a->part_cap >= 1 && a->part_used &&
+                             a->part_stride >= (int64_t)4 * ((a->C + 31) / 32 * 32) * a->C && reinterpret_cast<uintptr_t>(a->part) % 16 == 0),
+                MDL_E_ARG,
+                "mdl_cgconv_bwd_node_ex: part goes with the bf16 kernels outside MDL_DETERMINISTIC; it needs part_cap >= 1, part_stride >= 4Cp*C and a host part_used");
     if (a->flags & MDL_SPLIT_BF16) {
         using namespace mdl;
         MDL_REQUIRE(a->dtype == MDL_F32 && a->r_src_dtype == MDL_F32 && a->C == 64 && !(a->flags & MDL_DETERMINISTIC), MDL_E_UNSUPP,
@@ -407,36 +474,44 @@
         return check_launch("mdl_cgconv_bwd_node_ex");
     }
     return bwd_node_launch(a->x, a->grad_out, a->r_tgt, static_cast<float*>(a->r_src), a->wn_t, a->dx, a->dwn, a->N, a->C,
-                           a->dtype | (int)a->flags, a->zero_src, a->r_src_dtype == MDL_BF16, stream);
+                           a->dtype | (int)a->flags, a->zero_src, a->r_src_dtype == MDL_BF16, a->part, a->part_stride, a->part_cap, a->part_used, stream);
 }
 
 static int bwd_node_launch(const void* x, const void* grad_out, const void* r_tgt, float* r_src, const void* wn_t, void* dx,
-                           float* dwn, int64_t N, int C, int dtype, int zero_src, bool rs16, mdlStream_t stream) {
+                           float* dwn, int64_t N, int C, int dtype, int zero_src, bool rs16, float* part, int64_t part_stride, int part_cap,
+                           int32_t* part_used, mdlStream_t stream) {
     using namespace mdl;
     const bool det = (dtype & MDL_DETERMINISTIC) != 0;
     dtype &= MDL_DTYPE_MASK;
     MDL_REQUIRE(dtype == MDL_BF16, MDL_E_UNSUPP, "mdl_cgconv_bwd_node: bf16 only (fp32 parity mode uses library GEMMs)");
     MDL_REQUIRE(C == 32 || C == 64, MDL_E_UNSUPP, "mdl_cgconv_bwd_node: C must be 32 or 64 (got %d)", C);
-    MDL_REQUIRE(N >= 0 && (N == 0 || (x && grad_out && r_tgt && r_src && wn_t && dx && dwn)), MDL_E_ARG,
+    MDL_REQUIRE(N >= 0 && (N == 0 || (x && grad_out && r_tgt && r_src && wn_t && dx && (dwn || part))), MDL_E_ARG,
                 "mdl_cgconv_bwd_node: bad arguments");
+    if (part) *part_used = 0;
     MDL_REQUIRE(reinterpret_cast<uintptr_t>(wn_t) % 16 == 0 && reinterpret_cast<uintptr_t>(r_tgt) % 16 == 0 &&
                     reinterpret_cast<uintptr_t>(r_src) % 16 == 0, MDL_E_ARG, "mdl_cgconv_bwd_node: 16-byte alignment required");
     if (N == 0) return MDL_OK;
     hipStream_t st = (hipStream_t)stream;
     int64_t sgrid = cdiv(N, 64);
     if (det) sgrid = 1;
-    if (sgrid > 256) sgrid = 256;
+    if (part) {
+        if (sgrid > part_cap) sgrid = part_cap;
+        if (sgrid > 512) sgrid = 512;
+        *part_used = (int)sgrid;
+    } else if (sgrid > 256) {
+        sgrid = 256;
+    }
     if (C == 64) {
         const int lds = (64 * (256 + 8) + 64 * (256 + 8) + 64 * (64 + 8)) * 2;
         auto kf = rs16 ? cgconv_node_stream_kernel<64, true, K3C_NW> : cgconv_node_stream_kernel<64, false, K3C_NW>;
         set_max_dynamic_lds(reinterpret_cast<const void*>(kf), lds);
         hipLaunchKernelGGL(kf, dim3((unsigned)sgrid), dim3(64 * K3C_NW), lds, st, (const bf16_t*)x, (const bf16_t*)grad_out,
-                           (const bf16_t*)r_tgt, r_src, (const bf16_t*)wn_t, (bf16_t*)dx, dwn, N, zero_src);
+                           (const bf16_t*)r_tgt, r_src, (const bf16_t*)wn_t, (bf16_t*)dx, dwn, N, zero_src, part, part_stride);
     } else {
         const int lds = (32 * (128 + 8) + 64 * (128 + 8) + 64 * (32 + 8)) * 2;
         auto kf = rs16 ? cgconv_node_stream_kernel<32, true> : cgconv_node_stream_kernel<32, false>;
         hipLaunchKernelGGL(kf, dim3((unsigned)sgrid), dim3(256), lds, st, (const bf16_t*)x, (const bf16_t*)grad_out,
-                           (const bf16_t*)r_tgt, r_src, (const bf16_t*)wn_t, (bf16_t*)dx, dwn, N, zero_src);
+                           (const bf16_t*)r_tgt, r_src, (const bf16_t*)wn_t, (bf16_t*)dx, dwn, N, zero_src, part, part_stride);
     }
     return check_launch("mdl_cgconv_bwd_node");
 }
diff --git a/matdeeplearn_amd/csrc/cgconv_tiles.inc b/matdeeplearn_amd/csrc/cgconv_tiles.inc
--- a/matdeeplearn_amd/csrc/cgconv_tiles.inc
+++ b/matdeeplearn_amd/csrc/cgconv_tiles.inc
@@ -59,6 +59,9 @@
     float* r_src;
     float* dwe;
     float* db;
+    float* part;
+    int64_t part_stride;
+    int part_cap, part_used;
     unsigned* ctr;
     void* ab;
     const int32_t* balance;
diff --git a/matdeeplearn_amd/ops.py b/matdeeplearn_amd/ops.py
--- a/matdeeplearn_amd/ops.py
+++ b/matdeeplearn_amd/ops.py
@@ -1,4 +1,5 @@
 import collections
+import ctypes
 import os
 import weakref
 
@@ -497,6 +498,22 @@
     return t
 
 
+_CG_PARTIALS = True
+_CG_PART_SLICES = 256
+_CGP = {}
+
+
+def _cg_part_scratch(device, C, G):
+    per = int(lib().mdl_cgconv_part_slice_floats(C, G))
+    key = _stream_key(device)
+    ent = _CGP.get(key)
+    if ent is None or ent[0].numel() < per * _CG_PART_SLICES:
+        if ent is not None and torch.cuda.is_current_stream_capturing():
+            return None
+        ent = _CGP[key] = (torch.empty(per * _CG_PART_SLICES, dtype=torch.float32, device=device),)
+    return ent[0], per, _CG_PART_SLICES
+
+
 def _gemm_tn(a, lda, M, y, ldy, act, b, ldb, K, c, colsum, N, flags, device):
     return lib().mdl_gemm_tn_ex(ptr(a), lda, M, ptr(y), ldy, act, ptr(b), ldb, K, ptr(c), ptr(colsum), ptr(_tn_scratch(device, N)), N, flags,
                                 stream())
@@ -538,6 +555,7 @@
     "mlp_head": ("_MLP_HEAD", "post-FC head as one launch per direction"),
     "linear_wide": ("_LINEAR_WIDE", "NNConv's Y = x W2r on the streaming kernel"),
     "set2set_fused": ("_SET2SET_FUSED", "Set2Set readout: all processing steps in one launch per direction (off: torch's LSTM + the composed attention)"),
+    "cg_partials": ("_CG_PARTIALS", "CGConv backward: weight-gradient partials as plain stores, summed by the assembly launch (off: atomics)"),
     "tn_scratch": ("_TN_SCRATCH", "weight-gradient blocks of the TN products as plain stores + a reduce launch (off: atomics from every workgroup)"),
 }
 
@@ -691,28 +709,40 @@
             r_src = r_src.view(torch.bfloat16).view(N, 2 * Cp) if rs16 else r_src.view(N, 2 * Cp)
         else:
             r_src = torch.zeros((N, 2 * Cp), dtype=torch.bfloat16 if rs16 else torch.float32, device=x.device)
-        small = _zeros_step((2 * Cp * GP + 2 * Cp + 4 * Cp * C,), x.device)
-        dwe = small[:2 * Cp * GP].view(2 * Cp, GP)
-        db = small[2 * Cp * GP:2 * Cp * GP + 2 * Cp]
-        dwn = small[2 * Cp * GP + 2 * Cp:].view(4 * Cp, C)
+        fl = _dflag()
+        part = _cg_part_scratch(x.device, C, G) if (_CG_PARTIALS and node_hip and not node_x3 and not fl and N > 0) else None
+        part_edge = part is not None and rs16 and C == 64 and (K3_VARIANT == "edge_lane" or (K3_VARIANT is None and E >= 400000))
+        if part is None:
+            small = _zeros_step((2 * Cp * GP + 2 * Cp + 4 * Cp * C,), x.device)
+        elif part_edge:
+            small = None
+        else:
+            small = _zeros_step((2 * Cp * GP + 2 * Cp,), x.device)
+        dwe = None if small is None else small[:2 * Cp * GP].view(2 * Cp, GP)
+        db = None if small is None else small[2 * Cp * GP:2 * Cp * GP + 2 * Cp]
+        dwn = None if part is not None else small[2 * Cp * GP + 2 * Cp:].view(4 * Cp, C)
+        used_e, used_n = ctypes.c_int32(0), ctypes.c_int32(0)
+        pkw = {} if not part_edge else dict(part=part[0], part_cap=part[2], part_used=ctypes.pointer(used_e))
         ws = _workspace(x.device, lib().mdl_cgconv_workspace_bytes(N, E, C, G, dt))
-        fl = _dflag()
         bal = csr.balance() if (rs16 and _BALANCE and E >= 400000 and not fl) else None
         eargs = _lib.cg_args(dtype=dt, flags=fl | (_k3flag() if rs16 else 0) | sp, aggr=ctx.aggr, N=N, E=E, C=Ck, G=G, x=xk, edge_attr=edge_attr,
                              rowptr=csr.rowptr, src=csr.src, tgt=csr.tgt, wpack=wpack, bpack=bpack, grad_out=gk, r_tgt=r_tgt, r_src=r_src,
                              r_src_dtype=_lib.MDL_BF16 if rs16 else _lib.MDL_F32, dwe=dwe, db=db, workspace=ws,
-                             workspace_bytes=ws.numel(), balance=bal)
+                             workspace_bytes=ws.numel(), balance=bal, **pkw)
         check(_launch_timed("bwd", lambda: lib().mdl_cgconv_bwd_ex(eargs, stream())), "mdl_cgconv_bwd_ex")
         if node_hip:
             wn_t = _node_weights(ctx, C, Cp, torch.float32 if node_x3 else torch.bfloat16, x.device, wf32, ws32)
             dx = torch.empty_like(x)
             nargs = _lib.cg_node_args(dtype=dt, flags=fl | (sp if node_x3 else 0), zero_src=1 if keep is not None else 0, N=N, C=C,
                                       r_src_dtype=_lib.MDL_BF16 if rs16 else _lib.MDL_F32, x=x, grad_out=g, r_tgt=r_tgt, r_src=r_src,
-                                      wn_t=wn_t, dx=dx, dwn=dwn)
+                                      wn_t=wn_t, dx=dx, dwn=dwn,
+                                      **({} if part is None else dict(part=part[0], part_stride=part[1], part_cap=part[2],
+                                                                      part_used=ctypes.pointer(used_n))))
             check(_launch_timed("bwd_node", lambda: lib().mdl_cgconv_bwd_node_ex(nargs, stream())), "mdl_cgconv_bwd_node_ex")
             if keep is not None:
                 keep[1] = False
-            dW_f, db_f, dW_s, db_s = _assemble_grads(ctx, dwn, dwe, db, C, G, x.device, timed=True)
+            dW_f, db_f, dW_s, db_s = _assemble_grads(ctx, dwn, dwe, db, C, G, x.device, timed=True,
+                                                     part=None if part is None else (part[0], used_n.value, used_e.value))
         elif dt == _lib.MDL_BF16 and Cp == 128 and C % 2 == 0 and N > 0:
             rs_b = r_src.to(torch.bfloat16)
             wn_t = _node_weights(ctx, C, Cp, torch.bfloat16, x.device, wf32, ws32)
@@ -747,12 +777,16 @@
     return wn_t
 
 
-def _assemble_grads(ctx, dwn, dwe, db, C, G, device, timed):
+def _assemble_grads(ctx, dwn, dwe, db, C, G, device, timed, part=None):
     dW_f = torch.empty((C, 2 * C + G), dtype=torch.float32, device=device)
     dW_s = torch.empty_like(dW_f)
     db_f = torch.empty(C, dtype=torch.float32, device=device) if ctx.has_bias[0] else None
     db_s = torch.empty(C, dtype=torch.float32, device=device) if ctx.has_bias[1] else None
-    launch = lambda: lib().mdl_cgconv_assemble_grads(ptr(dwn), ptr(dwe), ptr(db), C, G, ptr(dW_f), ptr(dW_s), ptr(db_f), ptr(db_s), stream())
+    if part is not None:
+        launch = lambda: lib().mdl_cgconv_assemble_grads_ex(ptr(part[0]), part[1], part[2], ptr(dwe), ptr(db), C, G, ptr(dW_f), ptr(dW_s),
+                                                            ptr(db_f), ptr(db_s), stream())
+    else:
+        launch = lambda: lib().mdl_cgconv_assemble_grads(ptr(dwn), ptr(dwe), ptr(db), C, G, ptr(dW_f), ptr(dW_s), ptr(db_f), ptr(db_s), stream())
     check(_launch_timed("bwd_grads", launch) if timed else launch(), "mdl_cgconv_assemble_grads")
     return dW_f, db_f, dW_s, db_s
 
```

Result: faster. 868.0 million, median of 6 (+5.1%).
